# hlesmqh/WS3D

Hardware: AMD Instinct MI355X
Metric: KITTI scenes/sec (16384 pts) Stage-1 RPN fwd, 1/2/4/8 GPU; FPS+group HBM GB/s (higher is better)
Workload: dtype f32

## Files before the change

### include/ws3d_ops.h

```cpp
#ifndef WS3D_OPS_H
#define WS3D_OPS_H

#include <stddef.h>
#include <stdint.h>

#ifdef __cplusplus
extern "C" {
#endif

#define WS3D_OK 0
#define WS3D_E_INVALID (-1)
#define WS3D_E_LAUNCH (-2)
#define WS3D_E_WORKSPACE (-3)
#define WS3D_E_UNSUPPORTED (-4)

#if defined(__GNUC__)
#define WS3D_API __attribute__((visibility("default")))
#else
#define WS3D_API
#endif

typedef void *ws3d_stream_t;

#define WS3D_ABI_VERSION 6
WS3D_API int ws3d_abi_version(void);
WS3D_API int ws3d_tune(int key, int value);
WS3D_API int ws3d_dist_mode(void);
WS3D_API const char *ws3d_last_error(void);
WS3D_API int ws3d_device_info(char *name, int name_len, int *cu_count, int *lds_bytes_per_block);


WS3D_API int ws3d_furthest_point_sampling(int b, int n, int m, const float *xyz, float *temp, int32_t *idx,
                                 ws3d_stream_t stream);

WS3D_API int ws3d_furthest_point_sampling_gather(int b, int n, int m, const float *xyz, float *temp,
                                        int32_t *idx, float *new_xyz, ws3d_stream_t stream);

WS3D_API int ws3d_furthest_point_sampling_nested(int b, int n, int m, const float *xyz, int32_t *idx, float *new_xyz,
                                        ws3d_stream_t stream);

WS3D_API int ws3d_furthest_point_sampling_nested_chain(int b, int n, int levels, const int *m, const float *xyz, int32_t *const *idx,
                                                       float *const *new_xyz, ws3d_stream_t stream);


WS3D_API int ws3d_gather_points(int b, int c, int n, int npoints, const float *points, const int32_t *idx,
                       float *out, ws3d_stream_t stream);

WS3D_API int ws3d_gather_points_grad(int b, int c, int n, int npoints, const float *grad_out,
                            const int32_t *idx, float *grad_points, ws3d_stream_t stream);

WS3D_API int ws3d_ball_query(int b, int n, int m, float radius, int nsample, const float *new_xyz,
                    const float *xyz, int32_t *idx, const void *sorted, ws3d_stream_t stream);
WS3D_API int ws3d_ball_query_fill(int b, int n, int m, float radius, int nsample, const float *new_xyz,
                         const float *xyz, int32_t *idx, const void *sorted, ws3d_stream_t stream);
WS3D_API int ws3d_ball_query_pairs(int b, int n, int m, float radius, int nsample, const float *new_xyz, const float *xyz, int32_t *idx,
                          const void *sorted_grid, int32_t *rowc, int32_t *rowsrc, int32_t *total, ws3d_stream_t stream);

WS3D_API int ws3d_ball_query_pairs2(int b, int n, int m, const float *new_xyz, const float *xyz, const void *sorted_grid,
                                    float radius0, int nsample0, int32_t *idx0, int32_t *rowc0, int32_t *rowsrc0, int32_t *total0,
                                    float radius1, int nsample1, int32_t *idx1, int32_t *rowc1, int32_t *rowsrc1, int32_t *total1,
                                    ws3d_stream_t stream);


WS3D_API size_t ws3d_sorted_points_bytes(int b, int n);
WS3D_API int ws3d_sort_points_x(int b, int n, const float *xyz, void *sorted, ws3d_stream_t stream);
WS3D_API int ws3d_sort_points_xz(int b, int n, const float *xyz, void *sorted, ws3d_stream_t stream);
WS3D_API int ws3d_sort_points_grid(int b, int n, const float *xyz, void *sorted, ws3d_stream_t stream);
WS3D_API int ws3d_sort_points_jobs(int b, int njobs, const int *n, const int *kind, const float *const *xyz, void *const *sorted,
                                   ws3d_stream_t stream);

WS3D_API int ws3d_group_points(int b, int c, int n, int npoints, int nsample, const float *points,
                      const int32_t *idx, float *out, ws3d_stream_t stream);

WS3D_API int ws3d_group_points_grad(int b, int c, int n, int npoints, int nsample, const float *grad_out,
                           const int32_t *idx, float *grad_points, ws3d_stream_t stream);

WS3D_API int ws3d_query_and_group(int b, int n, int m, int c, float radius, int nsample, int use_xyz,
                         const float *xyz, const float *new_xyz, const float *features,
                         int32_t *idx_out, float *out, const void *sorted, ws3d_stream_t stream);

WS3D_API int ws3d_three_nn(int b, int n, int m, const float *unknown, const float *known, float *dist2,
                  int32_t *idx, const void *sorted_known, ws3d_stream_t stream);

WS3D_API int ws3d_three_nn_weights(long rows, const float *dist2, float *weight, ws3d_stream_t stream);
WS3D_API int ws3d_three_nn_w(int b, int n, int m, const float *unknown, const float *known, float *dist2, int32_t *idx, float *weight,
                             const void *sorted_known, ws3d_stream_t stream);
WS3D_API int ws3d_three_nn_wq(int b, int n, int m, const float *unknown, const float *known, float *dist2, int32_t *idx, float *weight,
                              const void *sorted_known, const void *sorted_unknown, ws3d_stream_t stream);
WS3D_API int ws3d_three_nn_jobs(int b, int njobs, const int *n, const int *m, const float *const *unknown, const void *const *sorted_known,
                                float *const *dist2, int32_t *const *idx, float *const *weight, const void *const *sorted_unknown,
                                ws3d_stream_t stream);

WS3D_API int ws3d_pool_nsample(long rows, int nsample, const float *x, float *out, uint8_t *arg, ws3d_stream_t stream);
WS3D_API int ws3d_pool_nsample_grad(long rows, int nsample, const float *grad_out, const uint8_t *arg, float *grad_x,
                                    ws3d_stream_t stream);

WS3D_API int ws3d_gemm_pool(long rows, int nsample, int k_dim, int o_dim, const float *x_rows, const float *wt,
                            const float *bias, int relu, float *out, int out_stride, const int32_t *gate, long gate_limit, ws3d_stream_t stream);

WS3D_API int ws3d_gather_gemm(int b, int n, int m, int nsample, int c_feat, int o_dim, const float *feats, const float *xyz,
                     const float *new_xyz, const int32_t *nbr, const float *wt, const float *bias, int relu, float *out,
                     ws3d_stream_t stream);

WS3D_API int ws3d_gather_gemm2(int b, int n, int m, int nsample, int c_feat, int o1, int o2, const float *feats, const float *xyz,
                      const float *new_xyz, const int32_t *nbr, const float *w1t, const float *b1, int relu1, const float *w2t,
                      const float *b2, int relu2, float *out, ws3d_stream_t stream);

WS3D_API int ws3d_pgather_gemm2(int b, int n, int m, int nsample, int o1, int o2, const float *pmat, int p_stride, const float *xyz,
                       const float *new_xyz, const int32_t *nbr, const float *w1x, const float *b1, int relu1,
                       const float *w2t, const float *b2, int relu2, float *out, const int32_t *gate, long gate_limit, ws3d_stream_t stream);
WS3D_API int ws3d_pgather_rows(int b, int n, int m, int nsample, int o1, const float *pmat, int p_stride, const float *xyz, const float *new_xyz,
                      const int32_t *nbr, const float *w1x, const float *b1, int relu1, float *out, ws3d_stream_t stream);

WS3D_API int ws3d_qinterp_rows(int b, int n, int m, int o, const float *q, const int32_t *idx, const float *weight, const float *lin,
                      const float *skip, int c1, const float *wb, const float *bias, int relu, float *out, ws3d_stream_t stream);


WS3D_API int ws3d_compact_pairs(long centres, int nsample, const int32_t *nbr, int32_t *rowc, int32_t *rowsrc, int32_t *total, ws3d_stream_t stream);
WS3D_API int ws3d_compact_pairs_count(long centres, int nsample, const int32_t *nbr, int32_t *cnt, ws3d_stream_t stream);
WS3D_API int ws3d_compact_pairs_rows(long centres, int nsample, const int32_t *nbr, const int32_t *cnt, const int32_t *incl, int32_t *rowc,
                            int32_t *rowsrc, int32_t *total, ws3d_stream_t stream);
WS3D_API int ws3d_pgather_gemm2_compact(int b, int n, int m, long max_rows, int o1, int o2, const float *pmat, int p_stride, const float *xyz,
                               const float *new_xyz, const int32_t *rowc, const int32_t *rowsrc, const int32_t *total, const float *w1x,
                               const float *b1, int relu1, const float *w2t, const float *b2, int relu2, float *out, long limit, ws3d_stream_t stream);
WS3D_API int ws3d_pgather_gemm3_compact(int b, int n, int m, long max_rows, int o1, int o2, int o3, const float *pmat, int p_stride, const float *xyz,
                               const float *new_xyz, const int32_t *rowc, const int32_t *rowsrc, const int32_t *total, const float *w1x,
                               const float *b1, int relu1, const float *w2t, const float *b2, int relu2, const float *w3t, const float *b3,
                               float *out, int out_stride, long limit, ws3d_stream_t stream);
WS3D_API int ws3d_gemm_pool_compact(long max_rows, int k_dim, int o_dim, const float *x_rows, const int32_t *rowc, const int32_t *total,
                           const float *wt, const float *bias, float *out, int out_stride, long limit, ws3d_stream_t stream);
typedef struct ws3d_compact_mlp_args {
    int b, n, m;
    long max_rows;
    int o1, o2, o3;
    const float *pmat;
    int p_stride;
    const float *xyz, *new_xyz;
    const int32_t *rowc, *rowsrc, *total;
    const float *w1x, *b1;
    int relu1;
    const float *w2t, *b2;
    int relu2;
    const float *w3t, *b3;
    float *mid;
    float *out;
    int out_stride;
    long limit;
} ws3d_compact_mlp_args;
WS3D_API int ws3d_compact_mlp_pair(int kind, const ws3d_compact_mlp_args *scale0, const ws3d_compact_mlp_args *scale1, ws3d_stream_t stream);
WS3D_API int ws3d_chain_mlp3_ticket_ints(void);
WS3D_API size_t ws3d_chain_mlp3_blob_floats(int o2);
WS3D_API int ws3d_chain_mlp3_pack(const ws3d_compact_mlp_args *scale, float *blob, ws3d_stream_t stream);
WS3D_API int ws3d_chain_mlp3(const ws3d_compact_mlp_args *scale0, const ws3d_compact_mlp_args *scale1, const float *blob0, const float *blob1,
                             int32_t *ticket, int workgroups, ws3d_stream_t stream);

WS3D_API int ws3d_sa_mlp3_pool_compact(int b, int n, int m, long max_rows, int c1, int c2, int c3, const float *xyz, const float *new_xyz,
                              const float *feat, const int32_t *rowc, const int32_t *rowsrc, const int32_t *total, const float *w1t,
                              const float *b1, const float *w2t, const float *b2, const float *w3t, const float *b3, float *out,
                              int out_stride, long limit, ws3d_stream_t stream);

WS3D_API int ws3d_sa_mlp3_pool_lists(int b, int n, int m, int nsample, int c1, int c2, int c3, const float *xyz, const float *new_xyz,
                            const float *feat, const int32_t *nbr, const float *w1t, const float *b1, const float *w2t, const float *b2,
                            const float *w3t, const float *b3, int relu3, float *out, int out_stride, const int32_t *gate, long gate_limit,
                            ws3d_stream_t stream);

WS3D_API int ws3d_interp_gemm(int b, int n, int m, int c2, int c1, int o_dim, const float *known_feats, const float *unknown_feats,
                     const int32_t *idx, const float *weight, const float *wt, const float *bias, int relu, float *out,
                     ws3d_stream_t stream);

WS3D_API size_t ws3d_conv1x1_wgrad_workspace_bytes(int b, int o, int c, long l);
WS3D_API int ws3d_conv1x1_wgrad(int b, int o, int c, long l, const float *grad_out, const float *x, float *grad_w,
                                void *workspace, size_t workspace_bytes, ws3d_stream_t stream);

WS3D_API size_t ws3d_bn_workspace_bytes(int b, int c, long l);
WS3D_API int ws3d_bn_relu_train_fwd(int b, int c, long l, const float *x, const float *gamma, const float *beta, float eps,
                                    float momentum, int relu, float *running_mean, float *running_var,
                                    int64_t *num_batches_tracked, float *y, float *save_mean, float *save_invstd,
                                    void *workspace, size_t workspace_bytes, ws3d_stream_t stream);
WS3D_API int ws3d_bn_relu_train_bwd(int b, int c, long l, const float *x, const float *dy, const float *gamma,
                                    const float *beta, const float *save_mean, const float *save_invstd, int relu, float *dx,
                                    float *dgamma, float *dbeta, void *workspace, size_t workspace_bytes, ws3d_stream_t stream);

WS3D_API int ws3d_three_interpolate(int b, int c, int m, int n, const float *points, const int32_t *idx,
                           const float *weight, float *out, ws3d_stream_t stream);

WS3D_API int ws3d_three_interpolate_grad(int b, int c, int n, int m, const float *grad_out,
                                const int32_t *idx, const float *weight, float *grad_points,
                                ws3d_stream_t stream);

WS3D_API size_t ws3d_scatter_workspace_bytes(int b, int c, int n_targets, long slots_per_scene);
WS3D_API int ws3d_group_points_grad_det(int b, int c, int n, int npoints, int nsample, const float *grad_out,
                                        const int32_t *idx, float *grad_points, void *workspace,
                                        size_t workspace_bytes, ws3d_stream_t stream);
WS3D_API int ws3d_three_interpolate_grad_det(int b, int c, int n, int m, const float *grad_out, const int32_t *idx,
                                             const float *weight, float *grad_points, void *workspace,
                                             size_t workspace_bytes, ws3d_stream_t stream);

WS3D_API int ws3d_bias_act_inplace(int b, int o_ch, long l, int relu, float *y, const float *bias,
                                   ws3d_stream_t stream);

WS3D_API int ws3d_rowmax_bias_act(int b, int o_ch, long m, int s, int relu, const float *y, const float *bias,
                                  float *out, ws3d_stream_t stream);

WS3D_API int ws3d_query_and_group_nlc(int b, int n, int m, int c, float radius, int nsample, int use_xyz,
                                      const float *xyz, const float *new_xyz, const float *features_nlc,
                                      int32_t *idx_out, float *out_nlc, const void *sorted, ws3d_stream_t stream);
WS3D_API int ws3d_three_interpolate_nlc(int b, int c, int m, int n, const float *feats_nlc, const int32_t *idx,
                                        const float *weight, float *out_nlc, int out_stride, ws3d_stream_t stream);
WS3D_API int ws3d_rowmax_rows(long rows_out, int ns, int o_ch, const float *y, float *out, int out_stride,
                              ws3d_stream_t stream);

WS3D_API int ws3d_sa_mlp3_pool(long rows, int nsample, int c1, int c2, int c3, const float *x_rows4,
                               const float *w1t, const float *b1, const float *w2t, const float *b2,
                               const float *w3t, const float *b3, int relu3, float *out, int out_stride,
                               ws3d_stream_t stream);

WS3D_API int ws3d_mlp2_rows(long rows, int k_dim, int o1, int o2, const float *x_rows, const float *w1t, const float *b1, int relu1,
                   const float *w2t, const float *b2, int relu2, float *out, int *ticket, ws3d_stream_t stream);

WS3D_API size_t ws3d_rpn_heads_blob_bytes(int o2);
WS3D_API int ws3d_rpn_heads_pack(int o2, const float *w1t, const float *b1, int relu1, const float *w2t, const float *b2, int relu2, void *blob,
                        ws3d_stream_t stream);
WS3D_API int ws3d_rpn_heads(long rows, const float *x_rows, int heads, const void *blob_cls, float *out_cls, int *ticket_cls, int o2_reg,
                   const void *blob_reg, float *out_reg, int *ticket_reg, int workgroups, ws3d_stream_t stream);

WS3D_API size_t ws3d_gemm_rows_pack_bytes(int k_dim, int n_dim);
WS3D_API int ws3d_gemm_rows_pack(int k_dim, int n_dim, const float *wt, void *pack, ws3d_stream_t stream);
WS3D_API int ws3d_gemm_rows_split(long rows, int k_dim, int n_dim, const float *a, const void *pack, const float *bias, int relu, float *out,
                         ws3d_stream_t stream);

WS3D_API int ws3d_qinterp_gemm(int b, int n, int m, int c, int o_dim, const float *q, const int32_t *idx, const float *weight, const float *lin,
                      const float *skip, int c1, const float *wb, const float *b1, int relu1, const float *w2t, const float *b2, int relu2,
                      float *out, ws3d_stream_t stream);


WS3D_API int ws3d_boxes_overlap_bev(int num_a, const float *boxes_a, int num_b, const float *boxes_b,
                           float *ans, ws3d_stream_t stream);

WS3D_API int ws3d_boxes_iou_bev(int num_a, const float *boxes_a, int num_b, const float *boxes_b,
                       float *ans, ws3d_stream_t stream);

WS3D_API int ws3d_boxes_iou3d_paired(int n, const float *boxes_a, const float *boxes_b, float *overlap_bev, float *iou2d, float *iou3d,
                                     ws3d_stream_t stream);

WS3D_API int ws3d_nms_mask(int boxes_num, const float *boxes, float thresh, int normal, int full_grid,
                  uint64_t *mask, ws3d_stream_t stream);

WS3D_API size_t ws3d_nms_workspace_bytes(int boxes_num);
WS3D_API int ws3d_nms(int boxes_num, const float *boxes, float thresh, int normal, int max_keep,
                      void *workspace, size_t workspace_bytes, int64_t *keep, int32_t *num_keep,
                      ws3d_stream_t stream);

WS3D_API int ws3d_nms_batched(int batch, int boxes_num, const float *boxes, float thresh, int normal,
                              int max_keep, void *workspace, size_t workspace_bytes, int64_t *keep,
                              int32_t *num_keep, ws3d_stream_t stream);


WS3D_API int ws3d_radius_nms_batched(int batch, int n, const float *centers, float radius, int max_keep,
                                     void *workspace, size_t workspace_bytes, int64_t *keep,
                                     int32_t *num_keep, ws3d_stream_t stream);

WS3D_API int ws3d_topk_sorted(int b, int n, int k, const float *scores, float *out_scores, int64_t *out_idx,
                              ws3d_stream_t stream);
WS3D_API size_t ws3d_topk_workspace_bytes(int b, int n);
WS3D_API int ws3d_topk_sorted_ws(int b, int n, int k, const float *scores, float *out_scores, int64_t *out_idx, void *workspace,
                                 size_t workspace_bytes, ws3d_stream_t stream);
WS3D_API int ws3d_topk_sorted_sigmoid(int b, int n, int k, const float *logits, float *out_scores, int64_t *out_idx, ws3d_stream_t stream);
WS3D_API int ws3d_topk_sorted_sigmoid_ws(int b, int n, int k, const float *logits, float *out_scores, int64_t *out_idx, void *workspace,
                                         size_t workspace_bytes, ws3d_stream_t stream);

WS3D_API int ws3d_decode_center_boxes(int b, int n, int bins, float loc_scope, float loc_bin_size, float h, float w,
                                      float l, const float *xyz, const float *rpn_reg, float *boxes,
                                      ws3d_stream_t stream);

WS3D_API int ws3d_gather_boxes_bev(int b, int n, int top, const float *box, const int64_t *order, float *box_sorted, float *bev,
                          ws3d_stream_t stream);
WS3D_API int ws3d_decode_gather_boxes_bev(int b, int n, int top, int bins, float loc_scope, float loc_bin_size, float h, float w, float l,
                                          const float *xyz, const float *rpn_reg, const int64_t *order, float *box_sorted, float *bev,
                                          ws3d_stream_t stream);
WS3D_API int ws3d_select_proposals(int b, int top, int keep_stride, int k, const float *box_sorted, const float *scores_sorted,
                          const int64_t *keep, const int32_t *num, float extra_width, float *boxes_out, float *scores_out,
                          int64_t *count, float *pooled_boxes, ws3d_stream_t stream);
WS3D_API int ws3d_select_proposals_packed(int b, int top, int keep_stride, int k, const float *box_sorted, const float *scores_sorted,
                                          const int64_t *keep, const int32_t *num, float extra_width, float *boxes_out, float *scores_out,
                                          int64_t *count, float *pooled_boxes, float *packed, ws3d_stream_t stream);
WS3D_API int ws3d_select_proposals_send(int b, int top, int keep_stride, int k, const float *box_sorted, const float *scores_sorted,
                                        const int64_t *keep, const int32_t *num, float extra_width, float *boxes_out, float *scores_out,
                                        int64_t *count, float *pooled_boxes, float *send, long send_stride, ws3d_stream_t stream);
WS3D_API int ws3d_split_points_clear(long rows, int c, const float *pc, float *xyz, float *feats, void *clear, size_t clear_bytes,
                                     ws3d_stream_t stream);


WS3D_API int ws3d_roipool3d(int batch_size, int pts_num, int boxes_num, int feature_in_len,
                   int sampled_pts_num, const float *xyz, const float *boxes3d,
                   const float *pts_feature, float *pooled_features, int32_t *pooled_empty_flag,
                   int32_t *pts_idx, ws3d_stream_t stream);
WS3D_API int ws3d_roipool3d_fill(int batch_size, int pts_num, int boxes_num, int feature_in_len,
                   int sampled_pts_num, const float *xyz, const float *boxes3d,
                   const float *pts_feature, float *pooled_features, int32_t *pooled_empty_flag,
                   int32_t *pts_idx, ws3d_stream_t stream);

WS3D_API size_t ws3d_roipool3d_workspace_bytes(int batch_size, int pts_num);
WS3D_API int ws3d_roipool3d_ws(int batch_size, int pts_num, int boxes_num, int feature_in_len, int sampled_pts_num, const float *xyz,
                               const float *boxes3d, const float *pts_feature, float *pooled_features, int32_t *pooled_empty_flag,
                               int32_t *pts_idx, int fill, void *workspace, size_t workspace_bytes, ws3d_stream_t stream);


WS3D_API int ws3d_pts_in_boxes3d(int boxes_num, int pts_num, const float *pts, const float *boxes3d,
                        int64_t *flag, ws3d_stream_t stream);


WS3D_API int ws3d_instance_clouds(int batch, int pts_num, int centres_num, int feat_len, int sampled_pts_num, float radius, int mask_mode,
                                  float mask_thresh, const float *pts, const float *score, const float *feats, const float *centres,
                                  const int32_t *num, float *cloud, float *cloud_feats, int32_t *count, int32_t *pts_idx,
                                  ws3d_stream_t stream);
WS3D_API int ws3d_instance_clouds_count(int batch, int pts_num, int centres_num, float radius, const float *pts, const float *centres,
                                        const int32_t *num, int32_t *count, ws3d_stream_t stream);
WS3D_API int ws3d_instance_clouds_emit(int batch, int pts_num, int centres_num, int feat_len, float radius, int mask_mode, float mask_thresh,
                                       const float *pts, const float *score, const float *feats, const float *centres, const int32_t *num,
                                       const int64_t *offsets, float *rows, float *row_feats, int32_t *row_idx, ws3d_stream_t stream);


WS3D_API int ws3d_click_prepare(int batch, int pts_num, int clicks_num, int side, const float *offsets, float gauss_height, float gauss_status,
                                float gauss_cov, float centre_y, const float *pts, const float *clicks, const int32_t *num, float *score,
                                float *cand, int32_t *cand_num, ws3d_stream_t stream);



WS3D_API int ws3d_kitti_overlaps(int metric, int criterion, int frames, long max_pairs, const int32_t *gt_off, const int32_t *dt_off,
                                 const int64_t *out_off, const double *dt_boxes, const double *gt_boxes, double *out,
                                 ws3d_stream_t stream);

WS3D_API int ws3d_kitti_collect_scores(int frames, int max_dt, const int32_t *gt_off, const int32_t *dt_off, const int64_t *out_off,
                                       const double *overlaps, const int32_t *ignored_gt, const int32_t *ignored_dt,
                                       const double *dt_score, double min_overlap, double *tp_score, int32_t *tp_flag,
                                       ws3d_stream_t stream);

WS3D_API size_t ws3d_kitti_count_workspace_bytes(int frames, int num_thresh);
WS3D_API int ws3d_kitti_count(int metric, int frames, int max_dt, int num_thresh, const double *thresholds, const int32_t *gt_off,
                              const int32_t *dt_off, const int32_t *dc_off, const int64_t *out_off, const double *overlaps,
                              const int32_t *ignored_gt, const int32_t *ignored_dt, const double *dt_score, const double *dt_alpha,
                              const double *gt_alpha, const double *dt_bbox, const double *dc_bbox, double min_overlap, int compute_aos,
                              void *workspace, size_t workspace_bytes, double *pr, ws3d_stream_t stream);


WS3D_API int ws3d_stage2_embed(long rows, int pts_per_cloud, const float *pts, const float *box_ce, float extend, const float *wx0,
                               const float *bx0, const float *wx1, const float *bx1, const float *wf0, const float *bf0, const float *wf1,
                               const float *bf1, const float *wm, const float *bm, float *xyz_out, float *feat, ws3d_stream_t stream);
WS3D_API int ws3d_stage2_boxes(int rows, int loc_bins, int head_bins, float loc_scope, float h, float w, float l, const float *rcnn_reg,
                               float *pred_boxes3d, float *box_ce, ws3d_stream_t stream);
WS3D_API int ws3d_stage2_select(int batch, int slots, float cls_thresh, float iou_thresh, const float *size_window, float ground_y,
                                const float *box_ce, const float *rcnn_ref, const float *rcnn_cls, const float *rcnn_iou, const float *center,
                                const int32_t *num, float *boxes, int32_t *keep, float *key, ws3d_stream_t stream);

WS3D_API int ws3d_stage2_rcnn_loss(int rows, int loc_bins, int head_bins, float loc_scope, float h, float w, float l, const float *rcnn_cls,
                                   const float *rcnn_reg, const float *pred_boxes3d, const float *gt_boxes, const float *cls, float *vals,
                                   int32_t *counts, float *grad_cls, float *grad_reg, ws3d_stream_t stream);
WS3D_API int ws3d_stage2_ioun_loss(int rows, const float *rcnn_iou, const float *rcnn_ref, const float *pred_boxes3d, const float *refined_box,
                                   const float *gt_boxes, const float *cls, float *vals, int32_t *counts, float *grad_iou, float *grad_ref,
                                   ws3d_stream_t stream);

#ifdef __cplusplus
}
#endif
#endif
```

### ws3d_amd/_lib.py

```python
from __future__ import annotations

import ctypes as C
import os

_HERE = os.path.dirname(os.path.abspath(__file__))
DIST_MODE = int(os.environ.get("WS3D_DIST_MODE", "0") or 0)
LIB_PATH = os.environ.get("WS3D_HIP_LIB") or os.path.join(
    _HERE, "libws3d_hip.so" if DIST_MODE == 0 else "libws3d_hip_dm%d.so" % DIST_MODE)

E_INVALID, E_LAUNCH, E_WORKSPACE, E_UNSUPPORTED = -1, -2, -3, -4
ABI_VERSION = 6

_vp = C.c_void_p
_i = C.c_int
_f = C.c_float
_sz = C.c_size_t

class CompactMlpArgs(C.Structure):
    _fields_ = [("b", _i), ("n", _i), ("m", _i), ("max_rows", C.c_long), ("o1", _i), ("o2", _i), ("o3", _i), ("pmat", _vp), ("p_stride", _i),
                ("xyz", _vp), ("new_xyz", _vp), ("rowc", _vp), ("rowsrc", _vp), ("total", _vp), ("w1x", _vp), ("b1", _vp), ("relu1", _i),
                ("w2t", _vp), ("b2", _vp), ("relu2", _i), ("w3t", _vp), ("b3", _vp), ("mid", _vp), ("out", _vp), ("out_stride", _i), ("limit", C.c_long)]


SIGNATURES = {
    "ws3d_abi_version": (_i, []),
    "ws3d_tune": (_i, [_i, _i]),
    "ws3d_dist_mode": (_i, []),
    "ws3d_last_error": (C.c_char_p, []),
    "ws3d_device_info": (_i, [C.c_char_p, _i, C.POINTER(_i), C.POINTER(_i)]),
    "ws3d_furthest_point_sampling": (_i, [_i, _i, _i, _vp, _vp, _vp, _vp]),
    "ws3d_furthest_point_sampling_gather": (_i, [_i, _i, _i, _vp, _vp, _vp, _vp, _vp]),
    "ws3d_furthest_point_sampling_nested": (_i, [_i, _i, _i, _vp, _vp, _vp, _vp]),
    "ws3d_furthest_point_sampling_nested_chain": (_i, [_i, _i, _i, _vp, _vp, _vp, _vp, _vp]),
    "ws3d_gather_points": (_i, [_i, _i, _i, _i, _vp, _vp, _vp, _vp]),
    "ws3d_gather_points_grad": (_i, [_i, _i, _i, _i, _vp, _vp, _vp, _vp]),
    "ws3d_ball_query": (_i, [_i, _i, _i, _f, _i, _vp, _vp, _vp, _vp, _vp]),
    "ws3d_ball_query_fill": (_i, [_i, _i, _i, _f, _i, _vp, _vp, _vp, _vp, _vp]),
    "ws3d_ball_query_pairs": (_i, [_i, _i, _i, _f, _i, _vp, _vp, _vp, _vp, _vp, _vp, _vp, _vp]),
    "ws3d_ball_query_pairs2": (_i, [_i, _i, _i, _vp, _vp, _vp, C.c_float, _i, _vp, _vp, _vp, _vp, C.c_float, _i, _vp, _vp, _vp, _vp, _vp]),
    "ws3d_sorted_points_bytes": (_sz, [_i, _i]),
    "ws3d_sort_points_x": (_i, [_i, _i, _vp, _vp, _vp]),
    "ws3d_sort_points_xz": (_i, [_i, _i, _vp, _vp, _vp]),
    "ws3d_sort_points_grid": (_i, [_i, _i, _vp, _vp, _vp]),
    "ws3d_sort_points_jobs": (_i, [_i, _i, _vp, _vp, _vp, _vp, _vp]),
    "ws3d_group_points": (_i, [_i, _i, _i, _i, _i, _vp, _vp, _vp, _vp]),
    "ws3d_group_points_grad": (_i, [_i, _i, _i, _i, _i, _vp, _vp, _vp, _vp]),
    "ws3d_query_and_group": (_i, [_i, _i, _i, _i, _f, _i, _i, _vp, _vp, _vp, _vp, _vp, _vp, _vp]),
    "ws3d_three_nn": (_i, [_i, _i, _i, _vp, _vp, _vp, _vp, _vp, _vp]),
    "ws3d_three_interpolate": (_i, [_i, _i, _i, _i, _vp, _vp, _vp, _vp, _vp]),
    "ws3d_three_interpolate_grad": (_i, [_i, _i, _i, _i, _vp, _vp, _vp, _vp, _vp]),
    "ws3d_bn_workspace_bytes": (C.c_size_t, [_i, _i, C.c_long]),
    "ws3d_bn_relu_train_fwd": (_i, [_i, _i, C.c_long, _vp, _vp, _vp, C.c_float, C.c_float, _i, _vp, _vp, _vp, _vp, _vp, _vp,
                                    _vp, C.c_size_t, _vp]),
    "ws3d_bn_relu_train_bwd": (_i, [_i, _i, C.c_long, _vp, _vp, _vp, _vp, _vp, _vp, _i, _vp, _vp, _vp, _vp, C.c_size_t, _vp]),
    "ws3d_conv1x1_wgrad_workspace_bytes": (C.c_size_t, [_i, _i, _i, C.c_long]),
    "ws3d_conv1x1_wgrad": (_i, [_i, _i, _i, C.c_long, _vp, _vp, _vp, _vp, C.c_size_t, _vp]),
    "ws3d_gemm_pool": (_i, [C.c_long, _i, _i, _i, _vp, _vp, _vp, _i, _vp, _i, _vp, C.c_long, _vp]),
    "ws3d_pool_nsample": (_i, [C.c_long, _i, _vp, _vp, _vp, _vp]),
    "ws3d_pool_nsample_grad": (_i, [C.c_long, _i, _vp, _vp, _vp, _vp]),
    "ws3d_scatter_workspace_bytes": (C.c_size_t, [_i, _i, _i, C.c_long]),
    "ws3d_group_points_grad_det": (_i, [_i, _i, _i, _i, _i, _vp, _vp, _vp, _vp, C.c_size_t, _vp]),
    "ws3d_three_interpolate_grad_det": (_i, [_i, _i, _i, _i, _vp, _vp, _vp, _vp, _vp, C.c_size_t, _vp]),
    "ws3d_query_and_group_nlc": (_i, [_i, _i, _i, _i, _f, _i, _i, _vp, _vp, _vp, _vp, _vp, _vp, _vp]),
    "ws3d_three_interpolate_nlc": (_i, [_i, _i, _i, _i, _vp, _vp, _vp, _vp, _i, _vp]),
    "ws3d_rowmax_rows": (_i, [C.c_long, _i, _i, _vp, _vp, _i, _vp]),
    "ws3d_sa_mlp3_pool": (_i, [C.c_long, _i, _i, _i, _i, _vp, _vp, _vp, _vp, _vp, _vp, _vp, _i, _vp, _i, _vp]),
    "ws3d_qinterp_gemm": (_i, [_i, _i, _i, _i, _i, _vp, _vp, _vp, _vp, _vp, _i, _vp, _vp, _i, _vp, _vp, _i, _vp, _vp]),
    "ws3d_mlp2_rows": (_i, [C.c_long, _i, _i, _i, _vp, _vp, _vp, _i, _vp, _vp, _i, _vp, _vp, _vp]),
    "ws3d_rpn_heads_blob_bytes": (_sz, [_i]),
    "ws3d_rpn_heads_pack": (_i, [_i, _vp, _vp, _i, _vp, _vp, _i, _vp, _vp]),
    "ws3d_rpn_heads": (_i, [C.c_long, _vp, _i, _vp, _vp, _vp, _i, _vp, _vp, _vp, _i, _vp]),
    "ws3d_gemm_rows_pack_bytes": (_sz, [_i, _i]),
    "ws3d_gemm_rows_pack": (_i, [_i, _i, _vp, _vp, _vp]),
    "ws3d_gemm_rows_split": (_i, [C.c_long, _i, _i, _vp, _vp, _vp, _i, _vp, _vp]),
    "ws3d_decode_center_boxes": (_i, [_i, _i, _i, _f, _f, _f, _f, _f, _vp, _vp, _vp, _vp]),
    "ws3d_topk_sorted": (_i, [_i, _i, _i, _vp, _vp, _vp, _vp]),
    "ws3d_topk_workspace_bytes": (C.c_size_t, [_i, _i]),
    "ws3d_topk_sorted_ws": (_i, [_i, _i, _i, _vp, _vp, _vp, _vp, C.c_size_t, _vp]),
    "ws3d_topk_sorted_sigmoid": (_i, [_i, _i, _i, _vp, _vp, _vp, _vp]),
    "ws3d_topk_sorted_sigmoid_ws": (_i, [_i, _i, _i, _vp, _vp, _vp, _vp, C.c_size_t, _vp]),
    "ws3d_three_nn_weights": (_i, [C.c_long, _vp, _vp, _vp]),
    "ws3d_three_nn_w": (_i, [_i, _i, _i, _vp, _vp, _vp, _vp, _vp, _vp, _vp]),
    "ws3d_three_nn_wq": (_i, [_i, _i, _i, _vp, _vp, _vp, _vp, _vp, _vp, _vp, _vp]),
    "ws3d_three_nn_jobs": (_i, [_i, _i, _vp, _vp, _vp, _vp, _vp, _vp, _vp, _vp, _vp]),
    "ws3d_bias_act_inplace": (_i, [_i, _i, C.c_long, _i, _vp, _vp, _vp]),
    "ws3d_rowmax_bias_act": (_i, [_i, _i, C.c_long, _i, _i, _vp, _vp, _vp, _vp]),
    "ws3d_boxes_overlap_bev": (_i, [_i, _vp, _i, _vp, _vp, _vp]),
    "ws3d_boxes_iou_bev": (_i, [_i, _vp, _i, _vp, _vp, _vp]),
    "ws3d_boxes_iou3d_paired": (_i, [_i, _vp, _vp, _vp, _vp, _vp, _vp]),
    "ws3d_nms_mask": (_i, [_i, _vp, _f, _i, _i, _vp, _vp]),
    "ws3d_nms_workspace_bytes": (_sz, [_i]),
    "ws3d_nms": (_i, [_i, _vp, _f, _i, _i, _vp, _sz, _vp, _vp, _vp]),
    "ws3d_nms_batched": (_i, [_i, _i, _vp, _f, _i, _i, _vp, _sz, _vp, _vp, _vp]),
    "ws3d_radius_nms_batched": (_i, [_i, _i, _vp, _f, _i, _vp, _sz, _vp, _vp, _vp]),
    "ws3d_gather_gemm": (_i, [_i, _i, _i, _i, _i, _i, _vp, _vp, _vp, _vp, _vp, _vp, _i, _vp, _vp]),
    "ws3d_gather_gemm2": (_i, [_i, _i, _i, _i, _i, _i, _i, _vp, _vp, _vp, _vp, _vp, _vp, _i, _vp, _vp, _i, _vp, _vp]),
    "ws3d_pgather_gemm2": (_i, [_i, _i, _i, _i, _i, _i, _vp, _i, _vp, _vp, _vp, _vp, _vp, _i, _vp, _vp, _i, _vp, _vp, C.c_long, _vp]),
    "ws3d_pgather_rows": (_i, [_i, _i, _i, _i, _i, _vp, _i, _vp, _vp, _vp, _vp, _vp, _i, _vp, _vp]),
    "ws3d_qinterp_rows": (_i, [_i, _i, _i, _i, _vp, _vp, _vp, _vp, _vp, _i, _vp, _vp, _i, _vp, _vp]),
    "ws3d_compact_pairs": (_i, [C.c_long, _i, _vp, _vp, _vp, _vp, _vp]),
    "ws3d_compact_pairs_count": (_i, [C.c_long, _i, _vp, _vp, _vp]),
    "ws3d_compact_pairs_rows": (_i, [C.c_long, _i, _vp, _vp, _vp, _vp, _vp, _vp, _vp]),
    "ws3d_pgather_gemm2_compact": (_i, [_i, _i, _i, C.c_long, _i, _i, _vp, _i, _vp, _vp, _vp, _vp, _vp, _vp, _vp, _i, _vp, _vp, _i, _vp, C.c_long, _vp]),
    "ws3d_pgather_gemm3_compact": (_i, [_i, _i, _i, C.c_long, _i, _i, _i, _vp, _i, _vp, _vp, _vp, _vp, _vp, _vp, _vp, _i, _vp, _vp, _i, _vp, _vp, _vp, _i, C.c_long, _vp]),
    "ws3d_gemm_pool_compact": (_i, [C.c_long, _i, _i, _vp, _vp, _vp, _vp, _vp, _vp, _i, C.c_long, _vp]),
    "ws3d_compact_mlp_pair": (_i, [_i, C.POINTER(CompactMlpArgs), C.POINTER(CompactMlpArgs), _vp]),
    "ws3d_chain_mlp3_ticket_ints": (_i, []),
    "ws3d_chain_mlp3_blob_floats": (_sz, [_i]),
    "ws3d_chain_mlp3_pack": (_i, [C.POINTER(CompactMlpArgs), _vp, _vp]),
    "ws3d_chain_mlp3": (_i, [C.POINTER(CompactMlpArgs), C.POINTER(CompactMlpArgs), _vp, _vp, _vp, _i, _vp]),
    "ws3d_sa_mlp3_pool_compact": (_i, [_i, _i, _i, C.c_long, _i, _i, _i, _vp, _vp, _vp, _vp, _vp, _vp, _vp, _vp, _vp, _vp, _vp, _vp, _vp, _i, C.c_long, _vp]),
    "ws3d_sa_mlp3_pool_lists": (_i, [_i, _i, _i, _i, _i, _i, _i, _vp, _vp, _vp, _vp, _vp, _vp, _vp, _vp, _vp, _vp, _i, _vp, _i, _vp, C.c_long, _vp]),
    "ws3d_interp_gemm": (_i, [_i, _i, _i, _i, _i, _i, _vp, _vp, _vp, _vp, _vp, _vp, _i, _vp, _vp]),
    "ws3d_gather_boxes_bev": (_i, [_i, _i, _i, _vp, _vp, _vp, _vp, _vp]),
    "ws3d_select_proposals": (_i, [_i, _i, _i, _i, _vp, _vp, _vp, _vp, _f, _vp, _vp, _vp, _vp, _vp]),
    "ws3d_decode_gather_boxes_bev": (_i, [_i, _i, _i, _i, _f, _f, _f, _f, _f, _vp, _vp, _vp, _vp, _vp, _vp]),
    "ws3d_select_proposals_packed": (_i, [_i, _i, _i, _i, _vp, _vp, _vp, _vp, _f, _vp, _vp, _vp, _vp, _vp, _vp]),
    "ws3d_select_proposals_send": (_i, [_i, _i, _i, _i, _vp, _vp, _vp, _vp, _f, _vp, _vp, _vp, _vp, _vp, C.c_long, _vp]),
    "ws3d_split_points_clear": (_i, [C.c_long, _i, _vp, _vp, _vp, _vp, C.c_size_t, _vp]),
    "ws3d_roipool3d": (_i, [_i, _i, _i, _i, _i, _vp, _vp, _vp, _vp, _vp, _vp, _vp]),
    "ws3d_roipool3d_fill": (_i, [_i, _i, _i, _i, _i, _vp, _vp, _vp, _vp, _vp, _vp, _vp]),
    "ws3d_roipool3d_workspace_bytes": (C.c_size_t, [_i, _i]),
    "ws3d_roipool3d_ws": (_i, [_i, _i, _i, _i, _i, _vp, _vp, _vp, _vp, _vp, _vp, _i, _vp, C.c_size_t, _vp]),
    "ws3d_pts_in_boxes3d": (_i, [_i, _i, _vp, _vp, _vp, _vp]),
    "ws3d_instance_clouds": (_i, [_i, _i, _i, _i, _i, _f, _i, _f, _vp, _vp, _vp, _vp, _vp, _vp, _vp, _vp, _vp, _vp]),
    "ws3d_instance_clouds_count": (_i, [_i, _i, _i, _f, _vp, _vp, _vp, _vp, _vp]),
    "ws3d_instance_clouds_emit": (_i, [_i, _i, _i, _i, _f, _i, _f, _vp, _vp, _vp, _vp, _vp, _vp, _vp, _vp, _vp, _vp]),
    "ws3d_click_prepare": (_i, [_i, _i, _i, _i, _vp, _f, _f, _f, _f, _vp, _vp, _vp, _vp, _vp, _vp, _vp]),
    "ws3d_kitti_overlaps": (_i, [_i, _i, _i, C.c_long, _vp, _vp, _vp, _vp, _vp, _vp, _vp]),
    "ws3d_kitti_collect_scores": (_i, [_i, _i, _vp, _vp, _vp, _vp, _vp, _vp, _vp, C.c_double, _vp, _vp, _vp]),
    "ws3d_kitti_count_workspace_bytes": (_sz, [_i, _i]),
    "ws3d_kitti_count": (_i, [_i, _i, _i, _i, _vp, _vp, _vp, _vp, _vp, _vp, _vp, _vp, _vp, _vp, _vp, _vp, _vp, C.c_double, _i, _vp,
                              _sz, _vp, _vp]),
    "ws3d_stage2_embed": (_i, [C.c_long, _i, _vp, _vp, _f] + [_vp] * 10 + [_vp, _vp, _vp]),
    "ws3d_stage2_boxes": (_i, [_i, _i, _i, _f, _f, _f, _f, _vp, _vp, _vp, _vp]),
    "ws3d_stage2_select": (_i, [_i, _i, _f, _f, C.POINTER(_f), _f, _vp, _vp, _vp, _vp, _vp, _vp, _vp, _vp, _vp, _vp]),
    "ws3d_stage2_rcnn_loss": (_i, [_i, _i, _i, _f, _f, _f, _f] + [_vp] * 9 + [_vp]),
    "ws3d_stage2_ioun_loss": (_i, [_i] + [_vp] * 10 + [_vp]),
}


class Ws3dError(RuntimeError):
    pass


_lib = None


def load() -> C.CDLL:
    global _lib
    if _lib is not None:
        return _lib
    if not os.path.exists(LIB_PATH):
        raise Ws3dError(
            f"{LIB_PATH} is missing: the MI355X HIP library has not been built "
            "(run `python -m ws3d_amd.build`).  ws3d_amd has no CPU fallback.")
    import torch
    try:
        lib = C.CDLL(LIB_PATH)
    except OSError as e:
        raise Ws3dError(f"cannot load {LIB_PATH}: {e}") from e
    for name, (res, args) in SIGNATURES.items():
        fn = getattr(lib, name)
        fn.restype = res
        fn.argtypes = args
    if lib.ws3d_abi_version() != ABI_VERSION:
        raise Ws3dError(f"{LIB_PATH} exports ABI version {lib.ws3d_abi_version()}, this package binds version {ABI_VERSION}: "
                        "rebuild it (`python -m ws3d_amd.build`)")
    if not os.environ.get("WS3D_HIP_LIB") and lib.ws3d_dist_mode() != DIST_MODE:
        raise Ws3dError(f"{LIB_PATH} was built with WS3D_DIST_MODE={lib.ws3d_dist_mode()}, expected {DIST_MODE}: rebuild it")
    _lib = lib
    return lib


def check(rc: int, what: str = "") -> None:
    if rc != 0:
        msg = load().ws3d_last_error()
        raise Ws3dError(f"{what or 'ws3d'} failed (rc={rc}): {msg.decode() if msg else ''}")
```

### ws3d_amd/build.py

```python
from __future__ import annotations

import argparse
import concurrent.futures as cf
import glob
import os
import shutil
import subprocess
import sys

HERE = os.path.dirname(os.path.abspath(__file__))
CSRC = os.path.join(HERE, "csrc")
OBJ = os.path.join(CSRC, "build")
LIB = os.path.join(HERE, "libws3d_hip.so")
DIST_MODES = (0, 1, 2)


def lib_path(dist_mode: int = 0) -> str:
    return LIB if dist_mode == 0 else os.path.join(HERE, "libws3d_hip_dm%d.so" % dist_mode)
ARCH = "gfx950"
SOURCES = ["core.hip", "fps.hip", "fps_v3.hip", "fps_bucket.hip", "fps_nested.hip", "ballquery_group.hip", "interpolate.hip", "roipool3d.hip", "iou3d.hip", "proposals.hip", "scatter_det.hip", "sa_mlp.hip", "bn_relu.hip", "gemm_pool.hip", "conv_wgrad.hip", "chain_mlp.hip", "rpn_heads.hip", "gemm_rows.hip", "kitti_eval.hip", "instance_clouds.hip", "click.hip", "stage2.hip", "stage2_loss.hip"]
CXXFLAGS = ["-O3", "-std=c++17", "-fPIC", "-ffp-contract=off", "-fno-fast-math",
            "-fvisibility=hidden", "-Wall", "-Wno-unused-function"]


def hipcc() -> str:
    for cand in (os.environ.get("HIPCC"), shutil.which("hipcc"), "/opt/rocm/bin/hipcc"):
        if cand and os.path.exists(cand):
            return cand
    raise RuntimeError("hipcc not found (looked at $HIPCC, PATH, /opt/rocm/bin)")


def _deps(src: str):
    return [src, *glob.glob(os.path.join(CSRC, "*.h")), os.path.join(HERE, "..", "include", "ws3d_ops.h"),
            os.path.join(CSRC, "exports.map"), os.path.abspath(__file__)]


def _compile(src: str, force: bool, verbose: bool, dist_mode: int = 0) -> str:
    path = os.path.join(CSRC, src)
    obj = os.path.join(OBJ if dist_mode == 0 else OBJ + "_dm%d" % dist_mode, os.path.splitext(src)[0] + ".o")
    if not force and os.path.exists(obj) and all(
            os.path.getmtime(obj) >= os.path.getmtime(d) for d in _deps(path)):
        return obj
    cmd = [hipcc(), f"--offload-arch={ARCH}", *CXXFLAGS, f"-DWS3D_DIST_MODE={dist_mode}", *os.environ.get("WS3D_EXTRA_DEFS", "").split(), "-c", path, "-o", obj]
    if verbose:
        print(" ".join(cmd), flush=True)
    r = subprocess.run(cmd, capture_output=True, text=True)
    if r.returncode != 0:
        raise RuntimeError(f"hipcc failed for {src}:\n{r.stdout}\n{r.stderr}")
    if verbose and r.stderr.strip():
        print(r.stderr)
    return obj


def build(force: bool = False, verbose: bool = False, dist_mode: int = 0) -> str:
    LIB = lib_path(dist_mode)
    os.makedirs(OBJ if dist_mode == 0 else OBJ + "_dm%d" % dist_mode, exist_ok=True)
    with cf.ThreadPoolExecutor(max_workers=min(len(SOURCES), os.cpu_count() or 4, 16)) as ex:
        objs = list(ex.map(lambda s: _compile(s, force, verbose, dist_mode), SOURCES))
    if force or not os.path.exists(LIB) or any(os.path.getmtime(o) > os.path.getmtime(LIB) for o in objs):
        cmd = [hipcc(), f"--offload-arch={ARCH}", "-shared", "-fPIC", "-Wl,--version-script=" + os.path.join(CSRC, "exports.map"), "-o", LIB, *objs]
        if verbose:
            print(" ".join(cmd), flush=True)
        r = subprocess.run(cmd, capture_output=True, text=True)
        if r.returncode != 0:
            raise RuntimeError(f"link failed:\n{r.stdout}\n{r.stderr}")
    return LIB


def rebuild_one(src: str, verbose: bool = False) -> str:
    _compile(src, True, verbose)
    objs = [os.path.join(OBJ, os.path.splitext(s_)[0] + ".o") for s_ in SOURCES]
    missing = [o for o in objs if not os.path.exists(o)]
    if missing:
        return build(False, verbose)
    cmd = [hipcc(), f"--offload-arch={ARCH}", "-shared", "-fPIC", "-Wl,--version-script=" + os.path.join(CSRC, "exports.map"), "-o", LIB, *objs]
    r = subprocess.run(cmd, capture_output=True, text=True)
    if r.returncode != 0:
        raise RuntimeError(f"link failed:\n{r.stdout}\n{r.stderr}")
    return LIB


if __name__ == "__main__":
    ap = argparse.ArgumentParser()
    ap.add_argument("--force", action="store_true")
    ap.add_argument("--verbose", action="store_true")
    ap.add_argument("--dist-mode", type=int, default=0, choices=DIST_MODES)
    ap.add_argument("--all-dist-modes", action="store_true")
    ap.add_argument("--only", default=None, help="recompile this one source (forced) and relink")
    a = ap.parse_args()
    if a.only:
        print(rebuild_one(a.only, a.verbose))
        sys.exit(0)
    for dm in (DIST_MODES if a.all_dist_modes else (a.dist_mode,)):
        print(build(a.force, a.verbose, dm))
    sys.exit(0)
```

### ws3d_amd/compat.py

```python
from __future__ import annotations

import sys
import types

import os

import torch

from . import _lib
from ._lib import Ws3dError, check


def _dev(*tensors):
    dev = None
    for t in tensors:
        if t is None:
            continue
        if not t.is_cuda:
            raise Ws3dError("ws3d_amd ops need HIP ('cuda') tensors; there is no CPU fallback")
        if not t.is_contiguous():
            raise Ws3dError("ws3d_amd ops need contiguous tensors (the reference asserts the same)")
        if dev is None:
            dev = t.device
        elif t.device != dev:
# ... 345 lines not shown
    with _on(dev):
        check(_lib.load().ws3d_rowmax_rows(R, ns, O, _p(y), view.data_ptr(), out.size(1), _stream()), "rowmax_rows")
    return out


def bn_relu_train_fwd(x, gamma, beta, running_mean, running_var, momentum, eps, relu=True, num_batches_tracked=None):
    dev = _dev(x, gamma, beta, running_mean, running_var, num_batches_tracked)
    if num_batches_tracked is not None and num_batches_tracked.dtype != torch.int64:
        raise TypeError("num_batches_tracked must be int64")
    _f32(x, "x"); _f32(gamma, "gamma"); _f32(beta, "beta")
    b, c = x.size(0), x.size(1)
    l = x.numel() // max(b * c, 1)
    y = torch.empty_like(x)
    mean = torch.empty((c,), dtype=torch.float32, device=dev)
    invstd = torch.empty((c,), dtype=torch.float32, device=dev)
    lib = _lib.load()
    nbytes = lib.ws3d_bn_workspace_bytes(b, c, l)
    ws = torch.empty((nbytes + 7) // 8, dtype=torch.float64, device=dev)
    with _on(dev):
        check(lib.ws3d_bn_relu_train_fwd(b, c, l, _p(x), _p(gamma), _p(beta), float(eps), float(momentum), int(bool(relu)),
                                         _p(running_mean), _p(running_var), _p(num_batches_tracked), _p(y), _p(mean), _p(invstd), _p(ws), nbytes,
                                         _stream()), "bn_relu_train_fwd")
    return y, mean, invstd


def bn_relu_train_bwd(x, dy, gamma, beta, save_mean, save_invstd, relu=True):
    dev = _dev(x, dy, gamma, beta, save_mean, save_invstd)
    _f32(x, "x"); _f32(dy, "dy")
    b, c = x.size(0), x.size(1)
    l = x.numel() // max(b * c, 1)
    dx = torch.empty_like(x)
    dgamma = torch.empty((c,), dtype=torch.float32, device=dev)
    dbeta = torch.empty((c,), dtype=torch.float32, device=dev)
    lib = _lib.load()
    nbytes = lib.ws3d_bn_workspace_bytes(b, c, l)
    ws = torch.empty((nbytes + 7) // 8, dtype=torch.float64, device=dev)
    with _on(dev):
        check(lib.ws3d_bn_relu_train_bwd(b, c, l, _p(x), _p(dy), _p(gamma), _p(beta), _p(save_mean), _p(save_invstd),
                                         int(bool(relu)), _p(dx), _p(dgamma), _p(dbeta), _p(ws), nbytes, _stream()),
              "bn_relu_train_bwd")
    return dx, dgamma, dbeta


def conv1x1_wgrad(grad_out, x, shape=None):
    dev = _dev(grad_out, x)
    _f32(grad_out, "grad_out"); _f32(x, "x")
    b, o, c = x.size(0), grad_out.size(1), x.size(1)
    l = x.numel() // max(b * c, 1)
    if grad_out.numel() != b * o * l:
        raise Ws3dError("conv1x1_wgrad: grad_out and x disagree in shape")
    gw = torch.empty((o, c) if shape is None else tuple(shape), dtype=torch.float32, device=dev)
    lib = _lib.load()
    nbytes = lib.ws3d_conv1x1_wgrad_workspace_bytes(b, o, c, l)
    ws = torch.empty((nbytes + 3) // 4, dtype=torch.float32, device=dev)
    with _on(dev):
        check(lib.ws3d_conv1x1_wgrad(b, o, c, l, _p(grad_out), _p(x), _p(gw), _p(ws), nbytes, _stream()), "conv1x1_wgrad")
    return gw


def _gate(gate):
    if gate is None:
        return None, 0
    total, limit = gate
    return total.data_ptr(), int(limit)


def gemm_pool(x_rows, wt, bias, relu, nsample, out, col0=0, gate=None):
    dev = _dev(x_rows, wt, bias)
    _f32(x_rows, "x_rows"); _f32(wt, "wt")
    rows, k = x_rows.shape
    o = wt.size(1)
    if rows % 64 or rows // 64 > 65535 or o % 64 or k % 4 or nsample not in (16, 32) or wt.size(0) != k:
        return False
    view = out[:, col0:col0 + o]
    with _on(dev):
        check(_lib.load().ws3d_gemm_pool(rows, nsample, k, o, _p(x_rows), _p(wt), _p(bias), int(bool(relu)), view.data_ptr(),
                                         out.size(1), *_gate(gate), _stream()), "gemm_pool")
    return True


def gather_gemm(feats, xyz, new_xyz, nbr, wt_feat_then_xyz, bias, relu):
    dev = _dev(feats, xyz, new_xyz, nbr, wt_feat_then_xyz)
    _f32(feats, "feats"); _f32(xyz, "xyz"); _f32(new_xyz, "new_xyz"); _i32(nbr, "nbr"); _f32(wt_feat_then_xyz, "wt")
    B, N, C = feats.shape
    M, ns = nbr.size(1), nbr.size(2)
    O = wt_feat_then_xyz.size(1)
    rows = B * M * ns
    if C % 4 or O % 64 or rows % 64 or rows // 64 > 65535 or wt_feat_then_xyz.size(0) != C + 3 or not feats.is_contiguous():
        return None
    out = torch.empty((rows, O), dtype=torch.float32, device=dev)
    with _on(dev):
        check(_lib.load().ws3d_gather_gemm(B, N, M, ns, C, O, _p(feats), _p(xyz), _p(new_xyz), _p(nbr), _p(wt_feat_then_xyz), _p(bias),
                                           int(bool(relu)), _p(out), _stream()), "gather_gemm")
    return out


def gather_gemm2(feats, xyz, new_xyz, nbr, w1t_feat_then_xyz, b1, relu1, w2t, b2, relu2):
    dev = _dev(feats, xyz, new_xyz, nbr, w1t_feat_then_xyz, w2t)
    _f32(feats, "feats"); _f32(xyz, "xyz"); _f32(new_xyz, "new_xyz"); _i32(nbr, "nbr"); _f32(w1t_feat_then_xyz, "w1t"); _f32(w2t, "w2t")
    B, N, C = feats.shape
    M, ns = nbr.size(1), nbr.size(2)
    O1, O2 = w1t_feat_then_xyz.size(1), w2t.size(1)
    rows = B * M * ns
    if (C % 4 or O1 not in (64, 128, 256) or O2 % 4 or rows % 64 or w1t_feat_then_xyz.size(0) != C + 3 or w2t.size(0) != O1 or
            not feats.is_contiguous() or not w2t.is_contiguous() or not w1t_feat_then_xyz.is_contiguous()):
        return None
    out = torch.empty((rows, O2), dtype=torch.float32, device=dev)
    with _on(dev):
        check(_lib.load().ws3d_gather_gemm2(B, N, M, ns, C, O1, O2, _p(feats), _p(xyz), _p(new_xyz), _p(nbr), _p(w1t_feat_then_xyz), _p(b1),
                                            int(bool(relu1)), _p(w2t), _p(b2), int(bool(relu2)), _p(out), _stream()), "gather_gemm2")
    return out


def pgather_gemm2(pmat, col0, o1, xyz, new_xyz, nbr, w1x, b1, relu1, w2t, b2, relu2, out=None, gate=None):
    dev = _dev(pmat, xyz, new_xyz, nbr, w1x, w2t)
    _f32(pmat, "pmat"); _f32(xyz, "xyz"); _f32(new_xyz, "new_xyz"); _i32(nbr, "nbr"); _f32(w1x, "w1x"); _f32(w2t, "w2t")
    B, N = xyz.size(0), xyz.size(1)
    M, ns = nbr.size(1), nbr.size(2)
    O2 = w2t.size(1)
    if (o1 not in (64, 128) or O2 % 4 or (M * ns) % 64 or pmat.dim() != 2 or pmat.size(0) != B * N or pmat.stride(1) != 1 or
            col0 < 0 or col0 + o1 > pmat.size(1) or tuple(w1x.shape) != (3, o1) or w2t.size(0) != o1 or not w1x.is_contiguous() or not w2t.is_contiguous()):
        return None
    if out is None:
        out = torch.empty((B * M * ns, O2), dtype=torch.float32, device=dev)
    elif tuple(out.shape) != (B * M * ns, O2) or not out.is_contiguous():
        raise ValueError("pgather_gemm2: out must be a contiguous (B*M*ns, O2) tensor")
    with _on(dev):
        check(_lib.load().ws3d_pgather_gemm2(B, N, M, ns, o1, O2, pmat.data_ptr() + 4 * col0, pmat.stride(0), _p(xyz), _p(new_xyz), _p(nbr), _p(w1x), _p(b1),
                                             int(bool(relu1)), _p(w2t), _p(b2), int(bool(relu2)), _p(out), *_gate(gate), _stream()), "pgather_gemm2")
    return out


def pgather_rows(pmat, col0, o1, xyz, new_xyz, nbr, w1x, b1, relu1):
    dev = _dev(pmat, xyz, new_xyz, nbr, w1x)
    _f32(pmat, "pmat"); _f32(xyz, "xyz"); _f32(new_xyz, "new_xyz"); _i32(nbr, "nbr"); _f32(w1x, "w1x")
    B, N = xyz.size(0), xyz.size(1)
    M, ns = nbr.size(1), nbr.size(2)
    if (o1 % 4 or col0 % 4 or pmat.dim() != 2 or pmat.size(0) != B * N or pmat.stride(1) != 1 or pmat.stride(0) % 4 or col0 < 0 or
            col0 + o1 > pmat.size(1) or tuple(w1x.shape) != (3, o1) or not w1x.is_contiguous() or pmat.data_ptr() % 16):
        return None
    out = torch.empty((B * M * ns, o1), dtype=torch.float32, device=dev)
    with _on(dev):
        check(_lib.load().ws3d_pgather_rows(B, N, M, ns, o1, pmat.data_ptr() + 4 * col0, pmat.stride(0), _p(xyz), _p(new_xyz), _p(nbr), _p(w1x), _p(b1),
                                            int(bool(relu1)), _p(out), _stream()), "pgather_rows")
    return out


def qinterp_rows(q, idx, weight, lin=None, skip=None, wb=None, bias=None, relu=True):
    dev = _dev(q, idx, weight)
    _f32(q, "q"); _i32(idx, "idx"); _f32(weight, "weight")
    B, M, O = q.shape
    N = idx.size(1)
    c1 = 0 if skip is None else skip.size(2)
    if (O % 4 or not q.is_contiguous() or (lin is None and c1 > 4) or (lin is not None and (tuple(lin.shape) != (B * N, O) or not lin.is_contiguous())) or
            (lin is None and c1 > 0 and (wb is None or tuple(wb.shape) != (c1, O) or not wb.is_contiguous() or not skip.is_contiguous()))):
        return None
    out = torch.empty((B * N, O), dtype=torch.float32, device=dev)
    with _on(dev):
        check(_lib.load().ws3d_qinterp_rows(B, N, M, O, _p(q), _p(idx), _p(weight), _p(lin), _p(skip), c1, _p(wb), _p(bias), int(bool(relu)), _p(out),
                                            _stream()), "qinterp_rows")
    return out


def qinterp_gemm(q, idx, weight, w2t, b2, relu2, lin=None, skip=None, wb=None, bias=None, relu=True):
    dev = _dev(q, idx, weight, w2t)
    _f32(q, "q"); _i32(idx, "idx"); _f32(weight, "weight"); _f32(w2t, "w2t")
    B, M, C = q.shape
    N = idx.size(1)
    O = w2t.size(1)
    c1 = 0 if skip is None else skip.size(2)
    if ((B * N) % 64 or C % 16 or O % 128 or w2t.size(0) != C or not q.is_contiguous() or not w2t.is_contiguous() or not idx.is_contiguous() or
            not weight.is_contiguous() or (lin is None and c1 > 4) or (lin is not None and (tuple(lin.shape) != (B * N, C) or not lin.is_contiguous())) or
            (lin is None and c1 > 0 and (wb is None or tuple(wb.shape) != (c1, C) or not wb.is_contiguous() or not skip.is_contiguous()))):
        return None
    out = torch.empty((B * N, O), dtype=torch.float32, device=dev)
    with _on(dev):
        check(_lib.load().ws3d_qinterp_gemm(B, N, M, C, O, _p(q), _p(idx), _p(weight), _p(lin), _p(skip), c1, _p(wb), _p(bias), int(bool(relu)), _p(w2t),
                                            _p(b2), int(bool(relu2)), _p(out), _stream()), "qinterp_gemm")
    return out


def compact_pairs(nbr, ordered=False):
    if not ordered:
        dev = _dev(nbr)
        _i32(nbr, "nbr")
        B, M, ns = nbr.shape
        rowc = torch.empty(B * M * ns, dtype=torch.int32, device=dev)
        rowsrc = torch.empty(B * M * ns, dtype=torch.int32, device=dev)
        total = torch.zeros(1, dtype=torch.int32, device=dev)
        with _on(dev):
            check(_lib.load().ws3d_compact_pairs(B * M, ns, _p(nbr), _p(rowc), _p(rowsrc), _p(total), _stream()), "compact_pairs")
        return rowc, rowsrc, total
    dev = _dev(nbr)
    _i32(nbr, "nbr")
    B, M, ns = nbr.shape
    centres = B * M
    cnt = torch.empty(centres, dtype=torch.int32, device=dev)
    rowc = torch.empty(centres * ns, dtype=torch.int32, device=dev)
    rowsrc = torch.empty(centres * ns, dtype=torch.int32, device=dev)
    total = torch.empty(1, dtype=torch.int32, device=dev)
    with _on(dev):
        lib = _lib.load()
        check(lib.ws3d_compact_pairs_count(centres, ns, _p(nbr), _p(cnt), _stream()), "compact_pairs_count")
        incl = torch.cumsum(cnt, dim=0, dtype=torch.int32)
        check(lib.ws3d_compact_pairs_rows(centres, ns, _p(nbr), _p(cnt), _p(incl), _p(rowc), _p(rowsrc), _p(total), _stream()), "compact_pairs_rows")
    return rowc, rowsrc, total


def pgather_gemm2_compact(pmat, col0, o1, xyz, new_xyz, pairs, w1x, b1, relu1, w2t, b2, relu2, limit=-1):
    rowc, rowsrc, total = pairs
    dev = _dev(pmat, xyz, new_xyz, rowc, w1x, w2t)
    _f32(pmat, "pmat"); _f32(xyz, "xyz"); _f32(new_xyz, "new_xyz"); _f32(w1x, "w1x"); _f32(w2t, "w2t")
    B, N = xyz.size(0), xyz.size(1)
    M = new_xyz.size(1)
    O2 = w2t.size(1)
    rows = rowc.numel()
    if (o1 not in (64, 128, 256) or O2 % 4 or pmat.dim() != 2 or pmat.size(0) != B * N or pmat.stride(1) != 1 or col0 < 0 or col0 + o1 > pmat.size(1) or
            tuple(w1x.shape) != (3, o1) or w2t.size(0) != o1 or not w1x.is_contiguous() or not w2t.is_contiguous()):
        return None
    out = torch.empty((rows, O2), dtype=torch.float32, device=dev)
    with _on(dev):
        check(_lib.load().ws3d_pgather_gemm2_compact(B, N, M, rows, o1, O2, pmat.data_ptr() + 4 * col0, pmat.stride(0), _p(xyz), _p(new_xyz), _p(rowc),
                                                     _p(rowsrc), _p(total), _p(w1x), _p(b1), int(bool(relu1)), _p(w2t), _p(b2), int(bool(relu2)), _p(out),
                                                     int(limit), _stream()), "pgather_gemm2_compact")
    return out


def pgather_gemm3_compact(pmat, col0, o1, xyz, new_xyz, pairs, w1x, b1, relu1, w2t, b2, relu2, w3t, b3, out2d, col_offset, limit=-1, max_lds=160 * 1024):
    rowc, rowsrc, total = pairs
    dev = _dev(pmat, xyz, new_xyz, rowc, w1x, w2t, w3t, out2d)
    _f32(pmat, "pmat"); _f32(xyz, "xyz"); _f32(new_xyz, "new_xyz"); _f32(w1x, "w1x"); _f32(w2t, "w2t"); _f32(w3t, "w3t"); _f32(out2d, "out2d")
    B, N = xyz.size(0), xyz.size(1)
    M = new_xyz.size(1)
    O2, O3 = w2t.size(1), w3t.size(1)
    rows = rowc.numel()
    lds = 4 * ((o1 + (O2 + 15) // 16 * 16) * 65 + 2 * 16 * 64)
    if (o1 not in (64, 128) or O2 % 4 or O3 % 128 or lds > min(max_lds, 160 * 1024 - 1024) or pmat.dim() != 2 or pmat.size(0) != B * N or pmat.stride(1) != 1 or
            col0 < 0 or col0 + o1 > pmat.size(1) or tuple(w1x.shape) != (3, o1) or w2t.size(0) != o1 or w3t.size(0) != O2 or not w1x.is_contiguous() or
            not w2t.is_contiguous() or not w3t.is_contiguous() or out2d.dim() != 2 or out2d.stride(1) != 1 or col_offset < 0 or col_offset + O3 > out2d.size(1)):
        return False
    with _on(dev):
        check(_lib.load().ws3d_pgather_gemm3_compact(B, N, M, rows, o1, O2, O3, pmat.data_ptr() + 4 * col0, pmat.stride(0), _p(xyz), _p(new_xyz), _p(rowc),
                                                     _p(rowsrc), _p(total), _p(w1x), _p(b1), int(bool(relu1)), _p(w2t), _p(b2), int(bool(relu2)), _p(w3t), _p(b3),
                                                     out2d.data_ptr() + 4 * col_offset, out2d.stride(0), int(limit), _stream()), "pgather_gemm3_compact")
    return True


def gemm_pool_compact(x_rows, pairs, wt, bias, out2d, col_offset, limit=-1):
    rowc, rowsrc, total = pairs
    dev = _dev(x_rows, rowc, wt, out2d)
    _f32(x_rows, "x_rows"); _f32(wt, "wt"); _f32(out2d, "out2d")
    rows, k = x_rows.shape
    o = wt.size(1)
    if (k % 4 or o % 64 or wt.size(0) != k or rows != rowc.numel() or not x_rows.is_contiguous() or not wt.is_contiguous() or out2d.dim() != 2 or
            out2d.stride(1) != 1 or col_offset < 0 or col_offset + o > out2d.size(1)):
        return False
    with _on(dev):
        check(_lib.load().ws3d_gemm_pool_compact(rows, k, o, _p(x_rows), _p(rowc), _p(total), _p(wt), _p(bias), out2d.data_ptr() + 4 * col_offset,
                                                 out2d.stride(0), int(limit), _stream()), "gemm_pool_compact")
    return True


def compact_mlp_pair(kind, scales, max_lds=160 * 1024, mids=None):
    import ctypes as C
    if len(scales) != 2 or scales[0]["o1"] != scales[1]["o1"]:
        return None if kind == 2 else False
    blocks, keep, outs = [], [], []
    for si, a in enumerate(scales):
        rowc, rowsrc, total = a["pairs"]
        pmat, xyz, new_xyz, w1x, w2t, w3t, out2d, o1, col0, col = a["pmat"], a["xyz"], a["new_xyz"], a["w1x"], a["w2t"], a["w3t"], a["out2d"], a["o1"], a["col0"], a["col_offset"]
        dev = _dev(pmat, xyz, new_xyz, rowc, w1x, w2t, w3t, out2d)
        for t_, nm in ((pmat, "pmat"), (xyz, "xyz"), (new_xyz, "new_xyz"), (w1x, "w1x"), (w2t, "w2t"), (w3t, "w3t"), (out2d, "out2d")):
            _f32(t_, nm)
        B, N, M = xyz.size(0), xyz.size(1), new_xyz.size(1)
        O2, O3 = w2t.size(1), w3t.size(1)
        rows = rowc.numel()
        lds3 = 4 * ((o1 + (O2 + 15) // 16 * 16) * 65 + 2 * 16 * 64)
        ok = (O2 % 4 == 0 and pmat.dim() == 2 and pmat.size(0) == B * N and pmat.stride(1) == 1 and col0 >= 0 and col0 + o1 <= pmat.size(1) and
              tuple(w1x.shape) == (3, o1) and w2t.size(0) == o1 and w3t.size(0) == O2 and w1x.is_contiguous() and w2t.is_contiguous() and w3t.is_contiguous() and
              out2d.dim() == 2 and out2d.stride(1) == 1 and col >= 0 and col + O3 <= out2d.size(1))
        if kind == 3:
            ok = ok and o1 in (64, 128) and O3 % 128 == 0 and lds3 <= min(max_lds, 160 * 1024 - 1024)
        elif kind == 2:
            ok = ok and o1 in (64, 128, 256)
        else:
            ok = ok and O3 % 64 == 0 and mids is not None and tuple(mids[si].shape) == (rows, O2) and mids[si].is_contiguous()
        if not ok:
            return None if kind == 2 else False
        mid = mids[si] if kind == 1 else (torch.empty((rows, O2), dtype=torch.float32, device=dev) if kind == 2 else None)
        outs.append(mid)
        keep.append((pmat, xyz, new_xyz, rowc, rowsrc, total, w1x, w2t, w3t, out2d, mid, a["b1"], a["b2"], a["b3"]))
        blocks.append(_lib.CompactMlpArgs(B, N, M, rows, o1, O2, O3, pmat.data_ptr() + 4 * col0, pmat.stride(0), _p(xyz), _p(new_xyz), _p(rowc), _p(rowsrc),
                                          _p(total), _p(w1x), _p(a["b1"]), int(bool(a["relu1"])), _p(w2t), _p(a["b2"]), int(bool(a["relu2"])), _p(w3t), _p(a["b3"]),
                                          _p(mid), out2d.data_ptr() + 4 * col, out2d.stride(0), -1))
    with _on(dev):
        rc = _lib.load().ws3d_compact_mlp_pair(int(kind), C.byref(blocks[0]), C.byref(blocks[1]), _stream())
    if rc == _lib.E_UNSUPPORTED:
        return None if kind == 2 else False
    check(rc, "compact_mlp_pair")
    return outs if kind == 2 else True


CHAIN_WORKGROUPS = 0
TUNE_KEYS = {"chain_wgs": 0, "mlp2_wgs": 1, "sa1_wgs": 2, "fp_wgs": 3, "pair_wgs": 4, "bq_wide_nw": 5}


def tune(name: str, value: int = -1) -> int:
    rc = _lib.load().ws3d_tune(TUNE_KEYS[name], int(value))
    if rc < 0:
        check(rc, "tune")
    return rc


_CHAIN_BLOBS = {}


def chain_ticket_ints() -> int:
    return int(_lib.load().ws3d_chain_mlp3_ticket_ints())


def _chain_blob(block, tensors, dev):
    import ctypes as C
    key = tuple((t.data_ptr(), t._version) if t is not None else None for t in tensors)
    hit = _CHAIN_BLOBS.get(key)
    if hit is None:
        n = int(_lib.load().ws3d_chain_mlp3_blob_floats(block.o2))
        blob = torch.empty(n, dtype=torch.float32, device=dev)
        with _on(dev):
            check(_lib.load().ws3d_chain_mlp3_pack(C.byref(block), _p(blob), _stream()), "chain_mlp3_pack")
        if torch.cuda.is_current_stream_capturing():
            return blob
        hit = _CHAIN_BLOBS[key] = (blob, tensors)
    return hit[0]


def chain_mlp3(scales, ticket):
    import ctypes as C
    if len(scales) not in (1, 2) or ticket is None or ticket.dtype != torch.int32 or ticket.numel() < chain_ticket_ints() or not ticket.is_contiguous():
        return False
    blocks, keep, blobs = [], [], []
    for a in scales:
        rowc, rowsrc, total = a["pairs"]
        pmat, xyz, new_xyz, w1x, w2t, w3t, out2d, o1, col0, col = a["pmat"], a["xyz"], a["new_xyz"], a["w1x"], a["w2t"], a["w3t"], a["out2d"], a["o1"], a["col0"], a["col_offset"]
        dev = _dev(pmat, xyz, new_xyz, rowc, w1x, w2t, w3t, out2d, ticket)
        for t_, nm in ((pmat, "pmat"), (xyz, "xyz"), (new_xyz, "new_xyz"), (w1x, "w1x"), (w2t, "w2t"), (w3t, "w3t"), (out2d, "out2d")):
            _f32(t_, nm)
        B, N, M = xyz.size(0), xyz.size(1), new_xyz.size(1)
        O2, O3 = w2t.size(1), w3t.size(1)
        ok = (o1 == 64 and O2 <= 96 and O3 == 128 and pmat.dim() == 2 and pmat.size(0) == B * N and pmat.stride(1) == 1 and pmat.stride(0) % 4 == 0 and
              col0 >= 0 and col0 % 4 == 0 and col0 + o1 <= pmat.size(1) and tuple(w1x.shape) == (3, o1) and w2t.size(0) == o1 and w3t.size(0) == O2 and
              w1x.is_contiguous() and w2t.is_contiguous() and w3t.is_contiguous() and out2d.dim() == 2 and out2d.stride(1) == 1 and col >= 0 and
              col % 4 == 0 and col + O3 <= out2d.size(1) and xyz.is_contiguous() and new_xyz.is_contiguous())
        if not ok:
            return False
        keep.append((pmat, xyz, new_xyz, rowc, rowsrc, total, w1x, w2t, w3t, out2d, a["b1"], a["b2"], a["b3"]))
        blocks.append(_lib.CompactMlpArgs(B, N, M, rowc.numel(), o1, O2, O3, pmat.data_ptr() + 4 * col0, pmat.stride(0), _p(xyz), _p(new_xyz), _p(rowc), _p(rowsrc),
                                          _p(total), _p(w1x), _p(a["b1"]), int(bool(a["relu1"])), _p(w2t), _p(a["b2"]), int(bool(a["relu2"])), _p(w3t), _p(a["b3"]),
                                          None, out2d.data_ptr() + 4 * col, out2d.stride(0), int(a.get("limit", -1))))
        blobs.append(_chain_blob(blocks[-1], (w1x, a["b1"], w2t, a["b2"], w3t, a["b3"]), dev))
    with _on(dev):
        rc = _lib.load().ws3d_chain_mlp3(C.byref(blocks[0]), C.byref(blocks[1]) if len(blocks) > 1 else None, _p(blobs[0]), _p(blobs[1]) if len(blobs) > 1 else None,
                                         _p(ticket), int(CHAIN_WORKGROUPS), _stream())
    if rc == _lib.E_UNSUPPORTED:
        return False
    check(rc, "chain_mlp3")
    return True


def interp_gemm(known_feats, unknown_feats, idx, weight, wt, bias, relu):
    dev = _dev(known_feats, idx, weight, wt)
    _f32(known_feats, "known_feats"); _i32(idx, "idx"); _f32(weight, "weight"); _f32(wt, "wt")
    B, M, C2 = known_feats.shape
    N = idx.size(1)
    C1 = 0 if unknown_feats is None else unknown_feats.size(2)
    O = wt.size(1)
    rows = B * N
    if (C2 % 4 or O % 64 or rows % 64 or rows // 64 > 65535 or wt.size(0) != C2 + C1 or not known_feats.is_contiguous() or
            (unknown_feats is not None and not unknown_feats.is_contiguous())):
        return None
    out = torch.empty((rows, O), dtype=torch.float32, device=dev)
    with _on(dev):
        check(_lib.load().ws3d_interp_gemm(B, N, M, C2, C1, O, _p(known_feats), _p(unknown_feats), _p(idx), _p(weight), _p(wt), _p(bias),
                                           int(bool(relu)), _p(out), _stream()), "interp_gemm")
    return out


def mlp2_rows(x2d, w1t, b1, relu1, w2t, b2, relu2, ticket=None):
    dev = _dev(x2d, w1t, w2t)
    _f32(x2d, "x2d"); _f32(w1t, "w1t"); _f32(w2t, "w2t")
    R, K = x2d.shape
    O1, O2 = w1t.size(1), w2t.size(1)
    if (K != 128 or O1 != 128 or w1t.size(0) != 128 or w2t.size(0) != 128 or O2 > 64 or R % 32 or not x2d.is_contiguous() or
            not w1t.is_contiguous() or not w2t.is_contiguous()):
        return None
    out = torch.empty((R, O2), dtype=torch.float32, device=dev)
    if ticket is None:
        ticket = torch.zeros(1, dtype=torch.int32, device=dev)
    with _on(dev):
        check(_lib.load().ws3d_mlp2_rows(R, K, O1, O2, _p(x2d), _p(w1t), _p(b1), int(bool(relu1)), _p(w2t), _p(b2), int(bool(relu2)),
                                         _p(out), _p(ticket), _stream()), "mlp2_rows")
    return out


def rpn_heads_pack(w1t, b1, relu1, w2t, b2, relu2):
    dev = _dev(w1t, w2t)
    _f32(w1t, "w1t"); _f32(w2t, "w2t")
    O2 = w2t.size(1) if w2t.dim() == 2 else 0
    n = int(_lib.load().ws3d_rpn_heads_blob_bytes(O2))
    if n == 0 or tuple(w1t.shape) != (128, 128) or w2t.size(0) != 128 or not w1t.is_contiguous() or not w2t.is_contiguous():
        return None
    for b, nm, o in ((b1, "b1", 128), (b2, "b2", O2)):
        if b is not None:
            _f32(b, nm)
            if b.numel() != o or not b.is_contiguous():
                return None
    blob = torch.empty((n + 15) // 16 * 4, dtype=torch.float32, device=dev)
    with _on(dev):
        check(_lib.load().ws3d_rpn_heads_pack(O2, _p(w1t), _p(b1), int(bool(relu1)), _p(w2t), _p(b2), int(bool(relu2)), _p(blob), _stream()),
              "rpn_heads_pack")
    return blob


def rpn_heads(x2d, heads, blob_cls, blob_reg, o2_reg, tickets, workgroups=0):
    dev = _dev(x2d)
    _f32(x2d, "x2d")
    if (x2d.dim() != 2 or x2d.size(1) != 128 or x2d.size(0) % 32 or not x2d.is_contiguous() or heads not in (1, 2, 3) or
            tickets is None or tickets.dtype != torch.int32 or tickets.numel() < 2 or not tickets.is_contiguous()):
        return None
    R = x2d.size(0)
    out_cls = torch.empty((R, 1), dtype=torch.float32, device=dev) if heads & 1 else None
    out_reg = torch.empty((R, int(o2_reg)), dtype=torch.float32, device=dev) if heads & 2 else None
    with _on(dev):
        rc = _lib.load().ws3d_rpn_heads(R, _p(x2d), int(heads), _p(blob_cls) if heads & 1 else None, _p(out_cls), _p(tickets[0:1]),
                                        int(o2_reg) if heads & 2 else 0, _p(blob_reg) if heads & 2 else None, _p(out_reg), _p(tickets[1:2]),
                                        int(workgroups), _stream())
    if rc == _lib.E_UNSUPPORTED:
        return None
    check(rc, "rpn_heads")
    return out_cls, out_reg


def gemm_rows_pack(wt):
    dev = _dev(wt)
    _f32(wt, "wt")
    if wt.dim() != 2:
        return None
    K, N = wt.shape
    n = int(_lib.load().ws3d_gemm_rows_pack_bytes(K, N))
    if n == 0:
        return None
    pack = torch.empty((n + 15) // 16 * 4, dtype=torch.float32, device=dev)
    with _on(dev):
        check(_lib.load().ws3d_gemm_rows_pack(K, N, _p(wt), _p(pack), _stream()), "gemm_rows_pack")
    return pack


def gemm_rows_split(x2d, pack, n_dim, bias=None, relu=False, out=None):
    if pack is None or x2d.dim() != 2 or not x2d.is_contiguous() or (bias is not None and (not bias.is_contiguous() or bias.numel() != n_dim)):
        return None
    dev = _dev(x2d, pack, bias, out)
    _f32(x2d, "x2d")
    R, K = x2d.shape
    n_dim = int(n_dim)
    if R % 64 or K % 32 or n_dim % 64 or pack.numel() * pack.element_size() < K * n_dim * 6:
        return None
    if bias is not None:
        _f32(bias, "bias")
    if out is None:
        out = torch.empty((R, n_dim), dtype=torch.float32, device=dev)
    elif tuple(out.shape) != (R, n_dim) or out.dtype != torch.float32:
        return None
    with _on(dev):
        rc = _lib.load().ws3d_gemm_rows_split(R, K, n_dim, _p(x2d), _p(pack), _p(bias), int(bool(relu)), _p(out), _stream())
    if rc == _lib.E_UNSUPPORTED:
        return None
    check(rc, "gemm_rows_split")
    return out


def pool_nsample(x):
    dev = _dev(x)
    _f32(x, "x")
    ns = x.size(-1)
    out = torch.empty(x.shape[:-1], dtype=torch.float32, device=dev)
    arg = torch.empty(x.shape[:-1], dtype=torch.uint8, device=dev)
    with _on(dev):
        check(_lib.load().ws3d_pool_nsample(out.numel(), ns, _p(x), _p(out), _p(arg), _stream()), "pool_nsample")
    return out, arg


def pool_nsample_grad(grad_out, arg, nsample):
    dev = _dev(grad_out, arg)
    _f32(grad_out, "grad_out")
    if arg.dtype != torch.uint8 or not arg.is_contiguous():
        raise TypeError("arg must be a contiguous uint8 tensor")
    grad_x = torch.empty(tuple(grad_out.shape) + (nsample,), dtype=torch.float32, device=dev)
    with _on(dev):
        check(_lib.load().ws3d_pool_nsample_grad(grad_out.numel(), nsample, _p(grad_out), _p(arg), _p(grad_x), _stream()),
              "pool_nsample_grad")
    return grad_x


SA_MLP3_SHAPES = {(16, 16, 32), (32, 32, 64)}


def sa_mlp3_pool(x_rows4, nsample, layers, out, col0=0):
    (w1, b1, r1), (w2, b2, r2), (w3, b3, r3) = layers
    widths = (w1.size(1), w2.size(1), w3.size(1))
    if (x_rows4.size(1) != 4 or widths not in SA_MLP3_SHAPES or nsample not in (16, 32) or not (r1 and r2)
            or b1 is None or b2 is None or b3 is None):
        return False
    dev = _dev(x_rows4, out)
    view = out[:, col0:col0 + widths[2]]
    with _on(dev):
        check(_lib.load().ws3d_sa_mlp3_pool(x_rows4.size(0), nsample, widths[0], widths[1], widths[2], _p(x_rows4),
                                            _p(w1), _p(b1), _p(w2), _p(b2), _p(w3), _p(b3), int(bool(r3)),
                                            view.data_ptr(), out.size(1), _stream()), "sa_mlp3_pool")
    return True


def sa_mlp3_pool_compact(xyz, new_xyz, feat1, pairs, layers, out, col0=0, limit=-1):
    (w1, b1, r1), (w2, b2, r2), (w3, b3, r3) = layers
    widths = (w1.size(1), w2.size(1), w3.size(1))
    if (widths not in ((16, 16, 32), (32, 32, 64)) or w1.size(0) != 4 or not (r1 and r2 and r3) or b1 is None or b2 is None or b3 is None or
            feat1.numel() != xyz.size(0) * xyz.size(1) or not feat1.is_contiguous()):
        return False
    rowc, rowsrc, total = pairs
    dev = _dev(xyz, new_xyz, feat1, rowc, out)
    _f32(xyz, "xyz"); _f32(new_xyz, "new_xyz"); _f32(feat1, "feat1"); _f32(out, "out")
    view = out[:, col0:col0 + widths[2]]
    with _on(dev):
        check(_lib.load().ws3d_sa_mlp3_pool_compact(xyz.size(0), xyz.size(1), new_xyz.size(1), rowc.numel(), widths[0], widths[1], widths[2], _p(xyz),
                                                    _p(new_xyz), _p(feat1), _p(rowc), _p(rowsrc), _p(total), _p(w1), _p(b1), _p(w2), _p(b2), _p(w3),
                                                    _p(b3), view.data_ptr(), out.size(1), int(limit), _stream()), "sa_mlp3_pool_compact")
    return True


def sa_mlp3_pool_lists(xyz, new_xyz, feat1, nbr, layers, out, col0=0, gate=None):
    (w1, b1, r1), (w2, b2, r2), (w3, b3, r3) = layers
    widths = (w1.size(1), w2.size(1), w3.size(1))
    ns = nbr.size(2)
    if (widths not in ((16, 16, 32), (32, 32, 64)) or w1.size(0) != 4 or ns not in (16, 32) or not (r1 and r2) or b1 is None or b2 is None or b3 is None or
            feat1.numel() != xyz.size(0) * xyz.size(1) or not feat1.is_contiguous() or nbr.numel() % 32):
        return False
    dev = _dev(xyz, new_xyz, feat1, nbr, out)
    _f32(xyz, "xyz"); _f32(new_xyz, "new_xyz"); _f32(feat1, "feat1"); _i32(nbr, "nbr"); _f32(out, "out")
    view = out[:, col0:col0 + widths[2]]
    with _on(dev):
        check(_lib.load().ws3d_sa_mlp3_pool_lists(xyz.size(0), xyz.size(1), new_xyz.size(1), ns, widths[0], widths[1], widths[2], _p(xyz), _p(new_xyz),
                                                  _p(feat1), _p(nbr), _p(w1), _p(b1), _p(w2), _p(b2), _p(w3), _p(b3), int(bool(r3)), view.data_ptr(),
                                                  out.size(1), *_gate(gate), _stream()), "sa_mlp3_pool_lists")
    return True


def three_nn_wrapper(b, n, m, unknown_tensor, known_tensor, dist2_tensor, idx_tensor, sorted_known=None):
    dev = _dev(unknown_tensor, known_tensor, dist2_tensor, idx_tensor)
    _f32(unknown_tensor, "unknown"); _f32(known_tensor, "known"); _i32(idx_tensor, "idx")
    with _on(dev):
        check(_lib.load().ws3d_three_nn(b, n, m, _p(unknown_tensor), _p(known_tensor), _p(dist2_tensor),
                                         _p(idx_tensor), _p(sorted_known) if sorted_known is not None else None,
                                         _stream()), "three_nn")


def three_interpolate_wrapper(b, c, m, n, points_tensor, idx_tensor, weight_tensor, out_tensor):
    dev = _dev(points_tensor, idx_tensor, weight_tensor, out_tensor)
    _f32(points_tensor, "points"); _i32(idx_tensor, "idx"); _f32(weight_tensor, "weight")
    with _on(dev):
        check(_lib.load().ws3d_three_interpolate(b, c, m, n, _p(points_tensor), _p(idx_tensor),
                                                  _p(weight_tensor), _p(out_tensor), _stream()),
              "three_interpolate")


def three_interpolate_grad_wrapper(b, c, n, m, grad_out_tensor, idx_tensor, weight_tensor, grad_points_tensor):
    dev = _dev(grad_out_tensor, idx_tensor, weight_tensor, grad_points_tensor)
    _f32(grad_out_tensor, "grad_out"); _i32(idx_tensor, "idx"); _f32(weight_tensor, "weight")
    with _on(dev):
        check(_lib.load().ws3d_three_interpolate_grad(b, c, n, m, _p(grad_out_tensor), _p(idx_tensor),
                                                       _p(weight_tensor), _p(grad_points_tensor), _stream()),
              "three_interpolate_grad")


def group_points_grad_det(b, c, n, npoints, nsample, grad_out_tensor, idx_tensor, grad_points_tensor):
    dev = _dev(grad_out_tensor, idx_tensor, grad_points_tensor)
    _f32(grad_out_tensor, "grad_out"); _i32(idx_tensor, "idx"); _f32(grad_points_tensor, "grad_points")
    lib = _lib.load()
    nbytes = lib.ws3d_scatter_workspace_bytes(b, c, n, npoints * nsample)
    ws = torch.empty(max(nbytes, 256), dtype=torch.uint8, device=dev)
    with _on(dev):
        check(lib.ws3d_group_points_grad_det(b, c, n, npoints, nsample, _p(grad_out_tensor), _p(idx_tensor),
                                             _p(grad_points_tensor), _p(ws), nbytes, _stream()), "group_points_grad_det")
    return 1


def three_interpolate_grad_det(b, c, n, m, grad_out_tensor, idx_tensor, weight_tensor, grad_points_tensor):
    dev = _dev(grad_out_tensor, idx_tensor, weight_tensor, grad_points_tensor)
    _f32(grad_out_tensor, "grad_out"); _i32(idx_tensor, "idx"); _f32(weight_tensor, "weight")
    lib = _lib.load()
    nbytes = lib.ws3d_scatter_workspace_bytes(b, c, m, n * 3)
    ws = torch.empty(max(nbytes, 256), dtype=torch.uint8, device=dev)
    with _on(dev):
        check(lib.ws3d_three_interpolate_grad_det(b, c, n, m, _p(grad_out_tensor), _p(idx_tensor), _p(weight_tensor),
                                                  _p(grad_points_tensor), _p(ws), nbytes, _stream()),
              "three_interpolate_grad_det")
    return 1


def topk_sorted(scores, k, spread=None, sigmoid=False):
    dev = _dev(scores)
    _f32(scores, "scores")
    B, N = scores.shape
    vals = torch.empty((B, k), dtype=torch.float32, device=dev)
    idx = torch.empty((B, k), dtype=torch.int64, device=dev)
    lib = _lib.load()
    if spread is None:
        spread = TOPK_SEGMENTS and not torch.cuda.is_current_stream_capturing()
    need = int(lib.ws3d_topk_workspace_bytes(B, N)) if spread else 0
    with _on(dev):
        if need:
            ws = torch.empty(need // 8, dtype=torch.int64, device=dev)
            check((lib.ws3d_topk_sorted_sigmoid_ws if sigmoid else lib.ws3d_topk_sorted_ws)(B, N, k, _p(scores), _p(vals), _p(idx), _p(ws), need,
                                                                                            _stream()), "topk_sorted")
        else:
            check((lib.ws3d_topk_sorted_sigmoid if sigmoid else lib.ws3d_topk_sorted)(B, N, k, _p(scores), _p(vals), _p(idx), _stream()), "topk_sorted")
    return vals, idx


def decode_center_boxes(xyz, rpn_reg, loc_scope, loc_bin_size, mean_size):
    dev = _dev(xyz, rpn_reg)
    _f32(xyz, "xyz"); _f32(rpn_reg, "rpn_reg")
    B, N = xyz.size(0), xyz.size(1)
    bins = int(loc_scope / loc_bin_size) * 2
    if rpn_reg.size(2) != 4 * bins or not rpn_reg.is_contiguous() or not xyz.is_contiguous():
        raise ValueError("decode_center_boxes: rpn_reg must be contiguous (B,N,%d)" % (4 * bins))
    boxes = torch.empty((B, N, 7), dtype=torch.float32, device=dev)
    h, w, l = mean_size
    with _on(dev):
        check(_lib.load().ws3d_decode_center_boxes(B, N, bins, float(loc_scope), float(loc_bin_size), float(h), float(w),
                                                   float(l), _p(xyz), _p(rpn_reg), _p(boxes), _stream()), "decode_center_boxes")
    return boxes


def decode_gather_boxes_bev(xyz, rpn_reg, order, loc_scope, loc_bin_size, mean_size):
    dev = _dev(xyz, rpn_reg, order)
    _f32(xyz, "xyz"); _f32(rpn_reg, "rpn_reg")
    B, N, top = xyz.size(0), xyz.size(1), order.size(1)
    bins = int(loc_scope / loc_bin_size) * 2
    if rpn_reg.size(2) != 4 * bins or not rpn_reg.is_contiguous() or not xyz.is_contiguous():
        raise ValueError("decode_gather_boxes_bev: rpn_reg must be contiguous (B,N,%d)" % (4 * bins))
    if order.dtype != torch.int64 or not order.is_contiguous():
        raise ValueError("decode_gather_boxes_bev: order must be a contiguous int64 tensor")
    out = torch.empty((B, top, 7), dtype=torch.float32, device=dev)
    bev = torch.empty((B, top, 5), dtype=torch.float32, device=dev)
    h, w, l = mean_size
    with _on(dev):
        check(_lib.load().ws3d_decode_gather_boxes_bev(B, N, top, bins, float(loc_scope), float(loc_bin_size), float(h), float(w), float(l),
                                                       _p(xyz), _p(rpn_reg), _p(order), _p(out), _p(bev), _stream()), "decode_gather_boxes_bev")
    return out, bev


def split_points_clear(pointcloud, clear=None):
    dev = _dev(pointcloud) if clear is None else _dev(pointcloud, clear)
    _f32(pointcloud, "pointcloud")
    if not pointcloud.is_contiguous() or pointcloud.dim() != 3 or pointcloud.size(2) < 3:
        raise ValueError("split_points_clear: pointcloud must be a contiguous (B,N,C>=3) tensor")
    B, N, Cc = pointcloud.shape
    xyz = torch.empty((B, N, 3), dtype=torch.float32, device=dev)
    feats = torch.empty((B, N, Cc - 3), dtype=torch.float32, device=dev) if Cc > 3 else None
    nbytes = 0 if clear is None else clear.numel() * clear.element_size()
    if clear is not None and (not clear.is_contiguous() or nbytes % 16 or clear.data_ptr() % 16):
        raise ValueError("split_points_clear: `clear` must be contiguous, 16-byte aligned and a multiple of 16 bytes long")
    with _on(dev):
        check(_lib.load().ws3d_split_points_clear(B * N, Cc, _p(pointcloud), _p(xyz), _p(feats), _p(clear), nbytes, _stream()), "split_points_clear")
    return xyz, feats


def gather_boxes_bev(box, order):
    dev = _dev(box, order)
    _f32(box, "box")
    if order.dtype != torch.int64 or not order.is_contiguous() or not box.is_contiguous():
        raise ValueError("gather_boxes_bev: box must be contiguous fp32 and order contiguous int64")
    B, N, top = box.size(0), box.size(1), order.size(1)
    box_sorted = torch.empty((B, top, 7), dtype=torch.float32, device=dev)
    bev = torch.empty((B, top, 5), dtype=torch.float32, device=dev)
    with _on(dev):
        check(_lib.load().ws3d_gather_boxes_bev(B, N, top, _p(box), _p(order), _p(box_sorted), _p(bev), _stream()), "gather_boxes_bev")
    return box_sorted, bev


def select_proposals(box_sorted, scores_sorted, keep, num, k, extra_width=None, packed=False):
    dev = _dev(box_sorted, scores_sorted, keep, num)
    _f32(box_sorted, "box_sorted"); _f32(scores_sorted, "scores")
    if keep.dtype != torch.int64 or num.dtype != torch.int32:
        raise ValueError("select_proposals: keep must be int64 and num int32 (ws3d_nms_batched outputs)")
    B, top = box_sorted.size(0), box_sorted.size(1)
    boxes = torch.empty((B, k, 7), dtype=torch.float32, device=dev)
    scores = torch.empty((B, k), dtype=torch.float32, device=dev)
    count = torch.empty((B,), dtype=torch.int64, device=dev)
    pooled = torch.empty((B, k, 7), dtype=torch.float32, device=dev) if extra_width is not None else None
    send = packed if torch.is_tensor(packed) else None
    if send is not None:
        if send.dtype != torch.float32 or send.device != dev or send.dim() != 2 or send.size(0) < B or send.size(1) != k * 8 + 1 or not send.is_contiguous():
            raise ValueError("select_proposals: the send buffer must be a contiguous float32 (>= %d, %d) tensor on %s, got %s %s"
                             % (B, k * 8 + 1, dev, tuple(send.shape), send.dtype))
        with _on(dev):
            check(_lib.load().ws3d_select_proposals_send(B, top, keep.size(1), k, _p(box_sorted.contiguous()), _p(scores_sorted.contiguous()),
                                                         _p(keep), _p(num), float(extra_width or 0.0), _p(boxes), _p(scores), _p(count), _p(pooled),
                                                         _p(send), k * 8 + 1, _stream()), "select_proposals")
        return boxes, scores, count, pooled, send[:B, :k * 8].unflatten(1, (k, 8))
    pk = torch.empty((B, k, 8), dtype=torch.float32, device=dev) if packed else None
    with _on(dev):
        if packed:
            check(_lib.load().ws3d_select_proposals_packed(B, top, keep.size(1), k, _p(box_sorted.contiguous()), _p(scores_sorted.contiguous()),
                                                           _p(keep), _p(num), float(extra_width or 0.0), _p(boxes), _p(scores), _p(count), _p(pooled),
                                                           _p(pk), _stream()), "select_proposals")
        else:
            check(_lib.load().ws3d_select_proposals(B, top, keep.size(1), k, _p(box_sorted.contiguous()), _p(scores_sorted.contiguous()),
                                                    _p(keep), _p(num), float(extra_width or 0.0), _p(boxes), _p(scores), _p(count), _p(pooled),
                                                    _stream()), "select_proposals")
    return (boxes, scores, count, pooled, pk) if packed else (boxes, scores, count, pooled)


def bias_act_inplace(y, bias, relu=True):
    dev = _dev(y, bias)
    _f32(y, "y"); _f32(bias, "bias")
    B, O = y.size(0), y.size(1)
    L = y.numel() // max(B * O, 1)
    with _on(dev):
        check(_lib.load().ws3d_bias_act_inplace(B, O, L, int(bool(relu)), _p(y), _p(bias), _stream()), "bias_act")
    return y


def rowmax_bias_act(y, bias=None, relu=True):
    dev = _dev(y) if bias is None else _dev(y, bias)
    _f32(y, "y")
    if bias is not None:
        _f32(bias, "bias")
    B, O, M, S = y.shape
    out = torch.empty((B, O, M), dtype=torch.float32, device=dev)
    with _on(dev):
        check(_lib.load().ws3d_rowmax_bias_act(B, O, M, S, int(bool(relu)), _p(y), _p(bias) if bias is not None else None,
                                               _p(out), _stream()), "rowmax_bias_act")
    return out


def boxes_overlap_bev_gpu(boxes_a, boxes_b, ans_overlap):
    dev = _dev(boxes_a, boxes_b, ans_overlap)
    _f32(boxes_a, "boxes_a"); _f32(boxes_b, "boxes_b"); _f32(ans_overlap, "ans")
    with _on(dev):
        check(_lib.load().ws3d_boxes_overlap_bev(boxes_a.size(0), _p(boxes_a), boxes_b.size(0), _p(boxes_b),
                                                  _p(ans_overlap), _stream()), "boxes_overlap_bev")
    return 1


def boxes_iou_bev_gpu(boxes_a, boxes_b, ans_iou):
    dev = _dev(boxes_a, boxes_b, ans_iou)
    _f32(boxes_a, "boxes_a"); _f32(boxes_b, "boxes_b"); _f32(ans_iou, "ans")
    with _on(dev):
        check(_lib.load().ws3d_boxes_iou_bev(boxes_a.size(0), _p(boxes_a), boxes_b.size(0), _p(boxes_b),
                                              _p(ans_iou), _stream()), "boxes_iou_bev")
    return 1


def boxes_iou3d_paired(boxes_a, boxes_b):
    dev = _dev(boxes_a, boxes_b)
    _f32(boxes_a, "boxes_a"); _f32(boxes_b, "boxes_b")
    if boxes_a.dim() != 2 or boxes_a.size(1) != 7 or boxes_a.shape != boxes_b.shape:
        raise ValueError("boxes_iou3d_paired: boxes must both be (n,7), got %s and %s" % (tuple(boxes_a.shape), tuple(boxes_b.shape)))
    n = boxes_a.size(0)
    out = torch.empty((3, n), dtype=torch.float32, device=dev)
    if n == 0:
        return out[0], out[1], out[2]
    with _on(dev):
        check(_lib.load().ws3d_boxes_iou3d_paired(n, _p(boxes_a), _p(boxes_b), _p(out[0]), _p(out[1]), _p(out[2]), _stream()), "boxes_iou3d_paired")
    return out[0], out[1], out[2]


def nms_device(boxes, thresh, normal=False, max_keep=0):
    dev = _dev(boxes)
    _f32(boxes, "boxes")
    n = boxes.size(0)
# ... 390 lines not shown
```

### ws3d_amd/csrc/gemm_rows.hip

```cpp
#include "common.h"

namespace ws3d {

typedef float rows_f16 __attribute__((ext_vector_type(16)));
typedef __bf16 rows_bf8 __attribute__((ext_vector_type(8)));
typedef unsigned rows_u4 __attribute__((ext_vector_type(4)));
typedef float rows_f4 __attribute__((ext_vector_type(4)));

constexpr int GR_THREADS = 256;
constexpr int GR_TM = 64;
constexpr int GR_KB = 32;
constexpr int GR_FRAG = 1024;
#ifndef WS3D_GR_TALL_MIN_TILES
#define WS3D_GR_TALL_MIN_TILES 512
#endif
constexpr int GR_TALL_MIN_TILES = WS3D_GR_TALL_MIN_TILES;
constexpr int GR_MAX_DIM = 4096;
__host__ __device__ constexpr int gr_tile_rows(int nbt, int mbw) { return nbt == 4 ? 32 * mbw : 64 * mbw; }
__host__ __device__ constexpr int gr_a_stage(int tm) { return tm / 32 * 2 * 3 * GR_FRAG; }
__host__ __device__ constexpr int gr_lds_bytes(int tm) { return 2 * gr_a_stage(tm); }
static_assert(gr_lds_bytes(128) <= 64 * 1024 && gr_lds_bytes(128) * 2 <= 160 * 1024, "inside the default per-workgroup cap, two workgroups per CU");

__device__ __forceinline__ void rows_split3(float x, __bf16 &p1, __bf16 &p2, __bf16 &p3) {
    p1 = (__bf16)x;
    const float r1 = x - (float)p1;
    p2 = (__bf16)r1;
    const float r2 = r1 - (float)p2;
    p3 = (__bf16)r2;
}

__device__ __forceinline__ void rows_split8(const float *v, rows_bf8 &q1, rows_bf8 &q2, rows_bf8 &q3) {
#pragma unroll
    for (int j = 0; j < 8; ++j) {
        __bf16 p1, p2, p3;
        rows_split3(v[j], p1, p2, p3);
        q1[j] = p1; q2[j] = p2; q3[j] = p3;
    }
}

__device__ __forceinline__ float rows_relu(float y) { return y < 0.f ? 0.f : y; }

__global__ __launch_bounds__(256) void gemm_rows_pack_kernel(int K, int N, const float *__restrict__ wt, rows_u4 *__restrict__ pack) {
    const int nb_all = N / 32;
    const long total = (long)(K / GR_KB) * nb_all * 2 * 64;
    for (long i = (long)blockIdx.x * blockDim.x + threadIdx.x; i < total; i += (long)gridDim.x * blockDim.x) {
        const int lane = (int)(i & 63), s = (int)((i >> 6) & 1);
        const long f = i >> 7;
        const int nb = (int)(f % nb_all), kb = (int)(f / nb_all);
        const int col = nb * 32 + (lane & 31), k0 = kb * GR_KB + 16 * s + 8 * (lane >> 5);
        float v[8];
#pragma unroll
        for (int j = 0; j < 8; ++j) v[j] = wt[(long)(k0 + j) * N + col];
        rows_bf8 q1, q2, q3;
        rows_split8(v, q1, q2, q3);
        rows_u4 *dst = pack + ((f * 2 + s) * 3) * 64 + lane;
        dst[0] = __builtin_bit_cast(rows_u4, q1);
        dst[64] = __builtin_bit_cast(rows_u4, q2);
        dst[128] = __builtin_bit_cast(rows_u4, q3);
    }
}

template <int NBT, int MBW>
__global__ __launch_bounds__(GR_THREADS, 2) void gemm_rows_kernel(int K, int N, int ntn, const float *__restrict__ a, const rows_u4 *__restrict__ pack,
                                                                  const float *__restrict__ bias, int relu, float *__restrict__ out) {
    extern __shared__ __attribute__((aligned(16))) unsigned char smem_rows[];
    constexpr int TM = gr_tile_rows(NBT, MBW);
    constexpr int UNITS = TM / 64;
    constexpr int STAGE = gr_a_stage(TM);
    const int tid = threadIdx.x, w = tid >> 6, lane = tid & 63, r = lane & 31, h = lane >> 5;
    const int tn = (int)(blockIdx.x % (unsigned)ntn);
    const long tm = blockIdx.x / (unsigned)ntn;
    const int nb_all = N / 32, nkb = K / GR_KB;
    const int nbl = NBT == 4 ? w : (w & 1), mb0 = NBT == 4 ? 0 : (w >> 1) * MBW;

    const int srow = (lane & 7) + 8 * (lane >> 5) + 16 * w, skq = (lane >> 3) & 3;
    const rows_f4 *ap = reinterpret_cast<const rows_f4 *>(a + (tm * TM + srow) * (long)K + 8 * skq);
    const size_t a_unit = (size_t)16 * K;
    const int a_wr = ((srow >> 5) * 2 + (skq >> 1)) * 3 * GR_FRAG + ((skq & 1) * 32 + (srow & 31)) * 16;
    const rows_u4 *wp = pack + (size_t)(tn * NBT + nbl) * 6 * 64 + lane;
    const size_t w_kb = (size_t)nb_all * 6 * 64;

    rows_f16 acc[MBW];
#pragma unroll
    for (int m = 0; m < MBW; ++m)
#pragma unroll
        for (int i = 0; i < 16; ++i) acc[m][i] = 0.f;
    rows_u4 wc[6];
#pragma unroll
    for (int i = 0; i < 6; ++i) wc[i] = rows_u4{0u, 0u, 0u, 0u};

    for (int kb = -1; kb < nkb; ++kb) {
        const bool more = kb + 1 < nkb;
        rows_f4 ra[UNITS][2];
        rows_u4 wn[6];
        if (more) {
#pragma unroll
            for (int u = 0; u < UNITS; ++u) {
                ra[u][0] = ap[u * a_unit + (kb + 1) * (GR_KB / 4)];
                ra[u][1] = ap[u * a_unit + (kb + 1) * (GR_KB / 4) + 1];
            }
#pragma unroll
            for (int i = 0; i < 6; ++i) wn[i] = wp[(kb + 1) * w_kb + i * 64];
        }
        if (kb >= 0) {
            const unsigned char *buf = smem_rows + (kb & 1) * STAGE + lane * 16;
#pragma unroll
            for (int s = 0; s < 2; ++s) {
                const rows_bf8 w1 = __builtin_bit_cast(rows_bf8, wc[3 * s]), w2 = __builtin_bit_cast(rows_bf8, wc[3 * s + 1]),
                               w3 = __builtin_bit_cast(rows_bf8, wc[3 * s + 2]);
                rows_bf8 a1[MBW], a2[MBW], a3[MBW];
#pragma unroll
                for (int m = 0; m < MBW; ++m) {
                    const unsigned char *af = buf + ((mb0 + m) * 2 + s) * 3 * GR_FRAG;
                    a1[m] = *reinterpret_cast<const rows_bf8 *>(af);
                    a2[m] = *reinterpret_cast<const rows_bf8 *>(af + GR_FRAG);
                    a3[m] = *reinterpret_cast<const rows_bf8 *>(af + 2 * GR_FRAG);
                }
#pragma unroll
                for (int m = 0; m < MBW; ++m) acc[m] = __builtin_amdgcn_mfma_f32_32x32x16_bf16(w3, a1[m], acc[m], 0, 0, 0);
#pragma unroll
                for (int m = 0; m < MBW; ++m) acc[m] = __builtin_amdgcn_mfma_f32_32x32x16_bf16(w2, a2[m], acc[m], 0, 0, 0);
#pragma unroll
                for (int m = 0; m < MBW; ++m) acc[m] = __builtin_amdgcn_mfma_f32_32x32x16_bf16(w1, a3[m], acc[m], 0, 0, 0);
#pragma unroll
                for (int m = 0; m < MBW; ++m) acc[m] = __builtin_amdgcn_mfma_f32_32x32x16_bf16(w2, a1[m], acc[m], 0, 0, 0);
#pragma unroll
                for (int m = 0; m < MBW; ++m) acc[m] = __builtin_amdgcn_mfma_f32_32x32x16_bf16(w1, a2[m], acc[m], 0, 0, 0);
#pragma unroll
                for (int m = 0; m < MBW; ++m) acc[m] = __builtin_amdgcn_mfma_f32_32x32x16_bf16(w1, a1[m], acc[m], 0, 0, 0);
            }
        }
        if (more) {
            unsigned char *nxt = smem_rows + ((kb + 1) & 1) * STAGE + a_wr;
#pragma unroll
            for (int u = 0; u < UNITS; ++u) {
                const float v[8] = {ra[u][0][0], ra[u][0][1], ra[u][0][2], ra[u][0][3], ra[u][1][0], ra[u][1][1], ra[u][1][2], ra[u][1][3]};
                rows_bf8 q1, q2, q3;
                rows_split8(v, q1, q2, q3);
                *reinterpret_cast<rows_bf8 *>(nxt + u * 12 * GR_FRAG) = q1;
                *reinterpret_cast<rows_bf8 *>(nxt + u * 12 * GR_FRAG + GR_FRAG) = q2;
                *reinterpret_cast<rows_bf8 *>(nxt + u * 12 * GR_FRAG + 2 * GR_FRAG) = q3;
            }
#pragma unroll
            for (int i = 0; i < 6; ++i) wc[i] = wn[i];
        }
        __syncthreads();
    }

    const int n0 = (tn * NBT + nbl) * 32 + 4 * h;
    rows_f4 b4[4];
    if (bias) {
#pragma unroll
        for (int g = 0; g < 4; ++g) b4[g] = *reinterpret_cast<const rows_f4 *>(bias + n0 + 8 * g);
    }
#pragma unroll
    for (int m = 0; m < MBW; ++m) {
        float *orow = out + (tm * TM + (mb0 + m) * 32 + r) * (long)N + n0;
#pragma unroll
        for (int g = 0; g < 4; ++g) {
            rows_f4 y;
#pragma unroll
            for (int e = 0; e < 4; ++e) y[e] = acc[m][4 * g + e];
            if (bias) y = y + b4[g];
            if (relu) {
#pragma unroll
                for (int e = 0; e < 4; ++e) y[e] = rows_relu(y[e]);
            }
            *reinterpret_cast<rows_f4 *>(orow + 8 * g) = y;
        }
    }
}

static bool gr_dims_ok(int K, int N) { return K >= GR_KB && K <= GR_MAX_DIM && K % GR_KB == 0 && N >= 64 && N <= GR_MAX_DIM && N % 64 == 0; }

}

extern "C" size_t ws3d_gemm_rows_pack_bytes(int k_dim, int n_dim) {
    return ws3d::gr_dims_ok(k_dim, n_dim) ? (size_t)k_dim * n_dim * 6 : 0;
}

extern "C" int ws3d_gemm_rows_pack(int k_dim, int n_dim, const float *wt, void *pack, ws3d_stream_t stream) {
    using namespace ws3d;
    if (!wt || !pack || (reinterpret_cast<uintptr_t>(pack) & 15) || (reinterpret_cast<uintptr_t>(wt) & 3)) {
        set_error("ws3d_gemm_rows_pack: invalid argument");
        return WS3D_E_INVALID;
    }
    if (!gr_dims_ok(k_dim, n_dim)) {
        set_error("ws3d_gemm_rows_pack: unsupported shape K=%d N=%d (K %% 32, N %% 64, both <= %d)", k_dim, n_dim, GR_MAX_DIM);
        return WS3D_E_UNSUPPORTED;
    }
    const long threads = (long)(k_dim / GR_KB) * (n_dim / 32) * 128;
    hipLaunchKernelGGL(gemm_rows_pack_kernel, dim3((unsigned)((threads + 255) / 256)), dim3(256), 0, as_stream(stream), k_dim, n_dim, wt,
                       static_cast<rows_u4 *>(pack));
    return check_launch("ws3d_gemm_rows_pack");
}

extern "C" int ws3d_gemm_rows_split(long rows, int k_dim, int n_dim, const float *a, const void *pack, const float *bias, int relu, float *out,
                                    ws3d_stream_t stream) {
    using namespace ws3d;
    if (rows < 0 || k_dim <= 0 || n_dim <= 0 || !a || !pack || !out) {
        set_error("ws3d_gemm_rows_split: invalid argument (rows=%ld K=%d N=%d)", rows, k_dim, n_dim);
        return WS3D_E_INVALID;
    }
    const uintptr_t al = reinterpret_cast<uintptr_t>(a) | reinterpret_cast<uintptr_t>(pack) | reinterpret_cast<uintptr_t>(out) | reinterpret_cast<uintptr_t>(bias);
    const int nbt = n_dim % 128 == 0 ? 4 : 2;
    if (!gr_dims_ok(k_dim, n_dim) || rows % GR_TM || (al & 15) || (rows / GR_TM) * (n_dim / (32 * nbt)) > 0x7fffffffL) {
        set_error("ws3d_gemm_rows_split: unsupported shape or alignment (rows=%ld K=%d N=%d; rows %% 64, K %% 32, N %% 64, 16-byte pointers)", rows,
                  k_dim, n_dim);
        return WS3D_E_UNSUPPORTED;
    }
    if (rows == 0) return WS3D_OK;
    const int ntn = n_dim / (32 * nbt);
    const bool tall = nbt == 4 && rows % 128 == 0 && (rows / 128) * ntn >= GR_TALL_MIN_TILES;
    const int tm = tall ? 128 : 64;
    const unsigned grid = (unsigned)((rows / tm) * ntn);
    auto go = [&](auto kern) -> int {
        hipLaunchKernelGGL(kern, dim3(grid), dim3(GR_THREADS), (size_t)gr_lds_bytes(tm), as_stream(stream), k_dim, n_dim, ntn, a,
                           static_cast<const rows_u4 *>(pack), bias, relu ? 1 : 0, out);
        return WS3D_OK;
    };
    if (int rc = nbt == 2 ? go(gemm_rows_kernel<2, 1>) : tall ? go(gemm_rows_kernel<4, 4>) : go(gemm_rows_kernel<4, 2>)) return rc;
    return check_launch("ws3d_gemm_rows_split");
}
```

### ws3d_amd/fastpath.py

```python
from __future__ import annotations

import contextlib
import contextvars

import torch
import torch.nn as nn

from . import compat as _C
from . import nn_blocks, pn2_ops

FUSED_SA_MLP = True
SA1_FROM_LISTS = True
FUSED_GEMM_POOL = True
FUSED_INTERP_GEMM = True
NESTED_FPS = True
GEOMETRY_AHEAD = True
_AHEAD_OVERRIDE = contextvars.ContextVar("ws3d_geometry_ahead", default=None)


@contextlib.contextmanager
def geometry_ahead(on: bool):
    token = _AHEAD_OVERRIDE.set(bool(on))
    try:
        yield
    finally:
        _AHEAD_OVERRIDE.reset(token)


@contextlib.contextmanager
def compact_only_scales(keys):
    token = _COMPACT_ONLY.set(frozenset(keys))
    try:
        yield
    finally:
        _COMPACT_ONLY.reset(token)


def primed_compact_scales(net, pointcloud: torch.Tensor, margin: float = None):
    margin = PRIMED_MARGIN if margin is None else margin
    keys, per_level = set(), {}
    for row in list_fill(net, pointcloud):
        si = per_level.get(row["level"], 0)
        per_level[row["level"]] = si + 1
        if row["fill"] <= margin * COMPACT_MAX_FILL:
            keys.add((row["level"] - 1, si))
    return frozenset(keys)


def _geometry_ahead_now() -> bool:
    v = _AHEAD_OVERRIDE.get()
    return GEOMETRY_AHEAD if v is None else v
GEOMETRY_IN_CAPTURE = False
PER_POINT_L1 = True
COMPACT_MAX_FILL = 0.55
COMPACT_PAIRS = True
PAIR_DISPATCH = "device"
PRIMED_MARGIN = 0.85
_COMPACT_ONLY = contextvars.ContextVar("ws3d_compact_only_scales", default=frozenset())
CHAIN_MLP = True
PAIRED_SCALES = True
MERGED_THREE_NN = True
FUSED_PROLOGUE = True
MERGED_BINNING = True
PER_POINT_FP = True
FUSED_MLP2_ROWS = True
FUSED_HEADS = True
SPLIT_GEMMS = True
FUSED_GATHER_GEMM2 = True
BIN_INPUT_AHEAD = True
FUSED_QINTERP_GEMM_MIN_ROWS = 30000
FUSED_COMPACT3_MAX_LDS = 64 * 1024
FUSED_GATHER_GEMM = True
GRID_MIN_N = 256
DUAL_SCALE_SEARCH = True
NESTED_CHAIN = True
QUERY_CELL_ORDER = True
PARALLEL_SCALES = True
PARALLEL_HEADS = True


def _row_weights(block):
    w, shift, act = block._folded()
    if act is not None and not isinstance(act, nn.ReLU):
        raise NotImplementedError("fast path supports ReLU / no activation only")
    cache = block.__dict__.get("_row_cache")
    if cache is None or cache[0] is not w:
        cache = (w, w.t().contiguous())
        if not torch.cuda.is_current_stream_capturing():
            block.__dict__["_row_cache"] = cache
    return cache[1], shift, act is not None


def _row_weights_xyz_last(block):
    wt, bias, relu = _row_weights(block)
    cache = block.__dict__.get("_row_cache_xyz_last")
    if cache is None or cache[0] is not wt:
        cache = (wt, torch.cat((wt[3:], wt[:3]), dim=0).contiguous())
        if not torch.cuda.is_current_stream_capturing():
            block.__dict__["_row_cache_xyz_last"] = cache
    return cache[1], bias, relu


def _split_rows(block, wt: torch.Tensor, c2: int):
    cache = block.__dict__.get("_split_cache")
    if cache is None or cache[0] is not wt or cache[1] != c2:
        cache = (wt, c2, wt[:c2].contiguous(), wt[c2:].contiguous())
        if not torch.cuda.is_current_stream_capturing():
            block.__dict__["_split_cache"] = cache
    return cache[2], cache[3]


_SPLIT_GEMM_LIBRARY_WINS = frozenset({(512, 1024, 512)})


def _split_gemm_wins(rows: int, k: int, n: int) -> bool:
    return (rows, k, n) not in _SPLIT_GEMM_LIBRARY_WINS


def _split_gemm(x2d: torch.Tensor, holder, key: str, wt: torch.Tensor, bias=None, relu: bool = False):
    if not SPLIT_GEMMS or x2d.dim() != 2 or not _split_gemm_wins(x2d.size(0), wt.size(0), wt.size(1)):
        return None
    packs = holder.__dict__.get("_gemm_rows_packs")
    ent = None if packs is None else packs.get(key)
    if ent is None or ent[0] is not wt:
        if torch.cuda.is_current_stream_capturing():
            return None
        ent = (wt, _C.gemm_rows_pack(wt))
        holder.__dict__.setdefault("_gemm_rows_packs", {})[key] = ent
    if ent[1] is None:
        return None
    return _C.gemm_rows_split(x2d, ent[1], wt.size(1), bias, relu)


def gemm_rows_packs(model):
    return [ent[1] for m in model.modules() for ent in m.__dict__.get("_gemm_rows_packs", {}).values() if ent[1] is not None]


def _layer(x2d: torch.Tensor, block) -> torch.Tensor:
    wt, bias, relu = _row_weights(block)
    y = _split_gemm(x2d, block, "row", wt, bias, relu)
    if y is not None:
        return y
    if bias is None:
        y = torch.mm(x2d, wt)
        return torch.relu_(y) if relu else y
    if relu:
        return torch._addmm_activation(bias, x2d, wt, use_gelu=False)
    return torch.addmm(bias, x2d, wt)


def _blocks(seq):
    return [m for m in seq if isinstance(m, nn_blocks._ConvBlock)]


def mlp_rows(x2d: torch.Tensor, seq, ticket=None) -> torch.Tensor:
    blocks = _blocks(seq)
    if FUSED_MLP2_ROWS and len(blocks) == 2 and x2d.size(1) == 128 and x2d.is_contiguous():
        (w1, b1, r1), (w2, b2, r2) = _row_weights(blocks[0]), _row_weights(blocks[1])
        y = _C.mlp2_rows(x2d, w1, b1, r1, w2, b2, r2, ticket)
        if y is not None:
            return y
    for blk in blocks:
        x2d = _layer(x2d, blk)
    return x2d


def _heads_blob(seq):
    blocks = _blocks(seq)
    if len(blocks) != 2:
        return None
    (w1, b1, r1), (w2, b2, r2) = _row_weights(blocks[0]), _row_weights(blocks[1])
    cache = blocks[0].__dict__.get("_heads_blob")
    if cache is None or cache[0] is not w1 or cache[1] is not b1 or cache[2] is not w2 or cache[3] is not b2:
        cache = (w1, b1, w2, b2, _C.rpn_heads_pack(w1, b1, r1, w2, b2, r2), w2.size(1))
        if not torch.cuda.is_current_stream_capturing():
            blocks[0].__dict__["_heads_blob"] = cache
    return None if cache[4] is None else (cache[4], cache[5])


def heads_blobs(rpn):
    return [blk.__dict__["_heads_blob"][4] for seq in (rpn.rpn_cls_layer, rpn.rpn_reg_layer) for blk in _blocks(seq)[:1]
            if "_heads_blob" in blk.__dict__]


def _fused_heads(rows: torch.Tensor, blobs, which: int, tickets):
    if blobs is None or not all(blobs[i] is not None for i in (0, 1) if which & (1 << i)):
        return None
    (bc, oc), (br, orr) = blobs[0] or (None, 1), blobs[1] or (None, 0)
    if oc != 1 or (which & 2 and orr == 1):
        return None
    return _C.rpn_heads(rows, which, bc, br, orr, tickets, _C.tune("mlp2_wgs") * (2 if which == 3 else 1))


def supported(model) -> bool:
    try:
        for m in model.modules():
            if isinstance(m, nn_blocks._ConvBlock):
                if not m._pointwise or not isinstance(getattr(m, "activation", None), (nn.ReLU, type(None))):
                    return False
        for sa in model.rpn.backbone_net.SA_modules:
            if sa.pool_method != "max_pool" or sa.npoint is None:
                return False
            for g, mlp in zip(sa.groupers, sa.mlps):
                if not isinstance(g, pn2_ops.QueryAndGroup) or any(b.conv.out_channels % 4 for b in _blocks(mlp)):
                    return False
        return True
    except AttributeError:
        return False


def _gather_gemm_ok(sa, grouper, blocks, c_feat: int, B: int) -> bool:
    return (FUSED_GATHER_GEMM and c_feat >= 16 and c_feat % 4 == 0 and grouper.use_xyz and len(blocks) >= 2 and
            blocks[0].conv.out_channels % 64 == 0 and (B * sa.npoint * grouper.nsample) % 64 == 0 and
            (B * sa.npoint * grouper.nsample) // 64 <= 65535)


def _pair_limit(rows: int, dense_available: bool, key=None) -> int:
    if PAIR_DISPATCH != "device" or not dense_available or (key is not None and key in _COMPACT_ONLY.get()):
        return -1
    return max(0, int(COMPACT_MAX_FILL * rows))


@torch.no_grad()
def list_fill(net, pointcloud: torch.Tensor):
    xyz = pointcloud[..., 0:3].contiguous()
    rows = []
    for level, sa in enumerate(net.SA_modules):
        _, new_xyz = (pn2_ops.furthest_point_sample_gather_nested if NESTED_FPS and level >= 1 else pn2_ops.furthest_point_sample_gather)(xyz, sa.npoint)
        srt = pn2_ops.sort_points_x(xyz)
        for g in sa.groupers:
            nbr = _C.ball_query_lists(g.radius, g.nsample, xyz, new_xyz, srt)
            total = _C.compact_pairs(nbr)[2]
            rows.append({"level": level + 1, "n": xyz.size(1), "npoint": sa.npoint, "radius": float(g.radius), "nsample": g.nsample,
                         "distinct_per_list": float(total.item()) / max(nbr.numel() // g.nsample, 1),
                         "fill": float(total.item()) / max(nbr.numel(), 1)})
        xyz = new_xyz
    return rows


class _ZeroArena:

    def __init__(self, numel: int, device, clear: bool = True):
        n = (max(int(numel), 4) + 3) & ~3
        self.buf = (torch.zeros if clear else torch.empty)(n, dtype=torch.float32, device=device)
        self.dirty = not clear
        self.off = 0
        self.fallbacks = 0

    def ensure_clear(self):
        if self.dirty:
            self.buf.zero_()
            self.dirty = False

    def take(self, shape, dtype=torch.float32):
        n = 1
        for d in shape:
            n *= int(d)
        if self.off + n > self.buf.numel():
            self.fallbacks += 1
            self.fallback_shapes = getattr(self, "fallback_shapes", []) + [(tuple(shape), self.off, self.buf.numel())]
            return torch.zeros(shape, dtype=dtype, device=self.buf.device)
        v = self.buf[self.off:self.off + n]
        self.off += (n + 3) & ~3
        return (v if dtype == torch.float32 else v.view(dtype)).view(shape)


LAST_ARENA_FALLBACKS = 0


def _arena_for(net, B: int, device, extra: int = 0, clear: bool = True) -> _ZeroArena:
    n = extra + 64
    if COMPACT_PAIRS:
        for sa in net.SA_modules:
            n += B * sa.npoint * sum(_blocks(mlp)[-1].conv.out_channels for mlp in sa.mlps) + 4
            n += 4 * len(sa.groupers)
        if CHAIN_MLP:
            n += _C.chain_ticket_ints() + 4
    return _ZeroArena(n, device, clear)


class _PairList:
    __slots__ = ("nbr", "pairs")

    def __init__(self, nbr, pairs):
        self.nbr, self.pairs = nbr, pairs


def _per_point_l1(sa, feats: torch.Tensor, nbrs):
    B, N, C = feats.shape
    wts = [(_row_weights_xyz_last(_blocks(mlp)[0])[0] if nbr is not None else None) for mlp, nbr in zip(sa.mlps, nbrs)]
    cache = sa.__dict__.get("_pp_cache")
    if cache is None or len(cache[0]) != len(wts) or any(a is not b for a, b in zip(cache[0], wts)):
        used = [w for w in wts if w is not None]
        wcat = torch.cat([w[:C] for w in used], dim=1).contiguous()
        offs, w1xs, o = [], [], 0
        for w in wts:
            offs.append(o if w is not None else -1)
            w1xs.append(w[C:C + 3].contiguous() if w is not None else None)
            o += w.size(1) if w is not None else 0
        cache = (wts, wcat, offs, w1xs)
        if not torch.cuda.is_current_stream_capturing():
            sa.__dict__["_pp_cache"] = cache
    p = _split_gemm(feats.view(B * N, C), sa, "pp", cache[1])
    return (p if p is not None else torch.mm(feats.view(B * N, C), cache[1])), cache[2], cache[3]


def _lists_and_pairs(radius, nsample, xyz, new_xyz, sorted_xyz, zeros=None):
    total = zeros.take((1,), torch.int32) if zeros is not None else None
    both = _C.ball_query_pairs(radius, nsample, xyz, new_xyz, sorted_xyz, total)
    if both is not None:
        return both
    nbr = _C.ball_query_lists(radius, nsample, xyz, new_xyz, sorted_xyz)
    return nbr, _C.compact_pairs(nbr)


def _neighbour_lists(sa, xyz, new_xyz, sorted_xyz, c_feat: int, zeros=None):
    B = xyz.size(0)
    lists = []
    want_pairs = [(_gather_gemm_ok(sa, g, _blocks(mlp), c_feat, B) and COMPACT_PAIRS and PER_POINT_L1 and _blocks(mlp)[0].conv.out_channels <= 256
                   and len(_blocks(mlp)) == 3) for g, mlp in zip(sa.groupers, sa.mlps)]
    if DUAL_SCALE_SEARCH and len(want_pairs) == 2 and all(want_pairs) and sorted_xyz is not None:
        totals = [zeros.take((1,), torch.int32) for _ in range(2)] if zeros is not None else None
        both = _C.ball_query_pairs2([g.radius for g in sa.groupers], [g.nsample for g in sa.groupers], xyz, new_xyz, sorted_xyz, totals)
        if both is not None:
            return [_PairList(nbr, pairs) for nbr, pairs in both]
    for grouper, mlp in zip(sa.groupers, sa.mlps):
        if not _gather_gemm_ok(sa, grouper, _blocks(mlp), c_feat, B):
            lists.append(None)
            continue
        if COMPACT_PAIRS and PER_POINT_L1 and _blocks(mlp)[0].conv.out_channels <= 256 and len(_blocks(mlp)) == 3:
            nbr, pairs = _lists_and_pairs(grouper.radius, grouper.nsample, xyz, new_xyz, sorted_xyz, zeros)
            lists.append(_PairList(nbr, pairs))
        else:
            lists.append(_C.ball_query_lists(grouper.radius, grouper.nsample, xyz, new_xyz, sorted_xyz))
    return lists


def _side_streams(main: torch.cuda.Stream, count: int = 3, fresh: bool = False):
    from .streams import pass_streams
    return pass_streams(main, count, fresh)


class _Geometry:

    def __init__(self, net, xyz: torch.Tensor, c0: int, zeros=None):
        sas = list(net.SA_modules)
        main = torch.cuda.current_stream(xyz.device)
        s_fps, s_search, s_aux = _side_streams(main, fresh=True)
        self.aux = s_aux
        self.xyz = [xyz]
        srt0 = ev0 = None
        if BIN_INPUT_AHEAD:
            pre = torch.cuda.Event()
            pre.record(main)
        _, nx = pn2_ops.furthest_point_sample_gather(xyz, sas[0].npoint)
        if BIN_INPUT_AHEAD:
            s_search.wait_event(pre)
            with torch.cuda.stream(s_search):
                srt0 = pn2_ops.sort_points_x(xyz)
                ev0 = torch.cuda.Event()
                ev0.record(s_search)
        self.xyz.append(nx)
        start = torch.cuda.Event()
        start.record(main)
        fps_done = [start]
        s_fps.wait_event(start)
        with torch.cuda.stream(s_fps):
            if NESTED_FPS and NESTED_CHAIN and len(sas) > 1:
                for _, nx in pn2_ops.furthest_point_sample_gather_nested_chain(self.xyz[-1], [sa.npoint for sa in sas[1:]]):
                    self.xyz.append(nx)
                ev = torch.cuda.Event()
                ev.record(s_fps)
                fps_done.extend([ev] * (len(sas) - 1))
            else:
                for sa in sas[1:]:
                    _, nx = (pn2_ops.furthest_point_sample_gather_nested if NESTED_FPS else pn2_ops.furthest_point_sample_gather)(self.xyz[-1], sa.npoint)
                    self.xyz.append(nx)
                    ev = torch.cuda.Event()
                    ev.record(s_fps)
                    fps_done.append(ev)
        self.sorted, self.nbr, self.sa_ready = [srt0], [None], [ev0]
        self.nn, self.nn_ready = [], []
        c_feat = [c0] + [sum(_blocks(mlp)[-1].conv.out_channels for mlp in sa.mlps) for sa in sas]
        with torch.cuda.stream(s_search):
            for i in range(1, len(sas)):
                s_search.wait_event(fps_done[i - 1])
                srt = pn2_ops.sort_points_x(self.xyz[i], GRID_MIN_N)
                self.sorted.append(srt)
                s_search.wait_event(fps_done[i])
                self.nbr.append(_neighbour_lists(sas[i], self.xyz[i], self.xyz[i + 1], srt, c_feat[i], zeros))
                ev = torch.cuda.Event()
                ev.record(s_search)
                self.sa_ready.append(ev)
            self.nn, self.nn_ready = [None] * len(sas), [None] * len(sas)
            for i in range(len(sas) - 1, -1, -1):
                self.nn[i] = _C.three_nn_with_weights(self.xyz[i], self.xyz[i + 1], pn2_ops.sort_points_xz(self.xyz[i + 1]),
                                                      self.sorted[i] if QUERY_CELL_ORDER else None)
                ev = torch.cuda.Event()
                ev.record(s_search)
                self.nn_ready[i] = ev
        self.main, self.side = main, (s_fps, s_search, s_aux)

    def release(self):
        if torch.cuda.is_current_stream_capturing():
            return
        done = torch.cuda.Event()
        done.record(self.main)
        for s in self.side:
            s.wait_event(done)


def sa_forward(sa, xyz: torch.Tensor, feats: torch.Tensor, geo: _Geometry = None, level: int = 0, zeros: _ZeroArena = None, binned: list = None,
               new_xyz_pre: torch.Tensor = None, prebinned=None):
    B = xyz.size(0)
    c_feat = 0 if feats is None else feats.size(2)
    if geo is not None:
        new_xyz = geo.xyz[level + 1]
        if level >= 1:
            geo.main.wait_event(geo.sa_ready[level])
            sorted_xyz, nbrs = geo.sorted[level], geo.nbr[level]
        else:
            if geo.sa_ready[0] is not None:
                geo.main.wait_event(geo.sa_ready[0])
            sorted_xyz = geo.sorted[0] if geo.sa_ready[0] is not None else pn2_ops.sort_points_x(xyz)
            nbrs = _neighbour_lists(sa, xyz, new_xyz, None, c_feat, zeros)
    else:
        if new_xyz_pre is not None:
            new_xyz = new_xyz_pre
        else:
            _, new_xyz = (pn2_ops.furthest_point_sample_gather_nested if NESTED_FPS and level >= 1 else pn2_ops.furthest_point_sample_gather)(xyz, sa.npoint)
        sorted_xyz = prebinned[0] if prebinned is not None else pn2_ops.sort_points_x(xyz, GRID_MIN_N)
        nbrs = _neighbour_lists(sa, xyz, new_xyz, sorted_xyz, c_feat, zeros)
    if binned is not None:
        binned.append(sorted_xyz)
    widths = [_blocks(mlp)[-1].conv.out_channels for mlp in sa.mlps]
    if not COMPACT_PAIRS:
        out = torch.empty((B * sa.npoint, sum(widths)), dtype=torch.float32, device=xyz.device)
    elif zeros is not None:
        out = zeros.take((B * sa.npoint, sum(widths)))
    else:
        out = torch.zeros((B * sa.npoint, sum(widths)), dtype=torch.float32, device=xyz.device)
    cols = [sum(widths[:i]) for i in range(len(widths))]
    pp = [None]
    sa1_pairs = {}
    if (DUAL_SCALE_SEARCH and COMPACT_PAIRS and FUSED_SA_MLP and SA1_FROM_LISTS and len(widths) == 2 and feats is not None and feats.size(2) == 1
            and sorted_xyz is not None and all(n_ is None for n_ in nbrs) and all(g_.use_xyz and len(_blocks(m_)) == 3 for g_, m_ in zip(sa.groupers, sa.mlps))):
        totals = [zeros.take((1,), torch.int32) for _ in range(2)] if zeros is not None else None
        both = _C.ball_query_pairs2([g_.radius for g_ in sa.groupers], [g_.nsample for g_ in sa.groupers], xyz, new_xyz, sorted_xyz, totals)
        if both is not None:
            sa1_pairs = dict(enumerate(both))

    def run_scale(si: int) -> None:
        grouper, mlp, width, nbr, col = sa.groupers[si], sa.mlps[si], widths[si], nbrs[si], cols[si]
        blocks = _blocks(mlp)
        pairs = None
        if isinstance(nbr, _PairList):
            nbr, pairs = nbr.nbr, nbr.pairs
        if nbr is not None:
            wt1, b1, r1 = _row_weights_xyz_last(blocks[0])
            if PER_POINT_L1 and len(blocks) >= 3:
                if pp[0] is None:
                    pp[0] = _per_point_l1(sa, feats, nbrs)
                pmat, offs, w1xs = pp[0]
                o1 = blocks[0].conv.out_channels
                y = None
                wt3, b3, r3 = _row_weights(blocks[-1])
                if pairs is not None and o1 <= 256 and len(blocks) == 3 and r3:
                    wt2, b2, r2 = _row_weights(blocks[1])
                    rows, ns, o3 = nbr.numel(), grouper.nsample, wt3.size(1)
                    dense_ok = (o1 in (64, 128) and (sa.npoint * ns) % 64 == 0 and rows // 64 <= 65535 and o3 % 64 == 0 and
                                wt2.size(1) % 4 == 0 and ns in (16, 32))
                    limit = _pair_limit(rows, dense_ok, (level, si))
                    fused = _C.pgather_gemm3_compact(pmat, offs[si], o1, xyz, new_xyz, pairs, w1xs[si], b1, r1, wt2, b2, r2, wt3, b3, out, col,
                                                     limit=limit, max_lds=FUSED_COMPACT3_MAX_LDS)
                    yc = None if fused else _C.pgather_gemm2_compact(pmat, offs[si], o1, xyz, new_xyz, pairs, w1xs[si], b1, r1, wt2, b2, r2, limit=limit)
                    if fused or (yc is not None and _C.gemm_pool_compact(yc, pairs, wt3, b3, out, col, limit=limit)):
                        if limit >= 0:
                            gate = (pairs[2], limit)
                            yd = _C.pgather_gemm2(pmat, offs[si], o1, xyz, new_xyz, nbr, w1xs[si], b1, r1, wt2, b2, r2, out=yc, gate=gate)
                            if yd is None or not _C.gemm_pool(yd, wt3, b3, r3, ns, out, col, gate=gate):
                                yc = _C.pgather_gemm2_compact(pmat, offs[si], o1, xyz, new_xyz, pairs, w1xs[si], b1, r1, wt2, b2, r2, limit=-1)
                                if yc is None or not _C.gemm_pool_compact(yc, pairs, wt3, b3, out, col, limit=-1):
                                    raise RuntimeError("neither the gated dense nor the ungated compact kernels took the shape")
                        return
                if o1 <= 128:
                    wt2, b2, r2 = _row_weights(blocks[1])
                    y = _C.pgather_gemm2(pmat, offs[si], o1, xyz, new_xyz, nbr, w1xs[si], b1, r1, wt2, b2, r2)
                    rest_pp = blocks[2:-1]
                if y is None:
                    y = _C.pgather_rows(pmat, offs[si], o1, xyz, new_xyz, nbr, w1xs[si], b1, r1)
                    rest_pp = blocks[1:-1]
                if y is not None:
                    for blk in rest_pp:
                        y = _layer(y, blk)
                    wt, bias, relu = _row_weights(blocks[-1])
                    if not (FUSED_GEMM_POOL and _C.gemm_pool(y, wt, bias, relu, grouper.nsample, out, col)):
                        _C.rowmax_rows(_layer(y, blocks[-1]), grouper.nsample, out, col)
                    return
            y = None
            rest = blocks[1:-1]
            if FUSED_GATHER_GEMM2 and len(blocks) >= 3 and blocks[0].conv.out_channels <= 128:
                wt2, b2, r2 = _row_weights(blocks[1])
                y = _C.gather_gemm2(feats, xyz, new_xyz, nbr, wt1, b1, r1, wt2, b2, r2)
                if y is not None:
                    rest = blocks[2:-1]
            if y is None:
                y = _C.gather_gemm(feats, xyz, new_xyz, nbr, wt1, b1, r1)
            if y is not None:
                for blk in rest:
                    y = _layer(y, blk)
                wt, bias, relu = _row_weights(blocks[-1])
                if not (FUSED_GEMM_POOL and _C.gemm_pool(y, wt, bias, relu, grouper.nsample, out, col)):
                    _C.rowmax_rows(_layer(y, blocks[-1]), grouper.nsample, out, col)
                return
        if FUSED_SA_MLP and SA1_FROM_LISTS and feats is not None and feats.size(2) == 1 and grouper.use_xyz and len(blocks) == 3:
            layers = [_row_weights(b) for b in blocks]
            if not COMPACT_PAIRS:
                nbr1 = _C.ball_query_lists(grouper.radius, grouper.nsample, xyz, new_xyz, sorted_xyz)
                if _C.sa_mlp3_pool_lists(xyz, new_xyz, feats, nbr1, layers, out, col):
                    return
            else:
                nbr1, pairs1 = sa1_pairs[si] if si in sa1_pairs else _lists_and_pairs(grouper.radius, grouper.nsample, xyz, new_xyz, sorted_xyz, zeros)
                limit = _pair_limit(nbr1.numel(), layers[2][2] and nbr1.numel() % 32 == 0 and grouper.nsample in (16, 32), (level, si))
                if _C.sa_mlp3_pool_compact(xyz, new_xyz, feats, pairs1, layers, out, col, limit=limit):
                    if limit >= 0 and not _C.sa_mlp3_pool_lists(xyz, new_xyz, feats, nbr1, layers, out, col, gate=(pairs1[2], limit)):
                        if not _C.sa_mlp3_pool_compact(xyz, new_xyz, feats, pairs1, layers, out, col, limit=-1):
                            raise RuntimeError("neither ws3d_sa_mlp3_pool_lists nor the ungated compact kernel took the shape")
                    return
        g = _C.query_and_group_nlc(grouper.radius, grouper.nsample, xyz, new_xyz, feats, grouper.use_xyz, sorted_xyz)
        rows = g.view(-1, g.size(3))
        if not (FUSED_SA_MLP and rows.size(1) == 4 and len(blocks) == 3 and
                _C.sa_mlp3_pool(rows, grouper.nsample, [_row_weights(b) for b in blocks], out, col)):
            y = rows
            for blk in blocks[:-1]:
                y = _layer(y, blk)
            wt, bias, relu = _row_weights(blocks[-1])
            if not (FUSED_GEMM_POOL and _C.gemm_pool(y, wt, bias, relu, grouper.nsample, out, col)):
                _C.rowmax_rows(_layer(y, blocks[-1]), grouper.nsample, out, col)

    def run_paired() -> bool:
        if not (PAIRED_SCALES and COMPACT_PAIRS and PER_POINT_L1 and len(widths) == 2 and all(isinstance(n_, _PairList) for n_ in nbrs)):
            return False
        blk = [_blocks(m_) for m_ in sa.mlps]
        if any(len(b_) != 3 or b_[0].conv.out_channels > 256 for b_ in blk) or blk[0][0].conv.out_channels != blk[1][0].conv.out_channels:
            return False
        if any(_pair_limit(n_.nbr.numel(), True, (level, si_)) != -1 for si_, n_ in enumerate(nbrs)):
            return False
        if pp[0] is None:
            pp[0] = _per_point_l1(sa, feats, nbrs)
        pmat, offs, w1xs = pp[0]
        scales = []
        for si_ in range(2):
            _w1, b1, r1 = _row_weights_xyz_last(blk[si_][0])
            wt2, b2, r2 = _row_weights(blk[si_][1])
            wt3, b3, r3 = _row_weights(blk[si_][2])
            if not r3:
                return False
            scales.append({"pmat": pmat, "col0": offs[si_], "o1": blk[si_][0].conv.out_channels, "xyz": xyz, "new_xyz": new_xyz, "pairs": nbrs[si_].pairs,
                           "w1x": w1xs[si_], "b1": b1, "relu1": r1, "w2t": wt2, "b2": b2, "relu2": r2, "w3t": wt3, "b3": b3, "out2d": out, "col_offset": cols[si_]})
        if (CHAIN_MLP and zeros is not None and all(sc_["o1"] == 64 and sc_["w2t"].size(1) <= 96 and sc_["w3t"].size(1) == 128 for sc_ in scales)
                and _C.chain_mlp3(scales, zeros.take((_C.chain_ticket_ints(),), torch.int32))):
            return True
        if _C.compact_mlp_pair(3, scales, max_lds=FUSED_COMPACT3_MAX_LDS):
            return True
        mids = _C.compact_mlp_pair(2, scales)
        if mids is None:
            return False
        if not _C.compact_mlp_pair(1, scales, mids=mids):
            for sc_, mid in zip(scales, mids):
                if not _C.gemm_pool_compact(mid, sc_["pairs"], sc_["w3t"], sc_["b3"], out, sc_["col_offset"], limit=-1):
                    raise RuntimeError("ws3d_gemm_pool_compact declined a shape ws3d_pgather_gemm2_compact took")
        return True

    if run_paired():
        pass
    elif geo is not None and geo.aux is not None and PARALLEL_SCALES and len(widths) == 2:
        if PER_POINT_L1 and any(n is not None and len(_blocks(m)) >= 3 for n, m in zip(nbrs, sa.mlps)):
            pp[0] = _per_point_l1(sa, feats, nbrs)
        fork = torch.cuda.Event()
        fork.record(geo.main)
        geo.aux.wait_event(fork)
        with torch.cuda.stream(geo.aux):
            run_scale(1)
            join = torch.cuda.Event()
            join.record(geo.aux)
        run_scale(0)
        geo.main.wait_event(join)
    else:
        for si in range(len(widths)):
            run_scale(si)
    return new_xyz, out.view(B, sa.npoint, -1)


def fp_forward(fp, unknown: torch.Tensor, known: torch.Tensor, unknown_feats, known_feats: torch.Tensor, nn3=None, sorted_unknown=None,
               known_xz=None):
    B, n = unknown.size(0), unknown.size(1)
    idx, weight = nn3 if nn3 is not None else _C.three_nn_with_weights(unknown, known, known_xz[0] if known_xz is not None else pn2_ops.sort_points_xz(known),
                                                                        sorted_unknown if QUERY_CELL_ORDER else None)
    c2 = known_feats.size(2)
    c1 = 0 if unknown_feats is None else unknown_feats.size(2)
    blocks = _blocks(fp.mlp)
    if PER_POINT_FP and blocks and blocks[0].conv.out_channels % 4 == 0:
        wt1, b1, r1 = _row_weights(blocks[0])
        wa, wb = _split_rows(blocks[0], wt1, c2)
        m = known_feats.size(1)
        q = _split_gemm(known_feats.reshape(B * m, c2), blocks[0], "wa", wa)
        q = (q if q is not None else torch.mm(known_feats.reshape(B * m, c2), wa)).view(B, m, -1)
        fuse2 = len(blocks) == 2 and B * n >= FUSED_QINTERP_GEMM_MIN_ROWS
        if fuse2:
            wt2, b2, r2 = _row_weights(blocks[1])
        if c1 > 4:
            lin = _split_gemm(unknown_feats.reshape(B * n, c1), blocks[0], "wb", wb, b1)
            if lin is None:
                lin = torch.mm(unknown_feats.reshape(B * n, c1), wb) if b1 is None else torch.addmm(b1, unknown_feats.reshape(B * n, c1), wb)
            y = _C.qinterp_gemm(q, idx, weight, wt2, b2, r2, lin=lin, relu=r1) if fuse2 else None
            if y is not None:
                return y.view(B, n, -1)
            y = _C.qinterp_rows(q, idx, weight, lin=lin, relu=r1)
        else:
            sk = None if c1 == 0 else unknown_feats.contiguous()
            y = _C.qinterp_gemm(q, idx, weight, wt2, b2, r2, skip=sk, wb=wb if c1 else None, bias=b1, relu=r1) if fuse2 else None
            if y is not None:
                return y.view(B, n, -1)
            y = _C.qinterp_rows(q, idx, weight, skip=sk, wb=wb if c1 else None, bias=b1, relu=r1)
        if y is not None:
            for blk in blocks[1:]:
                y = _layer(y, blk)
            return y.view(B, n, -1)
    if FUSED_INTERP_GEMM and blocks and blocks[0].conv.out_channels % 64 == 0 and B * n >= 8192:
        wt1, b1, r1 = _row_weights(blocks[0])
        y = _C.interp_gemm(known_feats.contiguous(), None if unknown_feats is None else unknown_feats.contiguous(), idx, weight, wt1, b1, r1)
        if y is not None:
            for blk in blocks[1:]:
                y = _layer(y, blk)
            return y.view(B, n, -1)
    cat = torch.empty((B, n, c2 + c1), dtype=torch.float32, device=unknown.device)
    _C.three_interpolate_nlc(known_feats, idx, weight, cat)
    if c1:
        cat[:, :, c2:] = unknown_feats
    return mlp_rows(cat.view(B * n, c2 + c1), fp.mlp).view(B, n, -1)


@torch.no_grad()
def backbone_forward(net, pointcloud: torch.Tensor, zeros: _ZeroArena = None):
    if FUSED_PROLOGUE and pointcloud.is_cuda and pointcloud.dim() == 3 and pointcloud.is_contiguous() and pointcloud.size(-1) > 3:
        if zeros is None:
            zeros = _arena_for(net, pointcloud.size(0), pointcloud.device, clear=False)
        xyz, feats = _C.split_points_clear(pointcloud, zeros.buf if zeros.dirty else None)
        zeros.dirty = False
    else:
        xyz = pointcloud[..., 0:3].contiguous()
        feats = pointcloud[..., 3:].contiguous() if pointcloud.size(-1) > 3 else None
        if zeros is None:
            zeros = _arena_for(net, xyz.size(0), xyz.device)
        zeros.ensure_clear()
    ahead = _geometry_ahead_now() and (GEOMETRY_IN_CAPTURE or not torch.cuda.is_current_stream_capturing())
    geo = _Geometry(net, xyz, 0 if feats is None else feats.size(2), zeros) if ahead else None
    l_xyz, l_feats, binned = [xyz], [feats], []
    try:
        sas, chain, pre_grid, pre_xz, nn_pre = list(net.SA_modules), None, {}, {}, {}
        for level, sa in enumerate(sas):
            pre = chain[level - 1][1] if (chain is not None and level >= 1) else None
            nx, nf = sa_forward(sa, l_xyz[-1], l_feats[-1], geo, level, zeros, binned, pre, pre_grid.get(level))
            l_xyz.append(nx)
            l_feats.append(nf)
            if geo is None and level == 0 and NESTED_FPS and NESTED_CHAIN and len(sas) > 1:
                chain = pn2_ops.furthest_point_sample_gather_nested_chain(nx, [s_.npoint for s_ in sas[1:]])
                if MERGED_BINNING:
                    lv = [nx] + [c[1] for c in chain]
                    jobs = [(x_, "grid") for x_ in lv[:-1] if x_.size(1) >= GRID_MIN_N] + [(x_, "xz") for x_ in lv if x_.size(1) >= 256]
                    bufs = iter(_C.sort_points_jobs(jobs) if _C.BQ_FINE_GRID else [])
                    if _C.BQ_FINE_GRID:
                        pre_grid = {k + 1: ((next(bufs),) if x_.size(1) >= GRID_MIN_N else (None,)) for k, x_ in enumerate(lv[:-1])}
                        pre_xz = {k + 1: (next(bufs) if x_.size(1) >= 256 else None) for k, x_ in enumerate(lv)}
                        if MERGED_THREE_NN:
                            allx = [l_xyz[0]] + lv
                            qgrid = {0: binned[0]}
                            qgrid.update({k_: v_[0] for k_, v_ in pre_grid.items()})
                            lvls = [k_ for k_ in range(len(sas)) if pre_xz.get(k_ + 1) is not None and allx[k_ + 1].size(1) <= 4096]
                            got = _C.three_nn_jobs([(allx[k_], allx[k_ + 1], pre_xz[k_ + 1], qgrid.get(k_) if QUERY_CELL_ORDER else None) for k_ in lvls])
                            if got is not None:
                                nn_pre = dict(zip(lvls, got))
        for i in range(-1, -(len(net.FP_modules) + 1), -1):
            lvl = len(l_xyz) + i - 1
            nn3 = nn_pre.get(lvl)
            if geo is not None:
                geo.main.wait_event(geo.nn_ready[lvl])
                nn3 = geo.nn[lvl]
            known_level = len(l_xyz) + i
            l_feats[i - 1] = fp_forward(net.FP_modules[i], l_xyz[i - 1], l_xyz[i], l_feats[i - 1], l_feats[i], nn3, binned[len(l_xyz) + i - 1],
                                        (pre_xz[known_level],) if known_level in pre_xz else None)
    finally:
        if geo is not None:
            geo.release()
    return l_xyz[0], l_feats[0]


@torch.no_grad()
def rpn_forward(model, pts_input: torch.Tensor, defer_reg_join: bool = False) -> dict:
    rpn = model.rpn
    zeros = _arena_for(rpn.backbone_net, pts_input.size(0), pts_input.device, extra=8, clear=not FUSED_PROLOGUE)
    xyz, feats = backbone_forward(rpn.backbone_net, pts_input, zeros)
    B, N, C = feats.shape
    rows = feats.view(B * N, C)
    tickets = zeros.take((2,), torch.int32) if (FUSED_MLP2_ROWS or FUSED_HEADS) else (None, None)
    blobs = (_heads_blob(rpn.rpn_cls_layer), _heads_blob(rpn.rpn_reg_layer)) if FUSED_HEADS else None
    reg_ready = None
    if PARALLEL_HEADS and _geometry_ahead_now() and not torch.cuda.is_current_stream_capturing():
        main = torch.cuda.current_stream(rows.device)
        aux = _side_streams(main)[2]
        fork = torch.cuda.Event()
        fork.record(main)
        aux.wait_event(fork)
        with torch.cuda.stream(aux):
            fused = _fused_heads(rows, blobs, 2, tickets)
            rpn_reg = (fused[1] if fused is not None else mlp_rows(rows, rpn.rpn_reg_layer, tickets[1:2])).view(B, N, -1)
            reg_ready = torch.cuda.Event()
            reg_ready.record(aux)
        rpn_reg.record_stream(main)
        fused = _fused_heads(rows, blobs, 1, tickets)
        rpn_cls = (fused[0] if fused is not None else mlp_rows(rows, rpn.rpn_cls_layer, tickets[0:1])).view(B, N, -1)
        if not defer_reg_join:
            main.wait_event(reg_ready)
            reg_ready = None
    else:
        fused = _fused_heads(rows, blobs, 3, tickets)
        if fused is not None:
            rpn_cls, rpn_reg = fused[0].view(B, N, -1), fused[1].view(B, N, -1)
        else:
            rpn_cls = mlp_rows(rows, rpn.rpn_cls_layer, tickets[0:1]).view(B, N, -1)
            rpn_reg = mlp_rows(rows, rpn.rpn_reg_layer, tickets[1:2]).view(B, N, -1)
    global LAST_ARENA_FALLBACKS
    LAST_ARENA_FALLBACKS = zeros.fallbacks if not zeros.fallbacks else getattr(zeros, "fallback_shapes", zeros.fallbacks)
    out = {"rpn_cls": rpn_cls, "rpn_reg": rpn_reg, "backbone_xyz": xyz,
           "backbone_features": feats.transpose(1, 2),
           "backbone_features_nlc": feats}
    if reg_ready is not None:
        out["rpn_reg_ready"] = reg_ready
    return out
```

Measured before the change: 7045.

## Share input rows between SA per-point GEMM and FP skip GEMM in one launch

Adds a paired split-bf16 row GEMM kernel that computes two GEMMs over the same input rows in one launch. It is used to produce both the SA level's per-point layer-1 projection and the later FP module's skip-branch linear term from the same features. This saves a second read and bf16 split of the activations plus one kernel launch. The FP result is computed early and held until the FP stage, which lengthens its lifetime in memory. It also adds a tunable tile-variant knob and moves the GEMM helpers into a shared header with new 64x128/128x128 and deep-pipelined variants.

Result: no change. 7139 (median of 3 runs) (+1.3%).

```diff
diff --git a/include/ws3d_ops.h b/include/ws3d_ops.h
--- a/include/ws3d_ops.h
+++ b/include/ws3d_ops.h
@@ -228,6 +228,8 @@
 WS3D_API int ws3d_gemm_rows_pack(int k_dim, int n_dim, const float *wt, void *pack, ws3d_stream_t stream);
 WS3D_API int ws3d_gemm_rows_split(long rows, int k_dim, int n_dim, const float *a, const void *pack, const float *bias, int relu, float *out,
                          ws3d_stream_t stream);
+WS3D_API int ws3d_gemm_rows_split_pair(long rows, int k_dim, const float *a, const void *pack1, int n1, const float *bias1, int relu1, float *out1,
+                              const void *pack2, int n2, const float *bias2, int relu2, float *out2, ws3d_stream_t stream);
 
 WS3D_API int ws3d_qinterp_gemm(int b, int n, int m, int c, int o_dim, const float *q, const int32_t *idx, const float *weight, const float *lin,
                       const float *skip, int c1, const float *wb, const float *b1, int relu1, const float *w2t, const float *b2, int relu2,
diff --git a/ws3d_amd/_lib.py b/ws3d_amd/_lib.py
--- a/ws3d_amd/_lib.py
+++ b/ws3d_amd/_lib.py
@@ -73,6 +73,7 @@
     "ws3d_gemm_rows_pack_bytes": (_sz, [_i, _i]),
     "ws3d_gemm_rows_pack": (_i, [_i, _i, _vp, _vp, _vp]),
     "ws3d_gemm_rows_split": (_i, [C.c_long, _i, _i, _vp, _vp, _vp, _i, _vp, _vp]),
+    "ws3d_gemm_rows_split_pair": (_i, [C.c_long, _i, _vp, _vp, _i, _vp, _i, _vp, _vp, _i, _vp, _i, _vp, _vp]),
     "ws3d_decode_center_boxes": (_i, [_i, _i, _i, _f, _f, _f, _f, _f, _vp, _vp, _vp, _vp]),
     "ws3d_topk_sorted": (_i, [_i, _i, _i, _vp, _vp, _vp, _vp]),
     "ws3d_topk_workspace_bytes": (C.c_size_t, [_i, _i]),
diff --git a/ws3d_amd/build.py b/ws3d_amd/build.py
--- a/ws3d_amd/build.py
+++ b/ws3d_amd/build.py
@@ -18,7 +18,7 @@
 def lib_path(dist_mode: int = 0) -> str:
     return LIB if dist_mode == 0 else os.path.join(HERE, "libws3d_hip_dm%d.so" % dist_mode)
 ARCH = "gfx950"
-SOURCES = ["core.hip", "fps.hip", "fps_v3.hip", "fps_bucket.hip", "fps_nested.hip", "ballquery_group.hip", "interpolate.hip", "roipool3d.hip", "iou3d.hip", "proposals.hip", "scatter_det.hip", "sa_mlp.hip", "bn_relu.hip", "gemm_pool.hip", "conv_wgrad.hip", "chain_mlp.hip", "rpn_heads.hip", "gemm_rows.hip", "kitti_eval.hip", "instance_clouds.hip", "click.hip", "stage2.hip", "stage2_loss.hip"]
+SOURCES = ["core.hip", "fps.hip", "fps_v3.hip", "fps_bucket.hip", "fps_nested.hip", "ballquery_group.hip", "interpolate.hip", "roipool3d.hip", "iou3d.hip", "proposals.hip", "scatter_det.hip", "sa_mlp.hip", "bn_relu.hip", "gemm_pool.hip", "conv_wgrad.hip", "chain_mlp.hip", "rpn_heads.hip", "gemm_rows.hip", "gemm_rows_wide.hip", "kitti_eval.hip", "instance_clouds.hip", "click.hip", "stage2.hip", "stage2_loss.hip"]
 CXXFLAGS = ["-O3", "-std=c++17", "-fPIC", "-ffp-contract=off", "-fno-fast-math",
             "-fvisibility=hidden", "-Wall", "-Wno-unused-function"]
 
diff --git a/ws3d_amd/compat.py b/ws3d_amd/compat.py
--- a/ws3d_amd/compat.py
+++ b/ws3d_amd/compat.py
@@ -671,7 +671,8 @@
 
 
 CHAIN_WORKGROUPS = 0
-TUNE_KEYS = {"chain_wgs": 0, "mlp2_wgs": 1, "sa1_wgs": 2, "fp_wgs": 3, "pair_wgs": 4, "bq_wide_nw": 5}
+GEMM_ROWS_TILES = {"64x64": 1, "64x128": 2, "128x128": 3, "64x128_deep": 4, "128x128_deep": 5}
+TUNE_KEYS = {"chain_wgs": 0, "mlp2_wgs": 1, "sa1_wgs": 2, "fp_wgs": 3, "pair_wgs": 4, "bq_wide_nw": 5, "gemm_rows_tile": 6}
 
 
 def tune(name: str, value: int = -1) -> int:
@@ -845,6 +846,38 @@
         return None
     check(rc, "gemm_rows_split")
     return out
+
+
+def gemm_rows_split_pair(x2d, pack1, n1, pack2, n2, bias1=None, relu1=False, bias2=None, relu2=False, out1=None, out2=None):
+    if pack1 is None or pack2 is None or x2d.dim() != 2 or not x2d.is_contiguous():
+        return None
+    for b_, n_ in ((bias1, n1), (bias2, n2)):
+        if b_ is not None and (not b_.is_contiguous() or b_.numel() != n_):
+            return None
+    dev = _dev(x2d, pack1, pack2, bias1, bias2, out1, out2)
+    _f32(x2d, "x2d")
+    R, K = x2d.shape
+    n1, n2 = int(n1), int(n2)
+    if R % 64 or K % 32 or n1 % 128 or n2 % 128 or n1 <= 0 or n2 <= 0:
+        return None
+    if pack1.numel() * pack1.element_size() < K * n1 * 6 or pack2.numel() * pack2.element_size() < K * n2 * 6:
+        return None
+    outs = []
+    for o_, n_, b_ in ((out1, n1, bias1), (out2, n2, bias2)):
+        if b_ is not None:
+            _f32(b_, "bias")
+        if o_ is None:
+            o_ = torch.empty((R, n_), dtype=torch.float32, device=dev)
+        elif tuple(o_.shape) != (R, n_) or o_.dtype != torch.float32 or not o_.is_contiguous():
+            return None
+        outs.append(o_)
+    with _on(dev):
+        rc = _lib.load().ws3d_gemm_rows_split_pair(R, K, _p(x2d), _p(pack1), n1, _p(bias1), int(bool(relu1)), _p(outs[0]),
+                                                   _p(pack2), n2, _p(bias2), int(bool(relu2)), _p(outs[1]), _stream())
+    if rc == _lib.E_UNSUPPORTED:
+        return None
+    check(rc, "gemm_rows_split_pair")
+    return outs[0], outs[1]
 
 
 def pool_nsample(x):
diff --git a/ws3d_amd/csrc/gemm_rows.h b/ws3d_amd/csrc/gemm_rows.h
--- /dev/null
+++ b/ws3d_amd/csrc/gemm_rows.h
@@ -0,0 +1,229 @@
+#pragma once
+#include "common.h"
+
+namespace ws3d {
+
+typedef float rows_f16 __attribute__((ext_vector_type(16)));
+typedef __bf16 rows_bf8 __attribute__((ext_vector_type(8)));
+typedef unsigned rows_u4 __attribute__((ext_vector_type(4)));
+typedef float rows_f4 __attribute__((ext_vector_type(4)));
+
+constexpr int GR_THREADS = 256;
+constexpr int GR_TM = 64;
+constexpr int GR_KB = 32;
+constexpr int GR_FRAG = 1024;
+#ifndef WS3D_GR_TALL_MIN_TILES
+#define WS3D_GR_TALL_MIN_TILES 512
+#endif
+constexpr int GR_TALL_MIN_TILES = WS3D_GR_TALL_MIN_TILES;
+constexpr int GR_MAX_DIM = 4096;
+__host__ __device__ constexpr int gr_tile_rows(int nbt, int mbw) { return nbt == 4 ? 32 * mbw : 64 * mbw; }
+__host__ __device__ constexpr int gr_a_stage(int tm) { return tm / 32 * 2 * 3 * GR_FRAG; }
+__host__ __device__ constexpr int gr_lds_bytes(int tm) { return 2 * gr_a_stage(tm); }
+static_assert(gr_lds_bytes(128) <= 64 * 1024 && gr_lds_bytes(128) * 2 <= 160 * 1024, "inside the default per-workgroup cap, two workgroups per CU");
+
+enum : int {
+    GR_V_RULE = 0,
+    GR_V_64x64 = 1,
+    GR_V_64x128 = 2,
+    GR_V_128x128 = 3,
+    GR_V_64x128_DEEP = 4,
+    GR_V_128x128_DEEP = 5,
+    GR_V_COUNT = 6
+};
+constexpr int TUNE_GR_TILE = 6;
+static_assert(TUNE_GR_TILE < TUNE_COUNT, "ws3d_tune key");
+
+static inline bool gr_dims_ok(int K, int N) { return K >= GR_KB && K <= GR_MAX_DIM && K % GR_KB == 0 && N >= 64 && N <= GR_MAX_DIM && N % 64 == 0; }
+
+constexpr int GR_SMALL_MAX_TILES = 128;
+static inline int gr_pick_variant(long rows, bool n128, long ntn) {
+    if (!n128) return GR_V_64x64;
+    const bool can_tall = rows % 128 == 0;
+    const int v = g_tune[TUNE_GR_TILE];
+    if (v == GR_V_64x64 || v == GR_V_64x128 || v == GR_V_64x128_DEEP) return v;
+    if ((v == GR_V_128x128 || v == GR_V_128x128_DEEP) && can_tall) return v;
+    if (can_tall && (rows / 128) * ntn >= GR_TALL_MIN_TILES) return GR_V_128x128;
+    return (rows / 64) * ntn < GR_SMALL_MAX_TILES ? GR_V_64x64 : GR_V_64x128;
+}
+
+int gr_launch_deep(int variant, unsigned grid, int k_dim, int n_dim, int ntn, const float *a, const rows_u4 *pack, const float *bias, int relu,
+                   float *out, hipStream_t stream);
+
+#ifdef __HIPCC__
+__device__ __forceinline__ void rows_split3(float x, __bf16 &p1, __bf16 &p2, __bf16 &p3) {
+    p1 = (__bf16)x;
+    const float r1 = x - (float)p1;
+    p2 = (__bf16)r1;
+    const float r2 = r1 - (float)p2;
+    p3 = (__bf16)r2;
+}
+
+__device__ __forceinline__ void rows_split8(const float *v, rows_bf8 &q1, rows_bf8 &q2, rows_bf8 &q3) {
+#pragma unroll
+    for (int j = 0; j < 8; ++j) {
+        __bf16 p1, p2, p3;
+        rows_split3(v[j], p1, p2, p3);
+        q1[j] = p1; q2[j] = p2; q3[j] = p3;
+    }
+}
+
+__device__ __forceinline__ float rows_relu(float y) { return y < 0.f ? 0.f : y; }
+
+template <int MBW>
+__device__ __forceinline__ void rows_mfma_block(const unsigned char *buf, int mb0, const rows_u4 (&wc)[6], rows_f16 (&acc)[MBW]) {
+#pragma unroll
+    for (int s = 0; s < 2; ++s) {
+        const rows_bf8 w1 = __builtin_bit_cast(rows_bf8, wc[3 * s]), w2 = __builtin_bit_cast(rows_bf8, wc[3 * s + 1]),
+                       w3 = __builtin_bit_cast(rows_bf8, wc[3 * s + 2]);
+        rows_bf8 a1[MBW], a2[MBW], a3[MBW];
+#pragma unroll
+        for (int m = 0; m < MBW; ++m) {
+            const unsigned char *af = buf + ((mb0 + m) * 2 + s) * 3 * GR_FRAG;
+            a1[m] = *reinterpret_cast<const rows_bf8 *>(af);
+            a2[m] = *reinterpret_cast<const rows_bf8 *>(af + GR_FRAG);
+            a3[m] = *reinterpret_cast<const rows_bf8 *>(af + 2 * GR_FRAG);
+        }
+#pragma unroll
+        for (int m = 0; m < MBW; ++m) acc[m] = __builtin_amdgcn_mfma_f32_32x32x16_bf16(w3, a1[m], acc[m], 0, 0, 0);
+#pragma unroll
+        for (int m = 0; m < MBW; ++m) acc[m] = __builtin_amdgcn_mfma_f32_32x32x16_bf16(w2, a2[m], acc[m], 0, 0, 0);
+#pragma unroll
+        for (int m = 0; m < MBW; ++m) acc[m] = __builtin_amdgcn_mfma_f32_32x32x16_bf16(w1, a3[m], acc[m], 0, 0, 0);
+#pragma unroll
+        for (int m = 0; m < MBW; ++m) acc[m] = __builtin_amdgcn_mfma_f32_32x32x16_bf16(w2, a1[m], acc[m], 0, 0, 0);
+#pragma unroll
+        for (int m = 0; m < MBW; ++m) acc[m] = __builtin_amdgcn_mfma_f32_32x32x16_bf16(w1, a2[m], acc[m], 0, 0, 0);
+#pragma unroll
+        for (int m = 0; m < MBW; ++m) acc[m] = __builtin_amdgcn_mfma_f32_32x32x16_bf16(w1, a1[m], acc[m], 0, 0, 0);
+    }
+}
+
+template <int UNITS>
+__device__ __forceinline__ void rows_stage_block(unsigned char *nxt, const rows_f4 (&ra)[UNITS][2]) {
+#pragma unroll
+    for (int u = 0; u < UNITS; ++u) {
+        const float v[8] = {ra[u][0][0], ra[u][0][1], ra[u][0][2], ra[u][0][3], ra[u][1][0], ra[u][1][1], ra[u][1][2], ra[u][1][3]};
+        rows_bf8 q1, q2, q3;
+        rows_split8(v, q1, q2, q3);
+        *reinterpret_cast<rows_bf8 *>(nxt + u * 12 * GR_FRAG) = q1;
+        *reinterpret_cast<rows_bf8 *>(nxt + u * 12 * GR_FRAG + GR_FRAG) = q2;
+        *reinterpret_cast<rows_bf8 *>(nxt + u * 12 * GR_FRAG + 2 * GR_FRAG) = q3;
+    }
+}
+
+template <int NBT, int MBW, bool DEEP>
+__device__ __forceinline__ void rows_tile(unsigned char *smem_rows, int K, int N, int tn, long tm, const float *__restrict__ a,
+                                          const rows_u4 *__restrict__ pack, const float *__restrict__ bias, int relu, float *__restrict__ out) {
+    constexpr int TM = gr_tile_rows(NBT, MBW);
+    constexpr int UNITS = TM / 64;
+    constexpr int STAGE = gr_a_stage(TM);
+    const int tid = threadIdx.x, w = tid >> 6, lane = tid & 63, r = lane & 31, h = lane >> 5;
+    const int nb_all = N / 32, nkb = K / GR_KB;
+    const int nbl = NBT == 4 ? w : (w & 1), mb0 = NBT == 4 ? 0 : (w >> 1) * MBW;
+
+    const int srow = (lane & 7) + 8 * (lane >> 5) + 16 * w, skq = (lane >> 3) & 3;
+    const rows_f4 *ap = reinterpret_cast<const rows_f4 *>(a + (tm * TM + srow) * (long)K + 8 * skq);
+    const size_t a_unit = (size_t)16 * K;
+    const int a_wr = ((srow >> 5) * 2 + (skq >> 1)) * 3 * GR_FRAG + ((skq & 1) * 32 + (srow & 31)) * 16;
+    const rows_u4 *wp = pack + (size_t)(tn * NBT + nbl) * 6 * 64 + lane;
+    const size_t w_kb = (size_t)nb_all * 6 * 64;
+
+    rows_f16 acc[MBW];
+#pragma unroll
+    for (int m = 0; m < MBW; ++m)
+#pragma unroll
+        for (int i = 0; i < 16; ++i) acc[m][i] = 0.f;
+    rows_u4 wc[6];
+#pragma unroll
+    for (int i = 0; i < 6; ++i) wc[i] = rows_u4{0u, 0u, 0u, 0u};
+
+    if constexpr (!DEEP) {
+        for (int kb = -1; kb < nkb; ++kb) {
+            const bool more = kb + 1 < nkb;
+            rows_f4 ra[UNITS][2];
+            rows_u4 wn[6];
+            if (more) {
+#pragma unroll
+                for (int u = 0; u < UNITS; ++u) {
+                    ra[u][0] = ap[u * a_unit + (kb + 1) * (GR_KB / 4)];
+                    ra[u][1] = ap[u * a_unit + (kb + 1) * (GR_KB / 4) + 1];
+                }
+#pragma unroll
+                for (int i = 0; i < 6; ++i) wn[i] = wp[(kb + 1) * w_kb + i * 64];
+            }
+            if (kb >= 0) rows_mfma_block<MBW>(smem_rows + (kb & 1) * STAGE + lane * 16, mb0, wc, acc);
+            if (more) {
+                rows_stage_block<UNITS>(smem_rows + ((kb + 1) & 1) * STAGE + a_wr, ra);
+#pragma unroll
+                for (int i = 0; i < 6; ++i) wc[i] = wn[i];
+            }
+            __syncthreads();
+        }
+    } else {
+        rows_f4 ra0[UNITS][2], ra1[UNITS][2];
+        rows_u4 wn0[6], wn1[6];
+        auto fetch = [&](int kb, rows_f4 (&xa)[UNITS][2], rows_u4 (&xw)[6]) __attribute__((always_inline)) {
+            const int kf = kb < nkb ? kb : nkb - 1;
+#pragma unroll
+            for (int u = 0; u < UNITS; ++u) {
+                xa[u][0] = ap[u * a_unit + kf * (GR_KB / 4)];
+                xa[u][1] = ap[u * a_unit + kf * (GR_KB / 4) + 1];
+            }
+#pragma unroll
+            for (int i = 0; i < 6; ++i) xw[i] = wp[kf * w_kb + i * 64];
+        };
+        auto stage = [&](int kb, const rows_f4 (&xa)[UNITS][2], const rows_u4 (&xw)[6]) __attribute__((always_inline)) {
+            rows_stage_block<UNITS>(smem_rows + (kb & 1) * STAGE + a_wr, xa);
+#pragma unroll
+            for (int i = 0; i < 6; ++i) wc[i] = xw[i];
+            lds_barrier();
+        };
+        auto step = [&](int kb, rows_f4 (&la)[UNITS][2], rows_u4 (&lw)[6], const rows_f4 (&sa)[UNITS][2], const rows_u4 (&sw)[6]) __attribute__((always_inline)) {
+            fetch(kb + 2, la, lw);
+            __builtin_amdgcn_sched_barrier(0);
+            rows_mfma_block<MBW>(smem_rows + (kb & 1) * STAGE + lane * 16, mb0, wc, acc);
+            __builtin_amdgcn_sched_barrier(0);
+            stage(kb + 1, sa, sw);
+        };
+        fetch(0, ra0, wn0);
+        fetch(1, ra1, wn1);
+        stage(0, ra0, wn0);
+        int kb = 0;
+        for (; kb + 2 < nkb; kb += 2) {
+            step(kb, ra0, wn0, ra1, wn1);
+            step(kb + 1, ra1, wn1, ra0, wn0);
+        }
+        if (kb + 1 < nkb) {
+            step(kb, ra0, wn0, ra1, wn1);
+            ++kb;
+        }
+        rows_mfma_block<MBW>(smem_rows + (kb & 1) * STAGE + lane * 16, mb0, wc, acc);
+    }
+
+    const int n0 = (tn * NBT + nbl) * 32 + 4 * h;
+    rows_f4 b4[4];
+    if (bias) {
+#pragma unroll
+        for (int g = 0; g < 4; ++g) b4[g] = *reinterpret_cast<const rows_f4 *>(bias + n0 + 8 * g);
+    }
+#pragma unroll
+    for (int m = 0; m < MBW; ++m) {
+        float *orow = out + (tm * TM + (mb0 + m) * 32 + r) * (long)N + n0;
+#pragma unroll
+        for (int g = 0; g < 4; ++g) {
+            rows_f4 y;
+#pragma unroll
+            for (int e = 0; e < 4; ++e) y[e] = acc[m][4 * g + e];
+            if (bias) y = y + b4[g];
+            if (relu) {
+#pragma unroll
+                for (int e = 0; e < 4; ++e) y[e] = rows_relu(y[e]);
+            }
+            *reinterpret_cast<rows_f4 *>(orow + 8 * g) = y;
+        }
+    }
+}
+#endif
+
+}
diff --git a/ws3d_amd/csrc/gemm_rows.hip b/ws3d_amd/csrc/gemm_rows.hip
--- a/ws3d_amd/csrc/gemm_rows.hip
+++ b/ws3d_amd/csrc/gemm_rows.hip
@@ -1,44 +1,6 @@
-#include "common.h"
+#include "gemm_rows.h"
 
 namespace ws3d {
-
-typedef float rows_f16 __attribute__((ext_vector_type(16)));
-typedef __bf16 rows_bf8 __attribute__((ext_vector_type(8)));
-typedef unsigned rows_u4 __attribute__((ext_vector_type(4)));
-typedef float rows_f4 __attribute__((ext_vector_type(4)));
-
-constexpr int GR_THREADS = 256;
-constexpr int GR_TM = 64;
-constexpr int GR_KB = 32;
-constexpr int GR_FRAG = 1024;
-#ifndef WS3D_GR_TALL_MIN_TILES
-#define WS3D_GR_TALL_MIN_TILES 512
-#endif
-constexpr int GR_TALL_MIN_TILES = WS3D_GR_TALL_MIN_TILES;
-constexpr int GR_MAX_DIM = 4096;
-__host__ __device__ constexpr int gr_tile_rows(int nbt, int mbw) { return nbt == 4 ? 32 * mbw : 64 * mbw; }
-__host__ __device__ constexpr int gr_a_stage(int tm) { return tm / 32 * 2 * 3 * GR_FRAG; }
-__host__ __device__ constexpr int gr_lds_bytes(int tm) { return 2 * gr_a_stage(tm); }
-static_assert(gr_lds_bytes(128) <= 64 * 1024 && gr_lds_bytes(128) * 2 <= 160 * 1024, "inside the default per-workgroup cap, two workgroups per CU");
-
-__device__ __forceinline__ void rows_split3(float x, __bf16 &p1, __bf16 &p2, __bf16 &p3) {
-    p1 = (__bf16)x;
-    const float r1 = x - (float)p1;
-    p2 = (__bf16)r1;
-    const float r2 = r1 - (float)p2;
-    p3 = (__bf16)r2;
-}
-
-__device__ __forceinline__ void rows_split8(const float *v, rows_bf8 &q1, rows_bf8 &q2, rows_bf8 &q3) {
-#pragma unroll
-    for (int j = 0; j < 8; ++j) {
-        __bf16 p1, p2, p3;
-        rows_split3(v[j], p1, p2, p3);
-        q1[j] = p1; q2[j] = p2; q3[j] = p3;
-    }
-}
-
-__device__ __forceinline__ float rows_relu(float y) { return y < 0.f ? 0.f : y; }
 
 __global__ __launch_bounds__(256) void gemm_rows_pack_kernel(int K, int N, const float *__restrict__ wt, rows_u4 *__restrict__ pack) {
     const int nb_all = N / 32;
@@ -64,114 +26,10 @@
 __global__ __launch_bounds__(GR_THREADS, 2) void gemm_rows_kernel(int K, int N, int ntn, const float *__restrict__ a, const rows_u4 *__restrict__ pack,
                                                                   const float *__restrict__ bias, int relu, float *__restrict__ out) {
     extern __shared__ __attribute__((aligned(16))) unsigned char smem_rows[];
-    constexpr int TM = gr_tile_rows(NBT, MBW);
-    constexpr int UNITS = TM / 64;
-    constexpr int STAGE = gr_a_stage(TM);
-    const int tid = threadIdx.x, w = tid >> 6, lane = tid & 63, r = lane & 31, h = lane >> 5;
     const int tn = (int)(blockIdx.x % (unsigned)ntn);
     const long tm = blockIdx.x / (unsigned)ntn;
-    const int nb_all = N / 32, nkb = K / GR_KB;
-    const int nbl = NBT == 4 ? w : (w & 1), mb0 = NBT == 4 ? 0 : (w >> 1) * MBW;
-
-    const int srow = (lane & 7) + 8 * (lane >> 5) + 16 * w, skq = (lane >> 3) & 3;
-    const rows_f4 *ap = reinterpret_cast<const rows_f4 *>(a + (tm * TM + srow) * (long)K + 8 * skq);
-    const size_t a_unit = (size_t)16 * K;
-    const int a_wr = ((srow >> 5) * 2 + (skq >> 1)) * 3 * GR_FRAG + ((skq & 1) * 32 + (srow & 31)) * 16;
-    const rows_u4 *wp = pack + (size_t)(tn * NBT + nbl) * 6 * 64 + lane;
-    const size_t w_kb = (size_t)nb_all * 6 * 64;
-
-    rows_f16 acc[MBW];
-#pragma unroll
-    for (int m = 0; m < MBW; ++m)
-#pragma unroll
-        for (int i = 0; i < 16; ++i) acc[m][i] = 0.f;
-    rows_u4 wc[6];
-#pragma unroll
-    for (int i = 0; i < 6; ++i) wc[i] = rows_u4{0u, 0u, 0u, 0u};
-
-    for (int kb = -1; kb < nkb; ++kb) {
-        const bool more = kb + 1 < nkb;
-        rows_f4 ra[UNITS][2];
-        rows_u4 wn[6];
-        if (more) {
-#pragma unroll
-            for (int u = 0; u < UNITS; ++u) {
-                ra[u][0] = ap[u * a_unit + (kb + 1) * (GR_KB / 4)];
-                ra[u][1] = ap[u * a_unit + (kb + 1) * (GR_KB / 4) + 1];
-            }
-#pragma unroll
-            for (int i = 0; i < 6; ++i) wn[i] = wp[(kb + 1) * w_kb + i * 64];
-        }
-        if (kb >= 0) {
-            const unsigned char *buf = smem_rows + (kb & 1) * STAGE + lane * 16;
-#pragma unroll
-            for (int s = 0; s < 2; ++s) {
-                const rows_bf8 w1 = __builtin_bit_cast(rows_bf8, wc[3 * s]), w2 = __builtin_bit_cast(rows_bf8, wc[3 * s + 1]),
-                               w3 = __builtin_bit_cast(rows_bf8, wc[3 * s + 2]);
-                rows_bf8 a1[MBW], a2[MBW], a3[MBW];
-#pragma unroll
-                for (int m = 0; m < MBW; ++m) {
-                    const unsigned char *af = buf + ((mb0 + m) * 2 + s) * 3 * GR_FRAG;
-                    a1[m] = *reinterpret_cast<const rows_bf8 *>(af);
-                    a2[m] = *reinterpret_cast<const rows_bf8 *>(af + GR_FRAG);
-                    a3[m] = *reinterpret_cast<const rows_bf8 *>(af + 2 * GR_FRAG);
-                }
-#pragma unroll
-                for (int m = 0; m < MBW; ++m) acc[m] = __builtin_amdgcn_mfma_f32_32x32x16_bf16(w3, a1[m], acc[m], 0, 0, 0);
-#pragma unroll
-                for (int m = 0; m < MBW; ++m) acc[m] = __builtin_amdgcn_mfma_f32_32x32x16_bf16(w2, a2[m], acc[m], 0, 0, 0);
-#pragma unroll
-                for (int m = 0; m < MBW; ++m) acc[m] = __builtin_amdgcn_mfma_f32_32x32x16_bf16(w1, a3[m], acc[m], 0, 0, 0);
-#pragma unroll
-                for (int m = 0; m < MBW; ++m) acc[m] = __builtin_amdgcn_mfma_f32_32x32x16_bf16(w2, a1[m], acc[m], 0, 0, 0);
-#pragma unroll
-                for (int m = 0; m < MBW; ++m) acc[m] = __builtin_amdgcn_mfma_f32_32x32x16_bf16(w1, a2[m], acc[m], 0, 0, 0);
-#pragma unroll
-                for (int m = 0; m < MBW; ++m) acc[m] = __builtin_amdgcn_mfma_f32_32x32x16_bf16(w1, a1[m], acc[m], 0, 0, 0);
-            }
-        }
-        if (more) {
-            unsigned char *nxt = smem_rows + ((kb + 1) & 1) * STAGE + a_wr;
-#pragma unroll
-            for (int u = 0; u < UNITS; ++u) {
-                const float v[8] = {ra[u][0][0], ra[u][0][1], ra[u][0][2], ra[u][0][3], ra[u][1][0], ra[u][1][1], ra[u][1][2], ra[u][1][3]};
-                rows_bf8 q1, q2, q3;
-                rows_split8(v, q1, q2, q3);
-                *reinterpret_cast<rows_bf8 *>(nxt + u * 12 * GR_FRAG) = q1;
-                *reinterpret_cast<rows_bf8 *>(nxt + u * 12 * GR_FRAG + GR_FRAG) = q2;
-                *reinterpret_cast<rows_bf8 *>(nxt + u * 12 * GR_FRAG + 2 * GR_FRAG) = q3;
-            }
-#pragma unroll
-            for (int i = 0; i < 6; ++i) wc[i] = wn[i];
-        }
-        __syncthreads();
-    }
-
-    const int n0 = (tn * NBT + nbl) * 32 + 4 * h;
-    rows_f4 b4[4];
-    if (bias) {
-#pragma unroll
-        for (int g = 0; g < 4; ++g) b4[g] = *reinterpret_cast<const rows_f4 *>(bias + n0 + 8 * g);
-    }
-#pragma unroll
-    for (int m = 0; m < MBW; ++m) {
-        float *orow = out + (tm * TM + (mb0 + m) * 32 + r) * (long)N + n0;
-#pragma unroll
-        for (int g = 0; g < 4; ++g) {
-            rows_f4 y;
-#pragma unroll
-            for (int e = 0; e < 4; ++e) y[e] = acc[m][4 * g + e];
-            if (bias) y = y + b4[g];
-            if (relu) {
-#pragma unroll
-                for (int e = 0; e < 4; ++e) y[e] = rows_relu(y[e]);
-            }
-            *reinterpret_cast<rows_f4 *>(orow + 8 * g) = y;
-        }
-    }
+    rows_tile<NBT, MBW, false>(smem_rows, K, N, tn, tm, a, pack, bias, relu, out);
 }
-
-static bool gr_dims_ok(int K, int N) { return K >= GR_KB && K <= GR_MAX_DIM && K % GR_KB == 0 && N >= 64 && N <= GR_MAX_DIM && N % 64 == 0; }
 
 }
 
@@ -211,14 +69,22 @@
     }
     if (rows == 0) return WS3D_OK;
     const int ntn = n_dim / (32 * nbt);
-    const bool tall = nbt == 4 && rows % 128 == 0 && (rows / 128) * ntn >= GR_TALL_MIN_TILES;
-    const int tm = tall ? 128 : 64;
+    int variant = gr_pick_variant(rows, nbt == 4, ntn);
+    if (variant == GR_V_64x64 && (rows / 64) * (n_dim / 64) > 0x7fffffffL) variant = GR_V_64x128;
+    if (variant == GR_V_64x64) {
+        const int ntn64 = n_dim / 64;
+        hipLaunchKernelGGL((gemm_rows_kernel<2, 1>), dim3((unsigned)((rows / 64) * ntn64)), dim3(GR_THREADS), (size_t)gr_lds_bytes(64), as_stream(stream),
+                           k_dim, n_dim, ntn64, a, static_cast<const rows_u4 *>(pack), bias, relu ? 1 : 0, out);
+        return check_launch("ws3d_gemm_rows_split");
+    }
+    const int tm = variant == GR_V_128x128 || variant == GR_V_128x128_DEEP ? 128 : 64;
     const unsigned grid = (unsigned)((rows / tm) * ntn);
-    auto go = [&](auto kern) -> int {
+    if (variant == GR_V_64x128_DEEP || variant == GR_V_128x128_DEEP)
+        return gr_launch_deep(variant, grid, k_dim, n_dim, ntn, a, static_cast<const rows_u4 *>(pack), bias, relu ? 1 : 0, out, as_stream(stream));
+    auto go = [&](auto kern) {
         hipLaunchKernelGGL(kern, dim3(grid), dim3(GR_THREADS), (size_t)gr_lds_bytes(tm), as_stream(stream), k_dim, n_dim, ntn, a,
                            static_cast<const rows_u4 *>(pack), bias, relu ? 1 : 0, out);
-        return WS3D_OK;
     };
-    if (int rc = nbt == 2 ? go(gemm_rows_kernel<2, 1>) : tall ? go(gemm_rows_kernel<4, 4>) : go(gemm_rows_kernel<4, 2>)) return rc;
+    if (tm == 128) go(gemm_rows_kernel<4, 4>); else go(gemm_rows_kernel<4, 2>);
     return check_launch("ws3d_gemm_rows_split");
 }
diff --git a/ws3d_amd/csrc/gemm_rows_wide.hip b/ws3d_amd/csrc/gemm_rows_wide.hip
--- /dev/null
+++ b/ws3d_amd/csrc/gemm_rows_wide.hip
@@ -0,0 +1,74 @@
+#include "gemm_rows.h"
+
+namespace ws3d {
+
+struct RowsHalf {
+    const rows_u4 *pack;
+    const float *bias;
+    float *out;
+    int n, relu;
+};
+
+template <int NBT, int MBW, bool DEEP>
+__global__ __launch_bounds__(GR_THREADS, 2) void rows_pair_tiles(int K, int ntn1, int ntn, const float *__restrict__ a, RowsHalf h1, RowsHalf h2) {
+    extern __shared__ __attribute__((aligned(16))) unsigned char smem_rows[];
+    const int t = (int)(blockIdx.x % (unsigned)ntn);
+    const long tm = blockIdx.x / (unsigned)ntn;
+    const bool second = t >= ntn1;
+    const RowsHalf h = second ? h2 : h1;
+    rows_tile<NBT, MBW, DEEP>(smem_rows, K, h.n, second ? t - ntn1 : t, tm, a, h.pack, h.bias, h.relu, h.out);
+}
+
+template <int MBW>
+__global__ __launch_bounds__(GR_THREADS, 2) void rows_deep_tiles(int K, int N, int ntn, const float *__restrict__ a, const rows_u4 *__restrict__ pack,
+                                                                 const float *__restrict__ bias, int relu, float *__restrict__ out) {
+    extern __shared__ __attribute__((aligned(16))) unsigned char smem_rows[];
+    const int tn = (int)(blockIdx.x % (unsigned)ntn);
+    const long tm = blockIdx.x / (unsigned)ntn;
+    rows_tile<4, MBW, true>(smem_rows, K, N, tn, tm, a, pack, bias, relu, out);
+}
+
+int gr_launch_deep(int variant, unsigned grid, int k_dim, int n_dim, int ntn, const float *a, const rows_u4 *pack, const float *bias, int relu,
+                   float *out, hipStream_t stream) {
+    if (variant == GR_V_128x128_DEEP)
+        hipLaunchKernelGGL(rows_deep_tiles<4>, dim3(grid), dim3(GR_THREADS), (size_t)gr_lds_bytes(128), stream, k_dim, n_dim, ntn, a, pack, bias, relu, out);
+    else
+        hipLaunchKernelGGL(rows_deep_tiles<2>, dim3(grid), dim3(GR_THREADS), (size_t)gr_lds_bytes(64), stream, k_dim, n_dim, ntn, a, pack, bias, relu, out);
+    return check_launch("ws3d_gemm_rows_split");
+}
+
+}
+
+extern "C" int ws3d_gemm_rows_split_pair(long rows, int k_dim, const float *a, const void *pack1, int n1, const float *bias1, int relu1, float *out1,
+                                         const void *pack2, int n2, const float *bias2, int relu2, float *out2, ws3d_stream_t stream) {
+    using namespace ws3d;
+    if (rows < 0 || k_dim <= 0 || n1 <= 0 || n2 <= 0 || !a || !pack1 || !pack2 || !out1 || !out2) {
+        set_error("ws3d_gemm_rows_split_pair: invalid argument (rows=%ld K=%d N=%d, %d)", rows, k_dim, n1, n2);
+        return WS3D_E_INVALID;
+    }
+    const uintptr_t al = reinterpret_cast<uintptr_t>(a) | reinterpret_cast<uintptr_t>(pack1) | reinterpret_cast<uintptr_t>(pack2) |
+                         reinterpret_cast<uintptr_t>(out1) | reinterpret_cast<uintptr_t>(out2) | reinterpret_cast<uintptr_t>(bias1) |
+                         reinterpret_cast<uintptr_t>(bias2);
+    if (!gr_dims_ok(k_dim, n1) || !gr_dims_ok(k_dim, n2) || n1 % 128 || n2 % 128 || rows % GR_TM || (al & 15) ||
+        (rows / GR_TM) * ((n1 + n2) / 64) > 0x7fffffffL) {
+        set_error("ws3d_gemm_rows_split_pair: unsupported shape or alignment (rows=%ld K=%d N=%d, %d; rows %% 64, K %% 32, N %% 128, 16-byte pointers)",
+                  rows, k_dim, n1, n2);
+        return WS3D_E_UNSUPPORTED;
+    }
+    if (rows == 0) return WS3D_OK;
+    const RowsHalf h1{static_cast<const rows_u4 *>(pack1), bias1, out1, n1, relu1 ? 1 : 0}, h2{static_cast<const rows_u4 *>(pack2), bias2, out2, n2, relu2 ? 1 : 0};
+    const int variant = gr_pick_variant(rows, true, (n1 + n2) / 128);
+    const int cols = variant == GR_V_64x64 ? 64 : 128, tm = variant == GR_V_128x128 || variant == GR_V_128x128_DEEP ? 128 : 64;
+    const int ntn1 = n1 / cols, ntn = (n1 + n2) / cols;
+    auto go = [&](auto kern) {
+        hipLaunchKernelGGL(kern, dim3((unsigned)((rows / tm) * ntn)), dim3(GR_THREADS), (size_t)gr_lds_bytes(tm), as_stream(stream), k_dim, ntn1, ntn, a, h1, h2);
+    };
+    switch (variant) {
+        case GR_V_64x64: go(rows_pair_tiles<2, 1, false>); break;
+        case GR_V_128x128: go(rows_pair_tiles<4, 4, false>); break;
+        case GR_V_64x128_DEEP: go(rows_pair_tiles<4, 2, true>); break;
+        case GR_V_128x128_DEEP: go(rows_pair_tiles<4, 4, true>); break;
+        default: go(rows_pair_tiles<4, 2, false>); break;
+    }
+    return check_launch("ws3d_gemm_rows_split_pair");
+}
diff --git a/ws3d_amd/fastpath.py b/ws3d_amd/fastpath.py
--- a/ws3d_amd/fastpath.py
+++ b/ws3d_amd/fastpath.py
@@ -66,6 +66,7 @@
 FUSED_MLP2_ROWS = True
 FUSED_HEADS = True
 SPLIT_GEMMS = True
+SHARED_A_GEMMS = True
 FUSED_GATHER_GEMM2 = True
 BIN_INPUT_AHEAD = True
 FUSED_QINTERP_GEMM_MIN_ROWS = 30000
@@ -120,6 +121,13 @@
 def _split_gemm(x2d: torch.Tensor, holder, key: str, wt: torch.Tensor, bias=None, relu: bool = False):
     if not SPLIT_GEMMS or x2d.dim() != 2 or not _split_gemm_wins(x2d.size(0), wt.size(0), wt.size(1)):
         return None
+    pack = _split_pack(holder, key, wt)
+    if pack is None:
+        return None
+    return _C.gemm_rows_split(x2d, pack, wt.size(1), bias, relu)
+
+
+def _split_pack(holder, key: str, wt: torch.Tensor):
     packs = holder.__dict__.get("_gemm_rows_packs")
     ent = None if packs is None else packs.get(key)
     if ent is None or ent[0] is not wt:
@@ -127,9 +135,21 @@
             return None
         ent = (wt, _C.gemm_rows_pack(wt))
         holder.__dict__.setdefault("_gemm_rows_packs", {})[key] = ent
-    if ent[1] is None:
+    return ent[1]
+
+
+PAIR_LAUNCHES = 0
+
+
+def _fp_lin_weights(fp, c1: int):
+    blocks = _blocks(fp.mlp)
+    if not (PER_POINT_FP and blocks and blocks[0].conv.out_channels % 4 == 0 and c1 > 4):
         return None
-    return _C.gemm_rows_split(x2d, ent[1], wt.size(1), bias, relu)
+    wt1, b1, _r1 = _row_weights(blocks[0])
+    if wt1.size(0) <= c1:
+        return None
+    _wa, wb = _split_rows(blocks[0], wt1, wt1.size(0) - c1)
+    return blocks[0], wb, b1
 
 
 def gemm_rows_packs(model):
@@ -286,7 +306,7 @@
         self.nbr, self.pairs = nbr, pairs
 
 
-def _per_point_l1(sa, feats: torch.Tensor, nbrs):
+def _per_point_l1(sa, feats: torch.Tensor, nbrs, lin_for=None):
     B, N, C = feats.shape
     wts = [(_row_weights_xyz_last(_blocks(mlp)[0])[0] if nbr is not None else None) for mlp, nbr in zip(sa.mlps, nbrs)]
     cache = sa.__dict__.get("_pp_cache")
@@ -301,8 +321,20 @@
         cache = (wts, wcat, offs, w1xs)
         if not torch.cuda.is_current_stream_capturing():
             sa.__dict__["_pp_cache"] = cache
-    p = _split_gemm(feats.view(B * N, C), sa, "pp", cache[1])
-    return (p if p is not None else torch.mm(feats.view(B * N, C), cache[1])), cache[2], cache[3]
+    x2d = feats.view(B * N, C)
+    if lin_for is not None and SHARED_A_GEMMS and SPLIT_GEMMS and feats.is_contiguous():
+        got = _fp_lin_weights(lin_for["fp"], C)
+        if got is not None and _split_gemm_wins(B * N, C, cache[1].size(1)) and _split_gemm_wins(B * N, C, got[1].size(1)):
+            blk, wb, b1 = got
+            pack_p, pack_l = _split_pack(sa, "pp", cache[1]), _split_pack(blk, "wb", wb)
+            both = _C.gemm_rows_split_pair(x2d, pack_p, cache[1].size(1), pack_l, wb.size(1), bias2=b1)
+            if both is not None:
+                global PAIR_LAUNCHES
+                PAIR_LAUNCHES += 1
+                lin_for["lin"] = both[1]
+                return both[0], cache[2], cache[3]
+    p = _split_gemm(x2d, sa, "pp", cache[1])
+    return (p if p is not None else torch.mm(x2d, cache[1])), cache[2], cache[3]
 
 
 def _lists_and_pairs(radius, nsample, xyz, new_xyz, sorted_xyz, zeros=None):
@@ -411,7 +443,7 @@
 
 
 def sa_forward(sa, xyz: torch.Tensor, feats: torch.Tensor, geo: _Geometry = None, level: int = 0, zeros: _ZeroArena = None, binned: list = None,
-               new_xyz_pre: torch.Tensor = None, prebinned=None):
+               new_xyz_pre: torch.Tensor = None, prebinned=None, lin_for: dict = None):
     B = xyz.size(0)
     c_feat = 0 if feats is None else feats.size(2)
     if geo is not None:
@@ -460,7 +492,7 @@
             wt1, b1, r1 = _row_weights_xyz_last(blocks[0])
             if PER_POINT_L1 and len(blocks) >= 3:
                 if pp[0] is None:
-                    pp[0] = _per_point_l1(sa, feats, nbrs)
+                    pp[0] = _per_point_l1(sa, feats, nbrs, lin_for)
                 pmat, offs, w1xs = pp[0]
                 o1 = blocks[0].conv.out_channels
                 y = None
@@ -547,7 +579,7 @@
         if any(_pair_limit(n_.nbr.numel(), True, (level, si_)) != -1 for si_, n_ in enumerate(nbrs)):
             return False
         if pp[0] is None:
-            pp[0] = _per_point_l1(sa, feats, nbrs)
+            pp[0] = _per_point_l1(sa, feats, nbrs, lin_for)
         pmat, offs, w1xs = pp[0]
         scales = []
         for si_ in range(2):
@@ -576,7 +608,7 @@
         pass
     elif geo is not None and geo.aux is not None and PARALLEL_SCALES and len(widths) == 2:
         if PER_POINT_L1 and any(n is not None and len(_blocks(m)) >= 3 for n, m in zip(nbrs, sa.mlps)):
-            pp[0] = _per_point_l1(sa, feats, nbrs)
+            pp[0] = _per_point_l1(sa, feats, nbrs, lin_for)
         fork = torch.cuda.Event()
         fork.record(geo.main)
         geo.aux.wait_event(fork)
@@ -593,7 +625,7 @@
 
 
 def fp_forward(fp, unknown: torch.Tensor, known: torch.Tensor, unknown_feats, known_feats: torch.Tensor, nn3=None, sorted_unknown=None,
-               known_xz=None):
+               known_xz=None, lin=None):
     B, n = unknown.size(0), unknown.size(1)
     idx, weight = nn3 if nn3 is not None else _C.three_nn_with_weights(unknown, known, known_xz[0] if known_xz is not None else pn2_ops.sort_points_xz(known),
                                                                         sorted_unknown if QUERY_CELL_ORDER else None)
@@ -610,7 +642,8 @@
         if fuse2:
             wt2, b2, r2 = _row_weights(blocks[1])
         if c1 > 4:
-            lin = _split_gemm(unknown_feats.reshape(B * n, c1), blocks[0], "wb", wb, b1)
+            if lin is None:
+                lin = _split_gemm(unknown_feats.reshape(B * n, c1), blocks[0], "wb", wb, b1)
             if lin is None:
                 lin = torch.mm(unknown_feats.reshape(B * n, c1), wb) if b1 is None else torch.addmm(b1, unknown_feats.reshape(B * n, c1), wb)
             y = _C.qinterp_gemm(q, idx, weight, wt2, b2, r2, lin=lin, relu=r1) if fuse2 else None
@@ -658,10 +691,13 @@
     geo = _Geometry(net, xyz, 0 if feats is None else feats.size(2), zeros) if ahead else None
     l_xyz, l_feats, binned = [xyz], [feats], []
     try:
-        sas, chain, pre_grid, pre_xz, nn_pre = list(net.SA_modules), None, {}, {}, {}
+        sas, chain, pre_grid, pre_xz, nn_pre, lins = list(net.SA_modules), None, {}, {}, {}, {}
         for level, sa in enumerate(sas):
             pre = chain[level - 1][1] if (chain is not None and level >= 1) else None
-            nx, nf = sa_forward(sa, l_xyz[-1], l_feats[-1], geo, level, zeros, binned, pre, pre_grid.get(level))
+            share = {"fp": net.FP_modules[level]} if SHARED_A_GEMMS and PER_POINT_FP and level >= 1 and len(net.FP_modules) == len(sas) else None
+            nx, nf = sa_forward(sa, l_xyz[-1], l_feats[-1], geo, level, zeros, binned, pre, pre_grid.get(level), share)
+            if share is not None and share.get("lin") is not None:
+                lins[level] = share["lin"]
             l_xyz.append(nx)
             l_feats.append(nf)
             if geo is None and level == 0 and NESTED_FPS and NESTED_CHAIN and len(sas) > 1:
@@ -689,7 +725,7 @@
                 nn3 = geo.nn[lvl]
             known_level = len(l_xyz) + i
             l_feats[i - 1] = fp_forward(net.FP_modules[i], l_xyz[i - 1], l_xyz[i], l_feats[i - 1], l_feats[i], nn3, binned[len(l_xyz) + i - 1],
-                                        (pre_xz[known_level],) if known_level in pre_xz else None)
+                                        (pre_xz[known_level],) if known_level in pre_xz else None, lins.pop(lvl, None))
     finally:
         if geo is not None:
             geo.release()
```
